# swacisko/ALGA

Hardware: AMD Instinct MI355X
Metric: overlap_edges_per_sec (higher is better)
Workload: dtype u32; 1 GPU; cfg4_50M_150bp: 50000000 x 150 bp reads, genome 250000000, seed 11, err 0.00 -> 90621096 nodes (both strands, duplicates removed), min_overlap 82, rsoemo 116; generated on the device (alga_amd.workload.device_build) in 1.0 s; nodes=90621096, edges=92350115

## Files before the change

### alga_amd/csrc/engine.hip

```cpp
#include <hip/hip_runtime.h>

#include <algorithm>
#include <chrono>
#include <cstdio>
#include <cstdlib>
#include <cstring>
#include <new>
#include <string>
#include <thread>
#include <vector>

#include "engine_internal.h"
#include "prefsuf_shard.h"

using namespace alga;

namespace {

using Prepared = AlgaPrepared;

int prepare(alga_engine *e, const alga_nodes *nodes, const alga_prefsuf_params *p, hipStream_t s, Prepared &out) {
    if (!nodes || !p) return alga_fail(e, ALGA_ERR_INVALID_ARGUMENT, "nodes/params must not be NULL");
    if (nodes->n < 0) return alga_fail(e, ALGA_ERR_INVALID_ARGUMENT, "negative node count");
    if (nodes->n > 0 && (!nodes->words || !nodes->len)) return alga_fail(e, ALGA_ERR_INVALID_ARGUMENT, "words/len must not be NULL");
    if (nodes->stride_words <= 0 && nodes->n > 0) return alga_fail(e, ALGA_ERR_INVALID_ARGUMENT, "stride_words must be positive");
    if (p->min_overlap < 1 || p->min_overlap > 501) return alga_fail(e, ALGA_ERR_INVALID_ARGUMENT, "min_overlap must be in [1, 501]");
    if (p->soes != 3) return alga_fail(e, ALGA_ERR_INVALID_ARGUMENT, "soes must be 3 (the reference hard-codes SOES = 3)");
    if (p->max_len_cap < 1 || p->max_len_cap > 500) return alga_fail(e, ALGA_ERR_INVALID_ARGUMENT, "max_len_cap must be in [1, 500]");
    if (p->rsoe_min_overlap < 0) return alga_fail(e, ALGA_ERR_INVALID_ARGUMENT, "rsoe_min_overlap must be >= 0");
    if (p->keys_shared < 0 || p->keys_shared > 2) return alga_fail(e, ALGA_ERR_INVALID_ARGUMENT, "keys_shared must be 0, 1 or 2");
    int rc;
    if ((rc = alga_ensure(e, e->counters, (CNT_TOTAL + 2) * sizeof(unsigned long long)))) return rc;
    HIP_TRY(e, hipMemsetAsync(e->counters.p, 0, (CNT_TOTAL + 2) * sizeof(unsigned long long), s));
    NodesDev nd;
    nd.words = nodes->words; nd.len = nodes->len; nd.from = nodes->align_from; nd.to = nodes->align_to;
    nd.n = nodes->n; nd.stride = nodes->stride_words;
    unsigned long long *cnt = (unsigned long long *) e->counters.p;
    int *d_maxlen = (int *) (cnt + CNT_TOTAL);
    unsigned long long mask_asym = 0;
    int min_len = 0;
    if (p->keys_shared == 2 && e->store_n == nodes->n && e->store_words == (const void *) nodes->words && e->stat_len == (const void *) nodes->len &&
        e->stat_from == (const void *) nodes->align_from && e->stat_to == (const void *) nodes->align_to) {
        out.max_len = e->stat_max_len; out.live = e->stat_live; mask_asym = e->stat_mask_asym; min_len = e->stat_min_len;
    } else {
        launch_node_stats(nd, cnt, d_maxlen, s);
        if ((rc = alga_check_launch(e, "k_node_stats"))) return rc;
        HIP_TRY(e, hipMemcpyAsync(e->h_counters, e->counters.p, (CNT_TOTAL + 2) * sizeof(unsigned long long), hipMemcpyDeviceToHost, s));
        HIP_TRY(e, hipStreamSynchronize(s));
        out.max_len = (int) (e->h_counters[CNT_TOTAL] & 0xFFFFFFFFull);
        min_len = out.max_len > 0 ? 0x7FFFFFFF - (int) (e->h_counters[CNT_TOTAL] >> 32) : 0;
        out.live = e->h_counters[CNT_LIVE_NODES];
        mask_asym = e->h_counters[CNT_MASK_ASYM];
        e->stat_max_len = out.max_len; e->stat_min_len = min_len; e->stat_live = out.live; e->stat_mask_asym = mask_asym;
        e->stat_len = (const void *) nodes->len; e->stat_from = (const void *) nodes->align_from; e->stat_to = (const void *) nodes->align_to;
    }
    out.nd = nd;
    out.uniform_len = (out.max_len > 0 && min_len == out.max_len && !nodes->align_from) ? out.max_len : 0;
    if ((int64_t) blocks_of(out.max_len) > (int64_t) nodes->stride_words)
        return alga_fail(e, ALGA_ERR_INVALID_ARGUMENT, "stride_words is smaller than the longest read needs");
    if (out.max_len > OL_MAX_NODE_LEN) return alga_fail(e, ALGA_ERR_CAPACITY, "a node is longer than 4 194 303 nt (overlap records keep the offset in 22 bits)");
    PrefSufCfg c;
    c.Lmin = p->min_overlap;
    c.rsoemo = p->rsoe_min_overlap;
    c.Lcap = std::min(out.max_len, p->max_len_cap) + 1;
    c.soes = p->soes;
    const int seed_nt = std::min(c.Lmin, SEED_MAX_NT);
    c.seed_words = (2 * seed_nt + 31) >> 5;
    c.seed_last_mask = (2 * seed_nt & 31) ? ((1u << (2 * seed_nt & 31)) - 1u) : 0xFFFFFFFFu;
    c.reversed = (c.rsoemo > c.Lcap) ? 1 : 0;
    c.stats = p->collect_stats ? 1 : 0;
    out.cfg = c;
    if (p->reduction < ALGA_REDUCTION_AUTO || p->reduction > ALGA_REDUCTION_SOURCE_SIDE)
        return alga_fail(e, ALGA_ERR_INVALID_ARGUMENT, "reduction must be an alga_reduction value");
    out.local_ok = out.max_len <= p->max_len_cap && out.max_len - c.Lmin <= LOCAL_MAX_SPAN && c.Lmin <= c.rsoemo && c.rsoemo <= c.Lcap &&
                   mask_asym == 0;
    out.local_sw = out.max_len - c.Lmin <= 63 ? 1 : 2;
    out.cluster_eq = 0;
    const bool wide = out.local_sw == 2 || blocks_of(out.max_len) > 13;
    if (out.local_ok && e->opt_probe != ALGA_PROBE_TABLE && !(wide && e->opt_probe == ALGA_PROBE_AUTO && out.live < (4ull << 20))) {
        int eq = 0;
        if (cluster_plan(c, out.max_len, out.live, e->opt_cluster_bucket_bias, &out.cluster, &eq)) out.cluster_eq = eq;
    }
    out.keys_shared = p->keys_shared;
    out.reduction = p->reduction;
    if (out.reduction == ALGA_REDUCTION_AUTO && e->opt_force_per_target) out.reduction = ALGA_REDUCTION_PER_TARGET;
    return ALGA_OK;
}

int cluster_alloc(alga_engine *e, const Prepared &pp) {
    int rc;
    const uint64_t n = (uint64_t) pp.nd.n;
    for (int k = 0; k < 2; k++) {
        if ((rc = alga_ensure(e, e->cl_keys[k], (n + ALGA_KEY_ARRAY_SLACK + 1) * sizeof(uint32_t)))) return rc;
        if ((rc = alga_ensure(e, e->cl_vals[k], (n + 1) * sizeof(uint32_t)))) return rc;
    }
    if ((rc = alga_ensure(e, e->cl_meta, (n + ALGA_KEY_ARRAY_SLACK + 1) * sizeof(uint32_t)))) return rc;
    if ((rc = alga_ensure(e, e->cl_runs, (n + 1) * CL_RMAX * 8))) return rc;
    if ((rc = alga_ensure(e, e->cl_nruns, n + 16))) return rc;
    if ((rc = alga_ensure(e, e->cl_store, (n + 2) * 16 * (size_t) pp.cluster_eq))) return rc;
    if ((rc = alga_ensure(e, e->cl_dir, ((size_t) pp.cluster.n_buckets + 2) * 16))) return rc;
    return alga_ensure(e, e->sort_temp, cluster_sort_temp_bytes(n));
}

int pile_alloc(alga_engine *e, uint64_t n, uint32_t n_buckets, hipStream_t s) {
    int rc;
    if ((rc = alga_ensure(e, e->cl_pile_rec, pile_record_bytes(n)))) return rc;
    if ((rc = alga_ensure(e, e->cl_pile_rec2, pile_record_bytes(n)))) return rc;
    if ((rc = alga_ensure(e, e->cl_pile_succ, ((size_t) n + 64) * 16))) return rc;
    if ((rc = alga_ensure(e, e->cl_pile_cnt, PILE_CNT_WORDS * sizeof(unsigned long long)))) return rc;
    if ((rc = alga_ensure(e, e->cl_pile_own, pile_own_mask_bytes(n)))) return rc;
    if (e->opt_pile_runs_list && (rc = alga_ensure(e, e->cl_pile_list, pile_list_bytes(n)))) return rc;
    if ((rc = alga_ensure(e, e->cl_defer, (size_t) (n + 64) * sizeof(int32_t)))) return rc;
    const void *before = e->cl_pile_tab.p;
    const size_t cap_before = e->cl_pile_tab.cap;
    if ((rc = alga_ensure(e, e->cl_pile_tab, pile_table_bytes(n_buckets)))) return rc;
    if (e->cl_pile_tab.p != before || e->cl_pile_tab.cap != cap_before) {
        HIP_TRY(e, hipMemsetAsync(e->cl_pile_tab.p, 0, e->cl_pile_tab.cap, s));
        HIP_TRY(e, hipStreamSynchronize(s));
        e->pile_epoch = 0;
    }
    return ALGA_OK;
}

int discover_impl(alga_engine *e, const Prepared &pp, int32_t src_begin, int32_t src_end, hipStream_t s, uint64_t *n_rec, bool local = false,
                  bool *overflow = nullptr) {
    int rc;
    const NodesDev &nd = pp.nd;
    const PrefSufCfg &cfg = pp.cfg;
    unsigned long long *cnt = (unsigned long long *) e->counters.p;
    *n_rec = 0;
    HIP_TRY(e, hipEventRecord(e->ev[EV_START], s));
    if (pp.live >= (1ull << 31)) return alga_fail(e, ALGA_ERR_CAPACITY, "too many nodes for one seed table; shard the input");
    const bool clustered = local && pp.cluster_eq != 0;
    e->pairs_timed = false;
    e->store_timed = false;
    e->pile_timed = false;
    e->pile_deg_pending = false;
    const bool all_sources = src_begin == 0 && src_end == pp.nd.n;
    const bool pile_index_left = e->opt_pile_range != 0 && e->pile_n == pp.nd.n && e->pile_words == (const void *) pp.nd.words;
    bool pile = clustered && e->opt_pile != 0 && e->opt_cluster_pairs != 0 && e->opt_cluster_order != 0 && pp.local_sw == 1 &&
                      (pp.keys_shared == 0 || (pp.keys_shared == 2 && pile_index_left)) &&
                      (all_sources || (e->opt_pile_range != 0 && src_begin >= 0 && src_end <= pp.nd.n && src_begin < src_end)) && pile_plan(cfg, pp.cluster, pp.cluster_eq, pp.uniform_len, pp.nd.from != nullptr || pp.nd.to != nullptr);
    e->loc_second_used = false;
    bool keys_only = false;
    const bool need_vals = !e->opt_own_sort || e->opt_test_unsorted_index;
    uint32_t n_buckets = 0, filter_bits = 0;
    bool have_table = false;
    auto build_table = [&]() -> int {
        n_buckets = seed_buckets_for(pp.live, e->seed_fill_x10);
        const size_t table_bytes = (size_t) n_buckets * SEED_BUCKET * sizeof(unsigned long long);
        int r;
        if ((r = alga_ensure(e, e->table, table_bytes))) return r;
        HIP_TRY(e, hipMemsetAsync(e->table.p, 0xFF, table_bytes, s));
        filter_bits = seed_filter_bits_for(pp.live);
        if (filter_bits) {
            if ((r = alga_ensure(e, e->filter, filter_bits / 8))) return r;
            HIP_TRY(e, hipMemsetAsync(e->filter.p, 0, filter_bits / 8, s));
        }
        launch_seed_build(nd, cfg, (unsigned long long *) e->table.p, n_buckets, (uint32_t *) e->filter.p, filter_bits, s);
        if ((r = alga_check_launch(e, "k_seed_build"))) return r;
        e->stats.table_slots = (uint64_t) n_buckets * SEED_BUCKET;
        have_table = true;
        return ALGA_OK;
    };
    ClusterCfg cc{};
    if (clustered) {
        cc = pp.cluster;
        if ((rc = cluster_alloc(e, pp))) return rc;
        if (pp.keys_shared == 2) {
            const bool store_left = e->store_n == nd.n && e->store_words == (const void *) nd.words && e->store_eq == pp.cluster_eq && e->store_buckets == cc.n_buckets;
            const bool piles_serve = pile && e->pile_kept_pure && e->store_buckets == cc.n_buckets && e->store_eq == pp.cluster_eq;
            if (!(store_left || piles_serve) || src_begin < e->store_run_begin || src_end > e->store_run_end)
                return alga_fail(e, ALGA_ERR_INVALID_ARGUMENT, "keys_shared = 2: no entry array of this node set that covers the sources is left from the previous build");
            keys_only = pile && e->pile_keys_only;
        } else {
            int32_t run_begin = 0, run_end = nd.n;
            if (pp.keys_shared == 1) {
                if (e->keyed_n != nd.n || e->keyed_words != (const void *) nd.words || src_begin < e->keyed_begin || src_end > e->keyed_end)
                    return alga_fail(e, ALGA_ERR_INVALID_ARGUMENT, "keys_shared: alga_prefsuf_keys_device has not been called on this node set for a range that covers the sources");
                run_begin = e->keyed_begin; run_end = e->keyed_end;
            } else {
                keys_only = pile && e->opt_pile_runs != 0 && !e->expect_pairwise && !e->opt_pile_check;
                launch_cluster_keys(nd, cfg, cc, 0, nd.n, (uint32_t *) e->cl_keys[0].p, need_vals ? (uint32_t *) e->cl_vals[0].p : nullptr, (uint32_t *) e->cl_meta.p, e->cl_runs.p,
                                    (uint8_t *) e->cl_nruns.p, s, !keys_only);
                if ((rc = alga_check_launch(e, "k_node_runs"))) return rc;
            }
            HIP_TRY(e, hipEventRecord(e->ev[EV_KEYS], s));
            e->keyed_n = -1;
            e->store_n = -1;
            HIP_TRY(e, launch_cluster_sort(nd, cc, (uint32_t *) e->cl_keys[0].p, (uint32_t *) e->cl_vals[0].p, (uint32_t *) e->cl_keys[1].p,
                                           (uint32_t *) e->cl_vals[1].p, e->sort_temp.p, cluster_sort_temp_bytes((uint64_t) nd.n), pp.keys_shared == 1 || !need_vals,
                                           e->ev[EV_SORT], e->opt_test_unsorted_index != 0, s, e->opt_own_sort != 0));
            const bool dir_late = pile && e->opt_pile_dir >= 1;
            e->dir_late = dir_late;
            if (!dir_late) {
                HIP_TRY(e, launch_cluster_dir(nd, cc, (const uint32_t *) e->cl_keys[1].p, e->cl_dir.p, cnt + CNT_TOTAL + 1, nullptr, s));
                HIP_TRY(e, hipEventRecord(e->ev[EV_DIR], s));
            }
            e->pile_n = -1;
            if (pile) {
                rc = e->opt_test_pile_oom ? alga_fail(e, ALGA_ERR_OUT_OF_MEMORY, "pile_alloc (option test_pile_oom)") : pile_alloc(e, (uint64_t) nd.n, cc.n_buckets, s);
                if (rc == ALGA_ERR_OUT_OF_MEMORY) {
                    (void) hipGetLastError();
                    alga_release(e->cl_pile_tab); alga_release(e->cl_pile_rec); alga_release(e->cl_pile_rec2); alga_release(e->cl_pile_succ); alga_release(e->cl_pile_own);
                    alga_release(e->cl_pile_list);
                    e->pile_epoch = 0; e->pile_n = -1;
                    e->err.clear();
                    pile = false;
                    rc = ALGA_OK;
                    if (keys_only) {
                        launch_cluster_keys(nd, cfg, cc, 0, nd.n, (uint32_t *) e->cl_keys[0].p, (uint32_t *) e->cl_vals[0].p, (uint32_t *) e->cl_meta.p, e->cl_runs.p,
                                            (uint8_t *) e->cl_nruns.p, s, true);
                        if ((rc = alga_check_launch(e, "k_node_runs"))) return rc;
                        keys_only = false;
                    }
                } else if (rc) return rc;
            }
            if (pile) {
                launch_pile_sample(nd, cc, pp.uniform_len, (const uint32_t *) e->cl_keys[1].p, (const uint32_t *) e->cl_vals[1].p, e->cl_dir.p,
                                   (unsigned long long *) e->cl_pile_cnt.p, e->opt_pile >= 2 ? e->opt_pile - 1 : 0, s, e->opt_pile_dir >= 1);
                if ((rc = alga_check_launch(e, "k_pile_build<sample>"))) return rc;
            }
            e->pile_tab_index = pile && e->opt_pile_dir >= 2 && e->opt_pile_skip_gather && !cfg.stats;
            if (dir_late) {
                HIP_TRY(e, hipEventRecord(e->ev[EV_SAMPLE], s));
                HIP_TRY(e, launch_cluster_dir(nd, cc, (const uint32_t *) e->cl_keys[1].p, e->cl_dir.p, cnt + CNT_TOTAL + 1,
                                              e->pile_tab_index ? (const unsigned long long *) e->cl_pile_cnt.p : nullptr, s));
                HIP_TRY(e, hipEventRecord(e->ev[EV_DIR], s));
            }
            HIP_TRY(e, launch_cluster_gather(nd, cc, pp.cluster_eq, (const uint32_t *) e->cl_keys[1].p, (const uint32_t *) e->cl_vals[1].p, (const uint32_t *) e->cl_meta.p,
                                             pp.uniform_len, e->cl_store.p, (pile && e->opt_pile_skip_gather) ? (const unsigned long long *) e->cl_pile_cnt.p : nullptr, s));
            HIP_TRY(e, hipEventRecord(e->ev[EV_GATHER], s));
            if (pile) {
                if (e->pile_epoch >= 511u) {
                    HIP_TRY(e, hipMemsetAsync(e->cl_pile_tab.p, 0, e->cl_pile_tab.cap, s));
                    e->pile_epoch = 0;
                }
                e->pile_epoch++;
                const bool from_consensus = e->opt_pile_runs != 0;
                launch_pile_build(nd, cfg, cc, pp.uniform_len, (const uint32_t *) e->cl_keys[1].p, (const uint32_t *) e->cl_vals[1].p, e->cl_dir.p, e->cl_pile_rec.p, e->cl_pile_rec2.p, e->cl_pile_tab.p,
                                  e->pile_epoch, e->cl_pile_succ.p, e->cl_runs.p, pp.uniform_len - cfg.Lmin + 1, (const unsigned long long *) e->cl_pile_cnt.p,
                                  from_consensus ? (uint32_t *) e->cl_pile_own.p : nullptr, (from_consensus && e->opt_pile_runs_list) ? e->cl_pile_list.p : nullptr, s,
                                  e->opt_pile_dir >= 1, cnt + CNT_TOTAL + 1, e->pile_tab_index, e->opt_pile_runs_ahead != 0);
                if ((rc = alga_check_launch(e, "k_pile_build"))) return rc;
                if (keys_only) {
                    launch_pile_own_ids((const uint32_t *) e->cl_pile_own.p, (const uint32_t *) e->cl_vals[1].p, (uint64_t) nd.n, (int32_t *) e->cl_defer.p, (uint32_t) nd.n,
                                        (unsigned long long *) e->cl_pile_cnt.p, s);
                    launch_cluster_runs_list(nd, cfg, cc, (const int32_t *) e->cl_defer.p, (const unsigned long long *) e->cl_pile_cnt.p + 3, (uint32_t) nd.n, (uint32_t) e->n_cu * 16u,
                                             e->cl_runs.p, (uint8_t *) e->cl_nruns.p, s);
                    launch_cluster_keys(nd, cfg, cc, 0, nd.n, (uint32_t *) e->cl_keys[0].p, (uint32_t *) e->cl_vals[0].p, (uint32_t *) e->cl_meta.p, e->cl_runs.p,
                                        (uint8_t *) e->cl_nruns.p, s, true, (const unsigned long long *) e->cl_pile_cnt.p);
                    if ((rc = alga_check_launch(e, "k_node_runs (own lists)"))) return rc;
                }
                if (e->opt_pile_check && from_consensus)
                    launch_pile_check(e->cl_pile_succ.p, (uint64_t) nd.n, cc.n_buckets, e->cl_pile_tab.p, e->cl_pile_rec2.p, e->pile_epoch, e->cl_runs.p, nd.n, pp.uniform_len - cfg.Lmin + 1,
                                      (unsigned long long *) e->cl_pile_cnt.p, s);
                e->pile_n = nd.n; e->pile_words = (const void *) nd.words;
                e->pile_keys_only = keys_only; e->pile_kept_pure = false;
                e->pile_timed = nd.n > 0;
            }
            e->store_timed = nd.n > 0;
            e->store_n = pile ? -1 : nd.n;
            e->store_words = (const void *) nd.words; e->store_eq = pp.cluster_eq; e->store_buckets = cc.n_buckets;
            e->store_run_begin = run_begin; e->store_run_end = run_end;
        }
        e->stats.table_slots = cc.n_buckets;
    } else if ((rc = build_table())) return rc;
    HIP_TRY(e, hipEventRecord(e->ev[EV_SEED], s));

    const uint64_t n_src = (uint64_t) std::max<int64_t>(0, (int64_t) src_end - src_begin);
    const uint64_t slack = std::max(probe_record_slack(e->n_cu, n_src, local), clustered ? cluster_record_slack(e->n_cu, n_src) : 0);
    uint64_t &hint = local ? e->rec_cap_hint_local : e->rec_cap_hint;
    uint64_t cap = std::max<uint64_t>(hint, (local ? 2 : 16) * n_src + 4096) + slack;
    if (local) {
        if ((rc = alga_ensure(e, e->outdeg, (size_t) (n_src + 1) * sizeof(uint32_t)))) return rc;
        if ((rc = alga_ensure(e, e->loc_first, (size_t) (n_src + 1) * sizeof(unsigned long long)))) return rc;
    }
    const uint32_t big_list_cap = 1u << 20;
    if (local && (rc = alga_ensure(e, e->loc_big_list, big_list_cap * sizeof(int32_t)))) return rc;
    bool pure_streamed = false;
    for (int attempt = 0; attempt < 4; attempt++) {
        if (cap >= (1ull << 32) - 16) return alga_fail(e, ALGA_ERR_CAPACITY, "more than 2^32 overlap records; shard the input");
        if (local) HIP_TRY(e, hipMemsetAsync(e->outdeg.p, 0, (size_t) (n_src + 1) * sizeof(uint32_t), s));
        if ((rc = alga_ensure(e, e->rec_dst, cap * sizeof(uint32_t)))) return rc;
        if ((rc = alga_ensure(e, e->rec_val, cap * sizeof(unsigned long long)))) return rc;
        HIP_TRY(e, hipMemsetAsync(cnt, 0, CNT_TOTAL * sizeof(unsigned long long), s));
        ProbeBig big{(int32_t *) e->loc_big_list.p, big_list_cap, 0u, nullptr, 0u};
        e->defer_list_valid = clustered && e->opt_cluster_pairs && pp.local_sw == 1 && pp.cluster_eq <= 4;
        if (clustered) {
            if (e->opt_cluster_pairs && pp.local_sw == 1 && pp.cluster_eq <= 4) {
                if ((rc = alga_ensure(e, e->cl_defer, (size_t) (n_src + 64) * sizeof(int32_t)))) return rc;
                const uint32_t slot_stride = e->opt_stream_slots >= 4 ? (uint32_t) (n_src + 1) : 0u;
                if ((rc = alga_ensure(e, e->loc_second, (size_t) (slot_stride ? LOCAL_SLOTS_MAX - 1 : 1) * (n_src + 1) * sizeof(unsigned long long)))) return rc;
                e->loc_second_used = true;
                e->loc_slot_stride = slot_stride;
                const bool by_key = e->opt_cluster_order != 0 && src_begin == 0 && src_end == nd.n;
                const bool piled = pile && e->pile_n == nd.n && e->pile_words == (const void *) nd.words;
                if (piled) {
                    if (!all_sources) {
                        if ((rc = alga_ensure(e, e->cl_pile_side_r, (size_t) (n_src + 64) * 16))) return rc;
                        if ((rc = alga_ensure(e, e->cl_pile_cursor, 64))) return rc;
                    }
                    launch_pile_probe(nd, cfg, cc, pp.uniform_len, e->cl_pile_tab.p, e->pile_epoch, e->cl_pile_rec.p, e->cl_pile_rec2.p, e->cl_pile_succ.p,
                                      e->cl_runs.p, cnt, (uint32_t *) e->outdeg.p, (unsigned long long *) e->loc_first.p, (unsigned long long *) e->loc_second.p,
                                      (int32_t *) e->cl_defer.p, (uint32_t) n_src, (const unsigned long long *) e->cl_pile_cnt.p, e->n_cu, s, src_begin, src_end,
                                      e->cl_pile_side_r.p, (unsigned long long *) e->cl_pile_cursor.p, e->opt_pile_probe_lean != 0, e->opt_pile_probe_tail != 0);
                    if ((rc = alga_check_launch(e, "k_pile_probe"))) return rc;
                    if (keys_only)
                        launch_cluster_runs_list(nd, cfg, cc, (const int32_t *) e->cl_defer.p, cnt + CNT_DEFERRED, (uint32_t) std::min<uint64_t>(n_src + 64, 0xFFFFFFFFull),
                                                 (uint32_t) e->n_cu * 16u, e->cl_runs.p, (uint8_t *) e->cl_nruns.p, s);
                }
                launch_probe_stream(nd, cfg, cc, pp.cluster_eq, e->cl_store.p, e->cl_dir.p, e->cl_runs.p, (const uint8_t *) e->cl_nruns.p,
                                    src_begin, src_end, by_key, cnt, e->n_cu, (uint32_t *) e->outdeg.p, (unsigned long long *) e->loc_first.p,
                                    (unsigned long long *) e->loc_second.p, (int32_t *) e->cl_defer.p, (uint32_t) n_src,
                                    piled ? (const unsigned long long *) e->cl_pile_cnt.p : nullptr, s, slot_stride);
                if ((rc = alga_check_launch(e, "k_probe_stream"))) return rc;
                if (piled) {
                    if ((rc = alga_ensure(e, e->cl_defer2, (size_t) (n_src + 64) * sizeof(int32_t)))) return rc;
                    pure_streamed = launch_probe_stream_list(nd, cfg, cc, pp.cluster_eq, e->cl_store.p, e->cl_dir.p, e->cl_runs.p, (const uint8_t *) e->cl_nruns.p, (int32_t *) e->cl_defer.p,
                                             (uint32_t) n_src, cnt, e->n_cu, (uint32_t *) e->outdeg.p, (unsigned long long *) e->loc_first.p,
                                             (unsigned long long *) e->loc_second.p, (int32_t *) e->cl_defer2.p, (const unsigned long long *) e->cl_pile_cnt.p, s, slot_stride, src_begin,
                                             (const uint32_t *) e->cl_keys[1].p, (const uint32_t *) e->cl_vals[1].p, pp.uniform_len, e->opt_pile_stream_by_id != 0,
                                             e->pile_tab_index ? e->cl_pile_tab.p : nullptr, e->pile_epoch);
                    if ((rc = alga_check_launch(e, "k_probe_stream (list)"))) return rc;
                }
                HIP_TRY(e, hipEventRecord(e->ev[EV_PAIRS], s));
                e->pairs_timed = true;
                launch_probe_clustered(nd, cfg, cc, pp.cluster_eq, e->cl_store.p, e->cl_dir.p, e->cl_runs.p, (const uint8_t *) e->cl_nruns.p, 0,
                                       (int32_t) n_src, (const int32_t *) e->cl_defer.p, src_begin, (uint32_t *) e->rec_dst.p, (unsigned long long *) e->rec_val.p,
                                       cap, cnt, e->n_cu, (uint32_t *) e->outdeg.p, (unsigned long long *) e->loc_first.p, &big, cnt + CNT_DEFERRED, 1, s,
                                       (const uint32_t *) e->cl_keys[1].p, (const uint32_t *) e->cl_vals[1].p, pp.uniform_len,
                                       (piled && e->opt_pile_skip_gather) ? (const unsigned long long *) e->cl_pile_cnt.p : nullptr,
                                       (piled && e->pile_tab_index) ? e->cl_pile_tab.p : nullptr, e->pile_epoch);
                e->pile_deg_pending = piled && e->opt_pile_deg_fold != 0;
                if (piled && !e->pile_deg_pending) launch_pile_deg((int32_t) n_src, (unsigned long long *) e->loc_first.p, (uint32_t *) e->outdeg.p, (const unsigned long long *) e->cl_pile_cnt.p, s);
            } else {
                launch_probe_clustered(nd, cfg, cc, pp.cluster_eq, e->cl_store.p, e->cl_dir.p, e->cl_runs.p, (const uint8_t *) e->cl_nruns.p, src_begin,
                                       src_end, nullptr, src_begin, (uint32_t *) e->rec_dst.p, (unsigned long long *) e->rec_val.p, cap, cnt, e->n_cu,
                                       (uint32_t *) e->outdeg.p, (unsigned long long *) e->loc_first.p, &big, nullptr, pp.local_sw, s);
            }
        }
        else
            launch_probe(nd, cfg, (const unsigned long long *) e->table.p, n_buckets, (const uint32_t *) e->filter.p, filter_bits, src_begin, src_end,
                         (uint32_t *) e->rec_dst.p, (unsigned long long *) e->rec_val.p, cap, cnt, e->n_cu, local ? pp.local_sw : 0, (uint32_t *) e->outdeg.p,
                         (unsigned long long *) e->loc_first.p, local ? &big : nullptr, s);
        if ((rc = alga_check_launch(e, "k_probe_sources"))) return rc;
        HIP_TRY(e, hipEventRecord(e->ev[EV_PROBE], s));
        HIP_TRY(e, hipMemcpyAsync(e->h_counters, cnt, (CNT_TOTAL + 2) * sizeof(unsigned long long), hipMemcpyDeviceToHost, s));
        HIP_TRY(e, hipStreamSynchronize(s));
        if (clustered && e->h_counters[CNT_TOTAL + 1] != 0) {
            e->store_n = -1; e->keyed_n = -1;
            return alga_fail(e, ALGA_ERR_HIP, "clustered index: the sorted key array is not in order (entry directory invalid)");
        }
        if (local && e->h_counters[CNT_LOCAL_OVERFLOW] != 0) {
            const uint64_t n_big = e->h_counters[CNT_LOCAL_OVERFLOW], max_items = e->h_counters[CNT_LOCAL_MAXITEMS];
            const uint64_t limit = e->big_limit >= 0 ? (uint64_t) e->big_limit : (uint64_t) local_big_limit();
            if (n_big > big_list_cap || max_items > limit) { if (overflow) *overflow = true; *n_rec = 0; return ALGA_OK; }
            big.count = (uint32_t) n_big;
            big.item_cap = (uint32_t) ((max_items + 63) & ~63ull);
            if ((rc = alga_ensure(e, e->loc_big_items, probe_big_bytes(e->n_cu, big.count, pp.local_sw, big.item_cap)))) return rc;
            big.items = e->loc_big_items.p;
            if (!have_table && (rc = build_table())) return rc;
            if (e->pile_deg_pending) {
                launch_pile_deg((int32_t) n_src, (unsigned long long *) e->loc_first.p, (uint32_t *) e->outdeg.p, (const unsigned long long *) e->cl_pile_cnt.p, s);
                e->pile_deg_pending = false;
            }
            HIP_TRY(e, hipMemsetAsync(cnt + CNT_LOCAL_OVERFLOW, 0, sizeof(unsigned long long), s));
            launch_probe(nd, cfg, (const unsigned long long *) e->table.p, n_buckets, (const uint32_t *) e->filter.p, filter_bits, src_begin, src_end,
                         (uint32_t *) e->rec_dst.p, (unsigned long long *) e->rec_val.p, cap, cnt, e->n_cu, pp.local_sw, (uint32_t *) e->outdeg.p,
                         (unsigned long long *) e->loc_first.p, &big, s);
            if ((rc = alga_check_launch(e, "k_probe_sources (second pass)"))) return rc;
            HIP_TRY(e, hipEventRecord(e->ev[EV_PROBE], s));
            HIP_TRY(e, hipMemcpyAsync(e->h_counters, cnt, CNT_TOTAL * sizeof(unsigned long long), hipMemcpyDeviceToHost, s));
            HIP_TRY(e, hipStreamSynchronize(s));
            if (e->h_counters[CNT_LOCAL_OVERFLOW] != 0) { if (overflow) *overflow = true; *n_rec = 0; return ALGA_OK; }
            e->stats.big_sources = n_big;
        }
        const uint64_t need = e->h_counters[CNT_RECORDS];
        if (need <= cap) {
            *n_rec = need;
            hint = std::max<uint64_t>(hint, need + need / 16 + 4096);
            if (overflow) *overflow = false;
            if (local) { e->stats.transitive_compares = e->h_counters[CNT_TR_COMPARES]; e->stats.generic_sources = e->h_counters[CNT_LOCAL_GENERIC]; }
            e->stats.records = e->h_counters[CNT_VALID_RECORDS];
            e->stats.raw_overlaps = e->h_counters[CNT_RAW];
            e->stats.windows_probed = e->h_counters[CNT_WINDOWS];
            e->stats.slots_scanned = e->h_counters[CNT_SLOTS];
            e->stats.probe_rounds = e->h_counters[CNT_ROUNDS];
            e->stats.pile_buckets = e->h_counters[CNT_PILE_BUCKETS]; e->stats.pile_irregular = e->h_counters[CNT_PILE_IRREGULAR];
            e->stats.pile_own_lists = e->h_counters[CNT_PILE_OWN];
            if (pile && pp.keys_shared != 2 && e->pile_n == nd.n) {
                const bool kept = e->opt_pile == 2 || e->stats.pile_irregular * (uint64_t) ALGA_PILE_DECLINE_ONE_IN <= e->stats.pile_buckets;
                e->stats.pile_mixed = kept && e->stats.pile_irregular * (uint64_t) ALGA_PILE_IRREGULAR_ONE_IN > e->stats.pile_buckets;
                e->stats.pile_deferred = (e->stats.pile_mixed || (kept && pure_streamed)) ? e->h_counters[CNT_DEFERRED_PILE] : (kept ? e->h_counters[CNT_DEFERRED] : 0);
                if (!kept || e->stats.pile_mixed || !e->opt_pile_skip_gather) e->store_n = nd.n;
                e->expect_pairwise = !kept;
                e->pile_kept_pure = kept && !e->stats.pile_mixed && e->opt_pile_skip_gather != 0;
                e->stats.pile_list_checked = 0; e->stats.pile_list_mismatch = 0;
                if (e->opt_pile_check) {
                    unsigned long long chk[2] = {0ull, 0ull};
                    HIP_TRY(e, hipMemcpyAsync(chk, (const unsigned long long *) e->cl_pile_cnt.p + 4, sizeof(chk), hipMemcpyDeviceToHost, s));
                    HIP_TRY(e, hipStreamSynchronize(s));
                    e->stats.pile_list_checked = chk[0]; e->stats.pile_list_mismatch = chk[1];
// ... 130 lines not shown
    return ALGA_OK;
}

double now_ms_host() { return std::chrono::duration<double, std::milli>(std::chrono::steady_clock::now().time_since_epoch()).count(); }

float ev_ms(alga_engine *e, int a, int b) {
    float ms = 0.f;
    if (hipEventElapsedTime(&ms, e->ev[a], e->ev[b]) != hipSuccess) return 0.f;
    return ms;
}

void store_phase_stats(alga_engine *e) {
    if (!e->store_timed) return;
    e->stats.ms_keys = ev_ms(e, EV_START, EV_KEYS);
    e->stats.ms_sort = ev_ms(e, EV_KEYS, EV_SORT);
    e->stats.ms_dir = ev_ms(e, e->dir_late ? EV_SAMPLE : EV_SORT, EV_DIR);
    e->stats.ms_gather = ev_ms(e, EV_DIR, EV_GATHER) + (e->dir_late ? ev_ms(e, EV_SORT, EV_SAMPLE) : 0.0);
    e->stats.ms_pile = e->pile_timed ? ev_ms(e, EV_GATHER, EV_SEED) : 0.0;
}

}

int alga_prepare(alga_engine *e, const alga_nodes *nodes, const alga_prefsuf_params *p, hipStream_t s, AlgaPrepared &out) { return prepare(e, nodes, p, s, out); }
int alga_cluster_alloc(alga_engine *e, const AlgaPrepared &pp) { return cluster_alloc(e, pp); }

extern "C" {

int alga_abi_version(void) { return ALGA_AMD_ABI_VERSION; }

struct DeviceGuard {
    int prev = -1;
    DeviceGuard() { if (hipGetDevice(&prev) != hipSuccess) prev = -1; }
    ~DeviceGuard() { if (prev >= 0) (void) hipSetDevice(prev); }
};

static void engine_free_handles(alga_engine *e) {
    if (e->h_counters) (void) hipHostFree(e->h_counters);
    for (int i = 0; i < EV_COUNT; i++) if (e->ev[i]) (void) hipEventDestroy(e->ev[i]);
    if (e->own_stream) (void) hipStreamDestroy(e->own_stream);
    if (e->side_stream) (void) hipStreamDestroy(e->side_stream);
    if (e->ev_side) (void) hipEventDestroy(e->ev_side);
    e->h_counters = nullptr; e->own_stream = nullptr; e->side_stream = nullptr; e->ev_side = nullptr;
    for (int i = 0; i < EV_COUNT; i++) e->ev[i] = nullptr;
}

int alga_engine_create(int hip_device, alga_engine **out) {
    if (!out) return ALGA_ERR_INVALID_ARGUMENT;
    *out = nullptr;
    int ndev = 0;
    hipError_t err = hipGetDeviceCount(&ndev);
    if (err != hipSuccess || ndev <= 0) return ALGA_ERR_NO_DEVICE;
    if (hip_device < 0 || hip_device >= ndev) return ALGA_ERR_INVALID_ARGUMENT;
    DeviceGuard guard;
    if (hipSetDevice(hip_device) != hipSuccess) return ALGA_ERR_NO_DEVICE;
    alga_engine *e = new (std::nothrow) alga_engine();
    if (!e) return ALGA_ERR_OUT_OF_MEMORY;
    e->device = hip_device;
    memset(&e->stats, 0, sizeof(e->stats));
    hipDeviceProp_t prop;
    if (hipGetDeviceProperties(&prop, hip_device) == hipSuccess) {
        snprintf(e->dev_name, sizeof(e->dev_name), "%s (%s, %d CUs)", prop.name, prop.gcnArchName, prop.multiProcessorCount);
        if (prop.multiProcessorCount > 0) e->n_cu = prop.multiProcessorCount;
    }
    int rc = ALGA_OK;
    if (hipStreamCreateWithFlags(&e->own_stream, hipStreamNonBlocking) != hipSuccess) { e->own_stream = nullptr; rc = ALGA_ERR_HIP; }
    if (rc == ALGA_OK && hipStreamCreateWithFlags(&e->side_stream, hipStreamNonBlocking) != hipSuccess) { e->side_stream = nullptr; rc = ALGA_ERR_HIP; }
    if (rc == ALGA_OK && hipEventCreateWithFlags(&e->ev_side, hipEventDisableTiming) != hipSuccess) { e->ev_side = nullptr; rc = ALGA_ERR_HIP; }
    for (int i = 0; i < EV_COUNT && rc == ALGA_OK; i++)
        if (hipEventCreate(&e->ev[i]) != hipSuccess) { e->ev[i] = nullptr; rc = ALGA_ERR_HIP; }
    if (rc == ALGA_OK && hipHostMalloc((void **) &e->h_counters, (CNT_TOTAL + 2 + alga_engine::H_EXTRA) * sizeof(unsigned long long)) != hipSuccess) { e->h_counters = nullptr; rc = ALGA_ERR_OUT_OF_MEMORY; }
    if (rc == ALGA_OK && hipHostGetDevicePointer((void **) &e->h_counters_dev, e->h_counters, 0) != hipSuccess) rc = ALGA_ERR_HIP;
    if (rc != ALGA_OK) { engine_free_handles(e); delete e; return rc; }
    *out = e;
    return ALGA_OK;
}

void alga_engine_destroy(alga_engine *e) {
    if (!e) return;
    DeviceGuard guard;
    (void) hipSetDevice(e->device);
    if (e->own_stream) (void) hipStreamSynchronize(e->own_stream);
    if (e->side_stream) (void) hipStreamSynchronize(e->side_stream);
    for (DevBuf *b : e->owned) alga_release(*b);
    alga_release(e->up_raw);
    for (DevBuf *b : {&e->in_bytes[0], &e->in_bytes[1], &e->in_nl[0], &e->in_nl[1], &e->in_tiles, &e->in_tile_off}) alga_release(*b);
    for (DevBuf *b : {&e->sp_rowptr, &e->sp_sorted, &e->sp_list, &e->sp_cnt, &e->sp_orow, &e->sp_out, &e->sp_in}) alga_release(*b);
    alga_staging_release(e);
    for (void *&p : e->gfa_pin) { if (p) (void) hipHostFree(p); p = nullptr; }
    for (auto &kv : e->host_lists) free(kv.first);
    e->host_lists.clear();
    engine_free_handles(e);
    delete e;
}

const char *alga_last_error(const alga_engine *e) { return e ? e->err.c_str() : "no engine"; }

int alga_engine_device_name(const alga_engine *e, char *buf, size_t buflen) {
    if (!e || !buf || buflen == 0) return ALGA_ERR_INVALID_ARGUMENT;
    snprintf(buf, buflen, "%s", e->dev_name);
    return ALGA_OK;
}

int alga_engine_set_option(alga_engine *e, const char *name, int64_t value) {
    if (!e || !name) return ALGA_ERR_INVALID_ARGUMENT;
    e->err.clear();
    if (!strcmp(name, "probe")) {
        if (value < ALGA_PROBE_AUTO || value > ALGA_PROBE_CLUSTER) return alga_fail(e, ALGA_ERR_INVALID_ARGUMENT, "option probe: 0 auto, 1 table, 2 cluster");
        e->opt_probe = (int) value;
    } else if (!strcmp(name, "cluster_bucket_bias")) {
        if (value < -8 || value > 8) return alga_fail(e, ALGA_ERR_INVALID_ARGUMENT, "option cluster_bucket_bias: -8 .. 8");
        e->opt_cluster_bucket_bias = (int) value;
    } else if (!strcmp(name, "cluster_pairs")) {
        e->opt_cluster_pairs = value != 0;
    } else if (!strcmp(name, "pile")) {
        e->opt_pile = (value == 2 || value == 3) ? (int) value : (value != 0);
    } else if (!strcmp(name, "pile_runs")) {
        e->opt_pile_runs = value != 0;
    } else if (!strcmp(name, "pile_runs_list")) {
        e->opt_pile_runs_list = value != 0;
    } else if (!strcmp(name, "pile_dir")) {
        if (value < 0 || value > 2) return alga_fail(e, ALGA_ERR_INVALID_ARGUMENT, "option pile_dir: 0 directory records, 1 k_pile_build from the keys, 2 ... and no directory for a pure pile build");
        e->opt_pile_dir = (int) value;
    } else if (!strcmp(name, "pile_deg_fold")) {
        e->opt_pile_deg_fold = value != 0;
    } else if (!strcmp(name, "emit_fused")) {
        e->opt_emit_fused = value != 0;
    } else if (!strcmp(name, "pile_probe_lean")) {
        e->opt_pile_probe_lean = value != 0;
    } else if (!strcmp(name, "pile_probe_tail")) {
        e->opt_pile_probe_tail = value != 0;
    } else if (!strcmp(name, "pile_runs_ahead")) {
        e->opt_pile_runs_ahead = value != 0;
    } else if (!strcmp(name, "pile_stream_by_id")) {
        e->opt_pile_stream_by_id = value != 0;
    } else if (!strcmp(name, "pile_check")) {
        e->opt_pile_check = value != 0;
    } else if (!strcmp(name, "pile_skip_gather")) {
        e->opt_pile_skip_gather = value != 0;
    } else if (!strcmp(name, "cluster_order")) {
        e->opt_cluster_order = value != 0;
    } else if (!strcmp(name, "local_big_max")) {
        e->big_limit = value < 0 ? -1 : (int) std::min<int64_t>(value, 1 << 20);
    } else if (!strcmp(name, "shard_bucket_max")) {
        e->opt_shard_dmax = (int) std::max<int64_t>(1, std::min<int64_t>(value, 4096));
    } else if (!strcmp(name, "rsort_variant")) {
        if (value < 0 || value > 1) return alga_fail(e, ALGA_ERR_INVALID_ARGUMENT, "option rsort_variant: 0 tiles of 8192 pairs, 1 tiles of 16384 pairs");
        rsort_set_variant((int) value);
    } else if (!strcmp(name, "stream_slots")) {
        e->opt_stream_slots = value >= 4 ? 4 : 2;
    } else if (!strcmp(name, "pile_range")) {
        e->opt_pile_range = value != 0;
    } else if (!strcmp(name, "pkb_legacy")) {
        e->opt_pkb_legacy = (int) value;
    } else if (!strcmp(name, "own_sort")) {
        e->opt_own_sort = value != 0;
    } else if (!strcmp(name, "test_presort_oom")) {
        e->opt_test_presort_oom = value != 0;
    } else if (!strcmp(name, "test_pile_oom")) {
        e->opt_test_pile_oom = value != 0;
    } else if (!strcmp(name, "test_unsorted_index")) {
        e->opt_test_unsorted_index = value != 0;
    } else if (!strcmp(name, "gfa_chunk_mb")) {
        if (value < 1 || value > 4096) return alga_fail(e, ALGA_ERR_INVALID_ARGUMENT, "option gfa_chunk_mb: 1 .. 4096");
        e->opt_gfa_chunk_mb = (int) value;
    } else if (!strcmp(name, "mst_mid_nodes")) {
        if (value < 8 || value > (1 << 20)) return alga_fail(e, ALGA_ERR_INVALID_ARGUMENT, "option mst_mid_nodes: 8 .. 2^20");
        e->opt_mst_mid_nodes = (int) value;
    } else if (!strcmp(name, "consensus_max_blocks")) {
        if (value < 0 || value > (1 << 20)) return alga_fail(e, ALGA_ERR_INVALID_ARGUMENT, "option consensus_max_blocks: 0 .. 2^20");
        e->opt_consensus_max_blocks = (int) value;
    } else if (!strcmp(name, "unitig_ruling")) {
        if (value < -1 || value > 1) return alga_fail(e, ALGA_ERR_INVALID_ARGUMENT, "option unitig_ruling: -1, 0 or 1");
        e->opt_unitig_ruling = (int) value;
    } else if (!strcmp(name, "correct_slice_keys")) {
        if (value < 1 || value > (1ll << 31)) return alga_fail(e, ALGA_ERR_INVALID_ARGUMENT, "option correct_slice_keys: 1 .. 2^31");
        e->opt_correct_slice_keys = value;
    } else if (!strcmp(name, "correct_dir_bits")) {
        if (value < 0 || value > 28) return alga_fail(e, ALGA_ERR_INVALID_ARGUMENT, "option correct_dir_bits: 0 (auto) or 1 .. 28");
        e->opt_correct_dir_bits = (int) value;
    } else if (!strcmp(name, "place_dir_bits")) {
        if (value < 0 || value > 26) return alga_fail(e, ALGA_ERR_INVALID_ARGUMENT, "option place_dir_bits: 0 (auto) or 1 .. 26");
        e->opt_place_dir_bits = (int) value;
    } else if (!strcmp(name, "ipolish_max_blocks")) {
        if (value < 1 || value > 8192) return alga_fail(e, ALGA_ERR_INVALID_ARGUMENT, "option ipolish_max_blocks: 1 .. 8192");
        e->opt_ipolish_max_blocks = (int) value;
    } else if (!strcmp(name, "auto_reduction_per_target")) {
        e->opt_force_per_target = value != 0;
    } else return alga_fail(e, ALGA_ERR_INVALID_ARGUMENT, "unknown option");
    return ALGA_OK;
}

int alga_engine_reserve(alga_engine *e, int32_t n_nodes, int32_t max_len, int32_t min_overlap, uint64_t n_edges_hint) {
    if (!e) return ALGA_ERR_INVALID_ARGUMENT;
    e->err.clear();
    if (n_nodes < 0 || max_len < 1 || min_overlap < 1) return alga_fail(e, ALGA_ERR_INVALID_ARGUMENT, "alga_engine_reserve: n_nodes >= 0, max_len >= 1, min_overlap >= 1");
    DeviceGuard guard;
    HIP_TRY(e, hipSetDevice(e->device));
    int rc;
    const uint64_t n = (uint64_t) n_nodes;
    const uint64_t E = n_edges_hint ? n_edges_hint : n + n / 16 + 4096;
    if ((rc = alga_ensure(e, e->counters, (CNT_TOTAL + 2) * sizeof(unsigned long long)))) return rc;
    Prepared pp;
    pp.nd.n = n_nodes; pp.max_len = max_len; pp.live = n;
    pp.cfg.Lmin = min_overlap; pp.cfg.Lcap = std::min(max_len, 500) + 1; pp.cfg.rsoemo = min_overlap; pp.cfg.soes = 3;
    int eq = 0;
    const bool local = max_len <= 500 && max_len - min_overlap <= LOCAL_MAX_SPAN;
    const bool clustered = local && e->opt_probe != ALGA_PROBE_TABLE &&
                           cluster_plan(pp.cfg, max_len, n, e->opt_cluster_bucket_bias, &pp.cluster, &eq);
    if (clustered) {
        pp.cluster_eq = eq;
        if ((rc = cluster_alloc(e, pp))) return rc;
        if (max_len - min_overlap <= 63 && eq <= 4) {
            if ((rc = alga_ensure(e, e->cl_defer, (size_t) (n + 64) * sizeof(int32_t)))) return rc;
            if ((rc = alga_ensure(e, e->loc_second, (size_t) (e->opt_stream_slots >= 4 ? LOCAL_SLOTS_MAX - 1 : 1) * (n + 1) * sizeof(unsigned long long)))) return rc;
        }
        if (e->opt_pile != 0 && e->opt_cluster_pairs != 0 && e->opt_cluster_order != 0 && max_len - min_overlap <= 63 && pile_plan(pp.cfg, pp.cluster, eq, max_len, false)) {
            if ((rc = pile_alloc(e, n, pp.cluster.n_buckets, e->own_stream))) return rc;
        }
    } else {
        const uint32_t nb = seed_buckets_for(n, e->seed_fill_x10);
        if ((rc = alga_ensure(e, e->table, (size_t) nb * SEED_BUCKET * sizeof(unsigned long long)))) return rc;
        const uint32_t fb = seed_filter_bits_for(n);
        if (fb && (rc = alga_ensure(e, e->filter, fb / 8))) return rc;
    }
    if (local) {
        const uint64_t slack = std::max(probe_record_slack(e->n_cu, n, true), clustered ? cluster_record_slack(e->n_cu, n) : 0);
        const uint64_t cap = std::max<uint64_t>(e->rec_cap_hint_local, 2 * n + 4096) + slack;
        if ((rc = alga_ensure(e, e->outdeg, (size_t) (n + 1) * sizeof(uint32_t)))) return rc;
        if ((rc = alga_ensure(e, e->loc_first, (size_t) (n + 1) * sizeof(unsigned long long)))) return rc;
        if ((rc = alga_ensure(e, e->loc_big_list, (1u << 20) * sizeof(int32_t)))) return rc;
        if ((rc = alga_ensure(e, e->rec_dst, cap * sizeof(uint32_t)))) return rc;
        if ((rc = alga_ensure(e, e->rec_val, cap * sizeof(unsigned long long)))) return rc;
        if ((rc = alga_ensure(e, e->scan_scratch, scan_scratch_bytes(n)))) return rc;
        if ((rc = alga_ensure(e, e->out_rowptr, (size_t) (n + 1) * sizeof(uint32_t)))) return rc;
        if ((rc = alga_ensure(e, e->out_cnt, (size_t) (n + 1) * sizeof(uint32_t)))) return rc;
    }
    if ((rc = alga_ensure(e, e->edges, (size_t) (E + 1) * sizeof(alga_edge_dev)))) return rc;
    if (!e->warmed && n_nodes > 0) {
        const int W = blocks_of(max_len), stride = hbm_row_stride(W), wn = 4096;
        std::vector<uint32_t> rows((size_t) wn * stride, 0u);
        std::vector<int32_t> lens((size_t) wn, max_len);
        uint64_t x = 0x9E3779B97F4A7C15ull;
        for (int i = 0; i < wn; i++)
            for (int k = 0; k < W; k++) {
                x ^= x << 13; x ^= x >> 7; x ^= x << 17;
                uint32_t w = (uint32_t) (x >> 16);
                const int used = 2 * max_len - 32 * k;
                if (used < 32) w &= used <= 0 ? 0u : ((1u << used) - 1u);
                rows[(size_t) i * stride + k] = w;
            }
        void *d_rows = nullptr, *d_len = nullptr;
        if (hipMalloc(&d_rows, rows.size() * 4) == hipSuccess && hipMalloc(&d_len, lens.size() * 4) == hipSuccess &&
            hipMemcpy(d_rows, rows.data(), rows.size() * 4, hipMemcpyHostToDevice) == hipSuccess &&
            hipMemcpy(d_len, lens.data(), lens.size() * 4, hipMemcpyHostToDevice) == hipSuccess) {
            alga_nodes nd{(const uint32_t *) d_rows, stride, (const int32_t *) d_len, wn, nullptr, nullptr};
            alga_prefsuf_params wp;
            alga_prefsuf_default_params(&wp);
            wp.min_overlap = min_overlap; wp.rsoe_min_overlap = std::min(max_len, min_overlap + (max_len - min_overlap) / 2);
            const alga_edge *d = nullptr;
            uint64_t m = 0;
            const int wrc = alga_prefsuf_build_device(e, &nd, &wp, nullptr, &d, &m);
            (void) wrc;
            e->err.clear();
            e->warmed = true;
        }
        if (d_rows) (void) hipFree(d_rows);
        if (d_len) (void) hipFree(d_len);
        (void) hipGetLastError();
        alga_forget_node_set(e);
        memset(&e->stats, 0, sizeof(e->stats));
    }
    return ALGA_OK;
}

void alga_prefsuf_default_params(alga_prefsuf_params *p) {
    if (!p) return;
    memset(p, 0, sizeof(*p));
    p->min_overlap = 0;
    p->rsoe_min_overlap = 0;
    p->soes = 3;
    p->max_len_cap = 500;
    p->collect_stats = 0;
}

int alga_prefsuf_build_device(alga_engine *e, const alga_nodes *nodes, const alga_prefsuf_params *p, void *hip_stream,
                              const alga_edge **d_edges, uint64_t *n_edges) {
    if (!e) return ALGA_ERR_INVALID_ARGUMENT;
    e->err.clear();
    if (!d_edges || !n_edges) return alga_fail(e, ALGA_ERR_INVALID_ARGUMENT, "output pointers must not be NULL");
    *d_edges = nullptr; *n_edges = 0;
    HIP_TRY(e, hipSetDevice(e->device));
    hipStream_t s = hip_stream ? (hipStream_t) hip_stream : e->own_stream;
    memset(&e->stats, 0, sizeof(e->stats));
    Prepared pp;
    int rc = prepare(e, nodes, p, s, pp);
    if (rc) return rc;
    e->stats.nodes_live = pp.live;
    uint64_t n_rec = 0, E = 0;
    bool done = false;
    if (pp.reduction == ALGA_REDUCTION_SOURCE_SIDE || (pp.reduction == ALGA_REDUCTION_AUTO && pp.local_ok)) {
        rc = build_local(e, pp, 0, nodes->n, s, &E);
        if (rc == ALGA_OK) done = true;
        else if (rc != ALGA_ERR_UNSUPPORTED || pp.reduction == ALGA_REDUCTION_SOURCE_SIDE) return rc;
        else { e->err.clear(); memset(&e->stats, 0, sizeof(e->stats)); e->stats.nodes_live = pp.live; }
    }
    if (!done) {
// ... 581 lines not shown
```

### alga_amd/csrc/engine_internal.h

```cpp
#pragma once
#include <hip/hip_runtime.h>

#include <cstdio>
#include <algorithm>
#include <string>
#include <vector>
#include <unordered_map>

#include "../../include/alga_amd.h"
#include "prefsuf_common.h"
#include "prefsuf_kernels.h"
#include "pkb_kernels.h"

struct DevBuf {
    void  *p = nullptr;
    size_t cap = 0;
};

enum { EV_START = 0, EV_SEED, EV_PROBE, EV_GROUP, EV_REDUCE, EV_EMIT, EV_PAIRS, EV_KEYS, EV_SORT, EV_GATHER, EV_DIR, EV_SAMPLE, EV_COUNT };
constexpr int ALGA_STAGE_THREADS = 8;

struct alga_engine {
    std::vector<DevBuf *> owned;
    int         device = -1;
    hipStream_t own_stream = nullptr;
    hipStream_t side_stream = nullptr;
    hipEvent_t  ev_side = nullptr;
    std::string err;
    char        dev_name[256] = {0};
    int         n_cu = 256;
    int         seed_fill_x10 = 20;
    int         opt_probe = 0;
    int         opt_cluster_bucket_bias = 0;
    int         opt_force_per_target = 0;
    int         opt_shard_dmax = 4096;
    int         opt_test_unsorted_index = 0;
    hipEvent_t  ev[EV_COUNT] = {};
    DevBuf table, filter, counters, rowptr, rec_dst, rec_val, keys, seg_key, seg_val, heads, sort_temp, out_cnt, outdeg, out_rowptr, edges, scan_scratch;
    DevBuf cl_defer;
    uint32_t h_first_hkey = 255;
    int32_t keyed_n = -1, keyed_begin = 0, keyed_end = 0;
    bool defer_list_valid = false;
    const void *keyed_words = nullptr;
    int32_t store_n = -1, store_run_begin = 0, store_run_end = 0, store_eq = 0;
    uint32_t store_buckets = 0;
    const void *store_words = nullptr;
    int stat_max_len = 0, stat_min_len = 0; uint64_t stat_live = 0; unsigned long long stat_mask_asym = 0;
    const void *stat_len = nullptr, *stat_from = nullptr, *stat_to = nullptr;
    bool   warmed = false;
    bool   pairs_timed = false;
    bool   store_timed = false;
    bool   pile_keys_only = false, pile_kept_pure = false;
    int    opt_pile_range = 1;
    int    opt_pile_skip_gather = 1;
    int    opt_pile = 1;
    int    opt_pile_runs = 1;
    int    opt_pile_runs_list = 1;
    DevBuf cl_pile_list;
    int    opt_pile_deg_fold = 1;
    int    opt_emit_fused = 1;
    int    opt_pile_dir = 2;
    bool   dir_late = false;
    bool   pile_tab_index = false;
    int    opt_pile_stream_by_id = 0;
    int    opt_pile_probe_lean = 1;
    int    opt_pile_probe_tail = 1;
    int    opt_pile_runs_ahead = 0;
    bool   pile_deg_pending = false;
    int    opt_pile_check = 0;
    bool   expect_pairwise = false;
    DevBuf cl_pile_side_r, cl_pile_cursor;
    DevBuf cl_pile_own;
    int    opt_pkb_legacy = 0;
    int    opt_own_sort = 1;
    int    opt_test_presort_oom = 0;
    int    opt_test_pile_oom = 0;
    bool   pile_timed = false;
    DevBuf cl_pile_succ;
    DevBuf cl_pile_rec2;
    DevBuf cl_pile_rec, cl_pile_cnt, cl_pile_tab;
    uint32_t pile_epoch = 0;
    int32_t pile_n = -1; const void *pile_words = nullptr;
    int    opt_cluster_order = 1;
    int    opt_cluster_pairs = 1;
    DevBuf cl_keys[2], cl_vals[2], cl_meta, cl_runs, cl_nruns, cl_store, cl_dir;
    DevBuf loc_second;
    bool   loc_second_used = false;
    uint32_t loc_slot_stride = 0;
    int    opt_stream_slots = 4;
    DevBuf loc_first, loc_big_list, loc_big_items;
    int    big_limit = -1;
    DevBuf edge_keys, edge_keys2, edge_vals, edge_vals2, edges_sorted, xs_dst, xs_val;
    DevBuf up_words, up_len, up_from, up_to;
    DevBuf up_len_narrow;
    DevBuf cp_deg, cp_dst, cp_off;
    DevBuf cl_defer2;
    DevBuf pk_keys, pk_keys2, pk_vals, pk_vals2, pk_marks, pk_big, pk_add, pk_ekeys, pk_ekeys2, pk_flag, pk_pos, pk_edges[2], pk_rowptr, pk_deg,
           pk_mask, pk_cnt, pk_io, pk_io2, pk_tips, pk_heads, pk_g[2], pk_addk, pk_addk2, pk_merged, pk_hsz, pk_hsz2, pk_heads2, pk_nadd, pk_koff,
           pk_gsz, pk_fixlist, pk_bounds, pk_tiprec, pk_tipidx, pk_keys_all, pk_vals_all;
    DevBuf pk_keys2b, pk_vals2b, pk_headsb, pk_hszb, sort_temp2, pk_fixlist2, pk_cnt2;
    DevBuf pp_rows, pp_len, pp_perm[2], pp_keys[2], pp_mark, pp_keep, pp_pos, pp_out_rows, pp_out_len, pp_out_pair, pp_tally;
    bool        stage_ready = false;
    void       *stage_pin[ALGA_STAGE_THREADS][2] = {};
    hipEvent_t  stage_ev[ALGA_STAGE_THREADS][2] = {};
    hipStream_t stage_stream[ALGA_STAGE_THREADS] = {};
    DevBuf      up_raw;
    std::unordered_map<void *, size_t> host_lists;
    void       *host_spare = nullptr;
    size_t      host_spare_cap = 0;
    DevBuf      in_bytes[2], in_nl[2], in_tiles, in_tile_off;
    DevBuf      sp_rowptr, sp_sorted, sp_list, sp_cnt, sp_orow, sp_out, sp_in;
    DevBuf      tp_cnt, tp_keys[2], tp_vals[2], tp_flag, tp_pos, tp_best, tp_est, tp_rev, tp_rfid, tp_rowptr[2], tp_alive, tp_kill, tp_rec[2], tp_branch,
                tp_overflow, tp_ws, tp_out;
    DevBuf      mp_cnt, mp_rowptr, mp_rows, mp_len, mp_owner, mp_pend[2], mp_win, mp_overflow, mp_overflow2, mp_ws, mp_ws_big, mp_orow, mp_out;
    struct MstFilled { const void *p = nullptr; size_t bytes = 0; uint32_t hbits = 0, cap_nodes = 0, cap_edges = 0; int32_t n_ws = 0; } mp_filled[2];
    int         opt_mst_mid_nodes = 4096;
    DevBuf      gfa_sizes, gfa_off, gfa_rowptr, gfa_tiles, gfa_bounds, gfa_buf;
    void       *gfa_pin[2] = {nullptr, nullptr};
    size_t      gfa_pin_cap = 0;
    int         opt_gfa_chunk_mb = 256;
    DevBuf      ut_cnt, ut_keys[2], ut_vals[2], ut_flag, ut_pos, ut_best, ut_estar, ut_rowptr, ut_nxt, ut_noff, ut_prv, ut_rank[2], ut_min[2], ut_tail,
                ut_win, ut_pair, ut_pcnt, ut_ulen, ut_ulen2, ut_uwords, ut_path_off, ut_word_off, ut_tiles, ut_path_node, ut_path_pos, ut_uid, ut_words,
                ut_edges, ut_link, ut_rnode, ut_rrec[2];
    int         opt_unitig_ruling = -1;
    uint64_t    ut_n_pairs = 0, ut_n_edges = 0;
    bool        ut_valid = false;
    int32_t     ut_n_nodes = 0;
    uint64_t    ut_total_bases = 0;
    bool        ut_is_contig = false;
    DevBuf      ex_cnt, ex_rowptr, ex_w, ex_kcnt, ex_dlink, ex_outcnt, ex_sole, ex_xhead, ex_xbase, ex_xrank, ex_uid, ex_scnt, ex_seam_off,
                ex_seam_entry, ex_pcnt, ex_uwords, ex_ulen, ex_ulen2, ex_path_off, ex_word_off, ex_path_node, ex_path_pos, ex_words, ex_edges;
    bool        ut_is_extended = false;
    DevBuf      ct_cnt, ct_B[2], ct_rowptr, ct_pflag, ct_runkey, ct_chain, ct_headchain, ct_drop, ct_flag, ct_pos, ct_keys[2], ct_vals[2], ct_hw, ct_hk, ct_H,
                ct_hrow, ct_hsorted, ct_hlist, ct_hcnt, ct_win, ct_pair, ct_oid, ct_cid, ct_deg, ct_epos, ct_ekeys[2], ct_evals[2], ct_names;
    DevBuf      cs_cnt, cs_words, cs_mask, cs_votes, cs_trim, cs_len, cs_changed;
    bool        cs_valid = false;
    bool        cs_has_votes = false;
    DevBuf      fc_cnt, fc_keys[2], fc_vals, fc_first, fc_min, fc_list[2], fc_flag, fc_ids, fc_verdict, fc_rank, fc_id, fc_new, fc_trim, fc_begin, fc_len,
                fc_order, fc_wbegin, fc_wlen, fc_rows, fc_rlen, fc_tid;
    bool        fc_valid = false;
    uint64_t    fc_n_accepted = 0;
    int         opt_consensus_max_blocks = 0;
    DevBuf      cr_cnt, cr_table, cr_hist, cr_keys[2], cr_flag, cr_pos, cr_solid, cr_dir;
    int64_t     opt_correct_slice_keys = 1ll << 28;
    int         opt_correct_dir_bits = 0;
    DevBuf      seed_keys[2], seed_vals[2], seed_dir, seed_ub;
    DevBuf      pl_cnt, pl_fbegin, pl_flen, pl_scan, pl_cols, pl_diff;
    DevBuf      pl_target, pl_pos, pl_mm, pl_hits, pl_state, pl_coloff, pl_cover, pl_tstat, pl_hist;
    bool        pl_valid = false;
    uint64_t    pl_targets = 0, pl_reads = 0;
    uint64_t    pl_ncolumns = 0, pl_nhist = 0;
    uint64_t    pl_final_epoch = 0;
    uint64_t    fc_epoch = 0;
    int         opt_place_dir_bits = 0;
    DevBuf      po_cnt, po_keys[2], po_vals[2], po_marks, po_pop, po_scan;
    DevBuf      po_coloff, po_words, po_ccols, po_cbases, po_tstat, po_counts;
    bool        po_valid = false;
    uint64_t    po_targets = 0, po_columns = 0;
    uint64_t    po_final_epoch = 0;
    uint64_t    pl_serial = 0, po_pl_serial = 0;
    DevBuf      sc_cnt, sc_keys[2], sc_vals[2], sc_span, sc_heads, sc_pos, sc_bstart, sc_best, sc_choice, sc_partner, sc_lists[2], sc_head, sc_first, sc_scan;
    DevBuf      sc_ba, sc_bb, sc_blinks, sc_bspan, sc_bgap, sc_bstate, sc_estate, sc_scaffold, sc_rank, sc_orient, sc_start, sc_gapafter, sc_jlinks, sc_soff,
                sc_smembers, sc_slen;
    bool        sc_valid = false;
    uint64_t    sc_targets = 0, sc_scaffolds = 0, sc_longest = 0;
    uint64_t    sc_pl_serial = 0;
    DevBuf      br_cnt, br_diff, br_starts, br_rpos, br_marks, br_rfirst, br_rlast, br_closed, br_cpos;
    DevBuf      br_span, br_ccols, br_cfirst, br_clast, br_tcuts, br_poff, br_begin, br_len, br_ptarget, br_pstart, br_words;
    bool        br_valid = false;
    uint64_t    br_targets = 0, br_pieces = 0, br_cuts = 0, br_columns = 0, br_longest = 0;
    DevBuf      gr_cnt, gr_flag, gr_pos, gr_cand, gr_elen, gr_eoff, gr_ecols, gr_x, gr_g;
    struct GrowSet { DevBuf end, over, mm, hits, state, count, estop, evoters, left, right, len, coloff, begin, words; } gr_set[2];
    int         gr_cur = 0;
    bool        gr_valid = false;
    uint64_t    gr_reads = 0, gr_targets = 0, gr_columns = 0, gr_longest = 0;
    DevBuf      mg_cnt, mg_elen, mg_epad, mg_eoff, mg_ecols, mg_pcols, mg_join, mg_lists[2], mg_head, mg_first, mg_scan;
    struct MergeSet { DevBuf partner, olen, mm, hits, estate, merged, rank, orient, start, ovafter, moff, mmembers, len, coloff, begin, words; } mg_set[2];
    int         mg_cur = 0;
    bool        mg_valid = false;
    uint64_t    mg_targets = 0, mg_merged = 0, mg_columns = 0, mg_longest = 0;
    DevBuf      gp_cnt, gp_flag, gp_pos, gp_list, gp_cols, gp_best, gp_runs, gp_nruns, gp_diff, gp_scan;
    DevBuf      gp_target, gp_rpos, gp_end, gp_edits, gp_state, gp_cigoff, gp_cigar, gp_cover, gp_tstat;
    bool        gp_valid = false;
    uint64_t    gp_reads = 0, gp_targets = 0, gp_columns = 0, gp_ncigar = 0;
    uint64_t    gp_pl_serial = 0;
    DevBuf      ip_cnt, ip_keys[2], ip_vals[2], ip_marks, ip_pop, ip_pwords, ip_ptstat, ip_counts4, ip_del, ip_diff, ip_scan, ip_ikey[2], ip_islot[2], ip_winkey,
                ip_winvotes, ip_insall, ip_width, ip_evn, ip_evoff, ip_code;
    struct IpolishSet { DevBuf len, coloff, begin, words, newcol, evcol, evkind, evlen, evbases, evvotes, evcover, tstat, counts, span, oldoff; } ip_set[2];
    int         ip_cur = 0;
    int         opt_ipolish_max_blocks = 8192;
    bool        ip_valid = false;
    uint64_t    ip_targets = 0, ip_columns = 0, ip_columns_before = 0, ip_events = 0, ip_longest = 0;
    DevBuf      sh_keys[2], sh_vals[2], sh_store, sh_dir, sh_desc_out, sh_dkey[2], sh_dval[2], sh_small_top, sh_pending, sh_bitmap, sh_small_out,
                sh_ssrc[2], sh_skey[2], sh_edges_out, sh_deg, sh_rowptr, sh_cursor, sh_edges, sh_flagged, sh_cnt, sh_gflag, sh_gpos, sh_gstart;
    struct {
        int      phase = 0;
        int      rank = 0, n_ranks = 1, eq = 0, uniform_len = 0;
        int32_t  n = 0;
        const void *words = nullptr;
        alga::PrefSufCfg cfg{};
        alga::ClusterCfg cc{};
        uint32_t bucket_base = 0, bpr = 0;
        uint64_t n_targets = 0, n_desc = 0, n_rec = 0;
        uint32_t *d_keys_sorted = nullptr;
        unsigned long long *d_vals_sorted = nullptr;
    } sh;
    alga_shard_stats shard_stats{};
    struct {
        int      phase = 0;
        int      rounds = 0, round = 0, rank = 0, n_ranks = 1, cur = 0, key_bits = 0;
        int32_t  prio[4] = {0, 1, 2, 3};
        uint64_t E = 0, nk = 0;
        uint32_t n_tips = 0;
        int      pre_set = 0, cur_set = 0;
        bool     no_look_ahead = false;
        int      pre_round = -1;
        bool     kmers_all = false;
        size_t   kmers_stride = 0;
        int      kmers_sort_bits = 0;
        alga_nodes dn{};
// ... 122 lines not shown
```

### alga_amd/csrc/prefsuf_cluster.hip

```cpp
#include <hip/hip_runtime.h>
#include <algorithm>
#include "prefsuf_common.h"
#include "prefsuf_kernels.h"
#include "prefsuf_device.h"
#include "prefsuf_cluster_device.h"

namespace alga {


template <int TKW, bool WIDE, bool RUNS>
__global__ void __launch_bounds__(TK_ROWS) k_node_runs(NodesDev nd, PrefSufCfg cfg, ClusterCfg cc, int node_begin, int node_end,
                                                        uint32_t *__restrict__ keys, uint32_t *__restrict__ vals, uint32_t *__restrict__ meta,
                                                        uint2 *__restrict__ runs, uint8_t *__restrict__ nruns, const int32_t *__restrict__ id_list, const unsigned long long *__restrict__ id_count,
                                                        const unsigned long long *__restrict__ only_if_declined ) {
    if (only_if_declined && !pile_cnt_declines(only_if_declined)) return;
    __shared__ uint32_t s[TK_ROWS][TKW];
    __shared__ uint32_t stk[RUNS ? 2 * (NR_STACK + 1) : 1][TK_ROWS];
    __shared__ uint16_t rbuf[RUNS ? CL_RMAX + 1 : 1][TK_ROWS];
    const int list_n = id_list ? (int) min((unsigned long long) (node_end - node_begin), *id_count) : 0;
    __shared__ int sid[TK_ROWS];
    for (int blk = (int) blockIdx.x; id_list ? blk * TK_ROWS < list_n : node_begin + blk * TK_ROWS < node_end; blk += (int) gridDim.x) {
    const int base = node_begin + blk * TK_ROWS;
    const int nrows = id_list ? min(TK_ROWS, list_n - blk * TK_ROWS) : min(TK_ROWS, node_end - base);
    if (blk != (int) blockIdx.x) __syncthreads();
    if (id_list) {
        if ((int) threadIdx.x < nrows) sid[threadIdx.x] = min(max(id_list[blk * TK_ROWS + (int) threadIdx.x], 0), nd.n - 1);
        __syncthreads();
    }
    if ((nd.stride & 3) == 0 && 4 * ((TKW + 3) / 4) <= nd.stride && (reinterpret_cast<uintptr_t>(nd.words) & 15u) == 0) {
        constexpr int PCS = (TKW + 3) / 4;
        for (int u = (int) threadIdx.x; u < nrows * PCS; u += TK_ROWS) {
            const int r = u / PCS, pc = u - r * PCS;
            const uint4 x = *reinterpret_cast<const uint4 *>(nd.words + (size_t) (id_list ? sid[r] : base + r) * nd.stride + 4 * pc);
            const uint32_t xs[4] = {x.x, x.y, x.z, x.w};
#pragma unroll
            for (int q = 0; q < 4; q++) if (4 * pc + q < TKW) s[r][4 * pc + q] = xs[q];
        }
    } else
    for (int c = (int) (threadIdx.x & 15u); c < TKW; c += 16)
        for (int r = (int) (threadIdx.x >> 4); r < nrows; r += TK_ROWS / 16)
            s[r][c] = c < nd.stride ? nd.words[(size_t) (id_list ? sid[r] : base + r) * nd.stride + c] : 0u;
    __syncthreads();
    const int t = (int) threadIdx.x;
    const bool in = t < nrows;
    const int i = id_list ? sid[in ? t : 0] : base + (in ? t : 0);
    const int len = in ? nd.len[i] : 0;
    const bool act = in && len >= cfg.Lmin && len > 0;
    const bool is_tgt = act && (!nd.to || nd.to[i]);
    const bool is_src = act && (!nd.from || nd.from[i]);
    const uint32_t *row = s[in ? t : 0];
    const int w = cc.w;
    const int nwin = len - cfg.Lmin + 1;
    const int fs = cc.idx_shift - CL_MBITS;
    int nr = 0;
    bool uncovered = false;
    bool stack_ovf = false;
    uint32_t cur0 = 0xFFFFFFFFu;
    if (RUNS) {
        node_runs_core<WIDE>(row, nwin, act, cc, stk, rbuf, t, nr, uncovered, stack_ovf, cur0);
        const int nr_stored = nr < CL_RMAX ? nr : CL_RMAX;
        const uint32_t nr_code = !is_src ? 0u : ((nr > CL_RMAX || stack_ovf || uncovered) ? (uint32_t) CL_RUNS_FLAGGED : (uint32_t) nr);
        int p1 = nwin;
        for (int r = 0; r < CL_RMAX; r++) {
            if (r < nr_stored && is_src) {
                const uint32_t d = rbuf[r][t];
                const int q = (int) (d & 255u);
                uint32_t h, pk;
                kmer_key(row, q < (WIDE ? 192 : 128) ? q : 0, true, cc, h, pk);
                runs[(size_t) i * CL_RMAX + r] = make_uint2(cluster_key(h, fs), d | ((uint32_t) p1 << 16) | (r == 0 ? nr_code << 24 : 0u));
                p1 = (int) (d >> 8);
            }
        }
        if (in && !is_src) runs[(size_t) i * CL_RMAX] = make_uint2(0u, 0u);
        if (in) nruns[i] = (uint8_t) nr_code;
        if (id_list) continue;
    } else {
        const int nk = act ? min(nwin, WIDE ? 64 : nwin) - 1 + w : 0;
        uint64_t b0;
        {
            const uint32_t x0 = row[0], x1 = row[1], x2 = row[2], x3 = row[3], x4 = row[4];
            const uint32_t d0 = compress_even(class0_mask16(x0, x1)) | (compress_even(class0_mask16(x1, x2)) << 16);
            const uint32_t d1 = compress_even(class0_mask16(x2, x3)) | (compress_even(class0_mask16(x3, x4)) << 16);
            b0 = (uint64_t) d0 | ((uint64_t) d1 << 32);
            b0 &= nk >= 64 ? ~0ull : (nk <= 0 ? 0ull : ((1ull << nk) - 1ull));
            b0 &= w >= 64 ? ~0ull : ((1ull << w) - 1ull);
        }
        while (b0 != 0ull) {
            const int e = __builtin_ctzll(b0);
            b0 &= b0 - 1ull;
            const int bit = 2 * e, q = bit >> 5, r = bit & 31;
            const uint32_t x0 = row[q], x1 = row[q + 1], x2 = row[q + 2];
            const uint32_t pk = order_key0(kmer_hash(funnel(x0, x1, r) & cc.lo_mask, funnel(x1, x2, r) & cc.hi_mask), e);
            cur0 = pk < cur0 ? pk : cur0;
        }
    }
    uint32_t key = 0xFFFFFFFFu, m = act ? (((uint32_t) len << 8) | (is_src ? CL_META_FROM : 0u)) : 0u;
    if (is_tgt) {
        uint32_t pmin = cur0;
        if (pmin == 0xFFFFFFFFu) {
            for (int k = 0; k < w; k++) { uint32_t h, pk; kmer_key(row, k, true, cc, h, pk); pmin = pk < pmin ? pk : pmin; }
        }
        uint32_t h, pk;
        kmer_key(row, (int) (pmin & 255u), true, cc, h, pk);
        key = tgt_sort_key(cluster_key(h, fs), pmin & 255u, fs);
        m = (pmin & 255u) | ((uint32_t) len << 8) | (is_src ? CL_META_FROM : 0u);
    }
    if (in) { keys[i] = key; if (vals) vals[i] = (uint32_t) i; meta[i] = m; }
    }
}

template <int EQ, bool UNIFORM>
__global__ void __launch_bounds__(256) k_tgt_gather(NodesDev nd, uint64_t count ,
                                                     const uint32_t *__restrict__ keys, const uint32_t *__restrict__ vals,
                                                     const uint32_t *__restrict__ meta, uint32_t uniform_meta, int fs, uint4 *__restrict__ store,
                                                     const unsigned long long *__restrict__ pile_cnt ) {
    if (pile_cnt && pile_cnt[1] * PILE_IRREGULAR_ONE_IN <= pile_cnt[0]) return;
    for (uint64_t t = (uint64_t) blockIdx.x * blockDim.x + threadIdx.x; t < count * EQ; t += (uint64_t) gridDim.x * blockDim.x) {
    const uint64_t j = t / EQ;
    const int c = (int) (t % EQ);
    const uint32_t key = keys[j];
    const uint32_t id = vals[j];
    const uint32_t *row = nd.words + (size_t) id * nd.stride;
    uint4 v;
    if ((nd.stride & 3) == 0 && 4 * c + 3 < nd.stride && ((uintptr_t) nd.words & 15u) == 0) v = reinterpret_cast<const uint4 *>(row)[c];
    else {
        v.x = 4 * c + 0 < nd.stride ? row[4 * c + 0] : 0u; v.y = 4 * c + 1 < nd.stride ? row[4 * c + 1] : 0u;
        v.z = 4 * c + 2 < nd.stride ? row[4 * c + 2] : 0u; v.w = 4 * c + 3 < nd.stride ? row[4 * c + 3] : 0u;
    }
    if (c == EQ - 1) {
        v.y = id; v.z = key;
        if (!UNIFORM) v.w = meta[id];
        else if (key != 0xFFFFFFFFu) v.w = uniform_meta | ((key >> fs) & ((1u << CL_MBITS) - 1u));
        else v.w = (uint32_t) nd.len[id] == (uniform_meta >> 8 & 0xFFFu) ? uniform_meta : 0u;
    }
    store[j * EQ + c] = v;
    }
}

constexpr int TD_TILE = 256, TD_HALO = 96;
__global__ void __launch_bounds__(TD_TILE) k_tgt_dir(const uint32_t *__restrict__ keys, uint64_t n, int shift, uint32_t n_buckets ,
                                                     uint32_t bucket_base , uint4 *__restrict__ dir,
                                                     unsigned long long *__restrict__ bad ,
                                                     const unsigned long long *__restrict__ pile_cnt ) {
    if (pile_cnt && pile_cnt_pure(pile_cnt)) return;
    __shared__ uint32_t sb[TD_TILE + TD_HALO + 1];
    const uint64_t base = (uint64_t) blockIdx.x * TD_TILE;
    const uint32_t nb3 = n_buckets << 3;
    auto tagged = [&](uint64_t k) -> uint32_t { if (k >= n) return nb3; const uint32_t x = keys[k]; return x == 0xFFFFFFFFu ? nb3 : (x >> (shift - 3)) - (bucket_base << 3); };
    for (int k = (int) threadIdx.x; k <= TD_TILE + TD_HALO; k += TD_TILE)
        sb[k] = (base == 0 && k == 0) ? 0xFFFFFFFFu : tagged(base + (uint64_t) k - 1u);
    __syncthreads();
    const int t = (int) threadIdx.x, lane = lane_id();
    const uint64_t j = base + (uint64_t) t;
    auto put = [&](int64_t b, const uint4 &rec) { dir[b] = rec; };
    auto tally = [](unsigned long long acc, uint32_t cls) { return acc + (0x0101010101010100ull << (8u * cls)); };
    if (j >= 1 && j < n && sb[t + 1] < sb[t]) atomicOr(bad, 1ull);
    const uint32_t b = sb[t + 1] >> 3;
    const bool start = j <= n && b != (sb[t] >> 3);
    if (start && b == n_buckets) put(b, make_uint4((uint32_t) j, 0u, 0u, 0u));
    const bool real = start && b != n_buckets;
    constexpr int TD_SHORT = 4;
    const bool is_short = real && (sb[t + 1 + TD_SHORT] >> 3) != b;
    if (is_short) {
        unsigned long long acc = 0ull;
        int u = 0;
#pragma unroll
        for (; u < TD_SHORT; u++) {
            const uint32_t x = sb[t + 1 + u];
            if ((x >> 3) != b) break;
            acc = tally(acc, x & 7u);
        }
        put(b, make_uint4((uint32_t) j, (uint32_t) u, (uint32_t) acc, (uint32_t) (acc >> 32)));
    }
    unsigned long long longs = __ballot(real && !is_short);
    const int g = lane >> 4, gl = lane & 15;
    while (longs != 0ull) {
        int lsel = 64;
#pragma unroll
        for (int q = 0; q < 4; q++) {
            const int l = longs ? __builtin_ctzll(longs) : 64;
            longs = longs ? (longs & (longs - 1ull)) : 0ull;
            lsel = g == q ? l : lsel;
        }
        const bool has = lsel < 64;
        const int t0 = (t & ~63) + (has ? lsel : 0);
        const uint32_t bb = bperm(b, has ? lsel : 0);
        unsigned long long acc = 0ull;
        bool open = has, past = false;
        for (int u = 0;; u += 16) {
            const int idx = t0 + 1 + u + gl;
            const bool staged = idx <= TD_TILE + TD_HALO;
            const uint32_t x = staged ? sb[idx] : 0xFFFFFFFFu;
            const bool inb = open && staged && (x >> 3) == bb;
            const unsigned long long c = inb ? ((0x0101010101010100ull << (8u * (x & 7u))) | 1ull) : 0ull;
            uint32_t lo = (uint32_t) c, hi = (uint32_t) (c >> 32);
            lo += (uint32_t) __builtin_amdgcn_update_dpp(0, (int) lo, 0x111, 0xF, 0xF, true); hi += (uint32_t) __builtin_amdgcn_update_dpp(0, (int) hi, 0x111, 0xF, 0xF, true);
            lo += (uint32_t) __builtin_amdgcn_update_dpp(0, (int) lo, 0x112, 0xF, 0xF, true); hi += (uint32_t) __builtin_amdgcn_update_dpp(0, (int) hi, 0x112, 0xF, 0xF, true);
            lo += (uint32_t) __builtin_amdgcn_update_dpp(0, (int) lo, 0x114, 0xF, 0xF, true); hi += (uint32_t) __builtin_amdgcn_update_dpp(0, (int) hi, 0x114, 0xF, 0xF, true);
            lo += (uint32_t) __builtin_amdgcn_update_dpp(0, (int) lo, 0x118, 0xF, 0xF, true); hi += (uint32_t) __builtin_amdgcn_update_dpp(0, (int) hi, 0x118, 0xF, 0xF, true);
            lo = bperm(lo, lane | 15); hi = bperm(hi, lane | 15);
            acc += ((unsigned long long) hi << 32) | lo;
            const uint32_t took = lo & 255u, cnt = (uint32_t) acc & 255u;
            if (open && took < 16u) { open = false; past = t0 + 1 + u + (int) took > TD_TILE + TD_HALO; }
            else if (open && cnt >= 240u) { open = false; past = true; }
            if (__ballot(open) == 0ull) break;
        }
        if (has && gl == 0) {
            const uint64_t j0 = base + (uint64_t) t0;
            uint64_t k = j0 + (uint64_t) ((uint32_t) acc & 255u);
            acc &= ~255ull;
            if (past) {
                for (; k < j0 + 256u; k++) {
                    const uint32_t x = tagged(k);
                    if ((x >> 3) != bb) break;
                    acc = tally(acc, x & 7u);
                }
                if (k >= j0 + 256u && (tagged(k) >> 3) == bb) {
                    uint64_t a = k, z = n;
                    while (z - a > 1) { const uint64_t mid = a + (z - a) / 2; if ((tagged(mid) >> 3) == bb) a = mid; else z = mid; }
                    k = z;
                }
            }
            const uint32_t c = (uint32_t) (k - j0);
            put(bb, make_uint4((uint32_t) j0, c, c <= 255u ? (uint32_t) acc : 0u, c <= 255u ? (uint32_t) (acc >> 32) : 0u));
        }
    }
}

#ifndef CL_OCC
#define CL_OCC 6
#endif

struct ByIdEntries {
    const uint32_t *skeys, *sids;
    uint32_t uniform_meta;
    const unsigned long long *pile_cnt;
    BucketIndex bx;
};
__device__ __forceinline__ void by_id_pair(const ByIdEntries &by, size_t ei, uint32_t n_nodes, uint32_t &key, uint32_t &id) {
    key = by.skeys[ei];
    id = min(by.sids[ei], n_nodes - 1u);
}
template <int EQ>
__device__ __forceinline__ void entry_by_id(const NodesDev &nd, uint32_t uniform_meta, int fs, uint32_t key, uint32_t id, uint32_t (&ew)[4 * EQ]) {
    static_assert(EQ == 3, "entries by id: rows of nine words");
    const uint32_t *row = nd.words + (size_t) id * nd.stride;
    if ((nd.stride & 3) == 0 && nd.stride >= 12 && ((uintptr_t) nd.words & 15u) == 0) {
        const uint4 v0 = reinterpret_cast<const uint4 *>(row)[0], v1 = reinterpret_cast<const uint4 *>(row)[1];
        ew[0] = v0.x; ew[1] = v0.y; ew[2] = v0.z; ew[3] = v0.w; ew[4] = v1.x; ew[5] = v1.y; ew[6] = v1.z; ew[7] = v1.w;
        ew[8] = row[8];
    } else {
#pragma unroll
        for (int k = 0; k < 9; k++) ew[k] = k < nd.stride ? row[k] : 0u;
    }
    ew[9] = id; ew[10] = key;
    ew[11] = key != 0xFFFFFFFFu ? (uniform_meta | ((key >> fs) & ((1u << CL_MBITS) - 1u))) : 0u;
}
template <bool STATS, int EQ, int KF, int SW = 1, bool BYID = false>
__global__ void __launch_bounds__(PROBE_WAVES * 64, SW == 1 && EQ <= 4 ? CL_OCC : 4)
k_probe_clustered(NodesDev nd, PrefSufCfg cfg, ClusterCfg cc, const uint4 *__restrict__ store, const uint4 *__restrict__ dir,
// ... 645 lines not shown
                    const int rho_j = lenj - (lenBs - dj), Lv = lenj - (d - dj);
                    const bool vok = ((mjj & ITEM_FROM) != 0u) & (Cj != id) & (dj < d) & (Lv >= Lbig) & (rho_j <= rho) & ((rho_j > 0) | ((int) Cj > Bs));
                    const uint4 m4 = sMask[min(max(2 * rho_j, 0), 128)];
                    const uint32_t df = ((oi.w[0] ^ oj.w[0]) & m4.x) | ((oi.w[1] ^ oj.w[1]) & m4.y) | ((oi.w[2] ^ oj.w[2]) & m4.z) | ((oi.w[3] ^ oj.w[3]) & m4.w);
                    return want & vok & (df == 0u);
                } else return want && via_ok<1>(Bs, lenBs, Lbig, Cj, mjj, oj, id, d, rho, oi);
            };
            bool removed = via_of(j, has_pred);
            const int reach = (cfg.Lcap - 1) - Lbig;
            uint64_t cand = 0ull;
            if (pass && has_pred && !removed) {
                cand = below & ~(1ull << (63 - __clzll((long long) below)));
                if (d - reach > 0) cand &= ~((1ull << (d - reach)) - 1ull);
            }
            while (__ballot(cand != 0ull) != 0ull) {
                const bool need = cand != 0ull;
                const int top = need ? 63 - __clzll((long long) cand) : 0;
                const int j2 = need ? (int) Tb[top] : lane;
                const bool r2 = via_of(j2, need);
                removed = removed | r2;
                cand = (need && !r2) ? cand & ~(1ull << top) : 0ull;
                n_tried2 += need ? 1 : 0;
            }
            const bool keep = pass && !removed;
            if (clash) atomicOr(stp, 1u);
            if (keep) atomicAdd(stp, 0x100u);
            wave_lds_fence();
            stv = *stp;
            if (keep && stv == 0x100u) {
                o.first[Bs - o.src_base] = ((unsigned long long) id << 32) | (uint32_t) d;
                o.deg[Bs - o.src_base] = 1u;
                st_rec++;
            }
            const uint32_t nst = stv >> 8;
            const bool seg_multi = ev && (stv & 255u) == 0u && nst >= 2u && nst <= max_stand;
            if (__ballot(seg_multi) != 0ull) {
                uint64_t segm = 0ull;
#pragma unroll
                for (int q = 0; q < 8; q++) { const uint64_t mq = __ballot(ev && s8 == q); segm = s8 == q ? mq : segm; }
                const uint64_t km = __ballot(keep) & segm;
                const int ds0 = lenBs - cfg.rsoemo + 1;
                const uint64_t lowm = ds0 <= 0 ? 0ull : (ds0 >= 64 ? ~0ull : ((1ull << ds0) - 1ull));
                const bool my_kept = pass && (d < ds0 || __popcll(below & ~lowm) < 3);
                bool fin_me = false;
                uint64_t kmr = seg_multi ? km : 0ull;
                for (int it = 0; it < LOCAL_SLOTS_MAX; it++) {
                    if (__ballot(kmr != 0ull) == 0ull) break;
                    const bool on = kmr != 0ull;
                    const int sl = on ? __builtin_ctzll(kmr) : lane;
                    kmr = on ? kmr & (kmr - 1ull) : 0ull;
                    const uint32_t Cs = bperm(id, sl);
                    const int dsl = (int) bperm((uint32_t) d, sl);
                    const bool ks = bperm(my_kept ? 1u : 0u, sl) != 0u;
                    const uint64_t supm = __ballot(on && my_kept && id == Cs && d < dsl) & segm;
                    if (on && lane == sl) fin_me = ks && supm == 0ull;
                }
                const uint64_t F = __ballot(fin_me) & segm;
                if (fin_me) {
                    const int r = __popcll(F & ((1ull << lane) - 1ull));
                    const unsigned long long mine = ((unsigned long long) id << 32) | (uint32_t) d;
                    if (r == 0) { o.first[Bs - o.src_base] = mine; o.deg[Bs - o.src_base] = (uint32_t) __popcll(F); }
                    else o.second[(size_t) (r - 1) * o.slot_stride + (size_t) (Bs - o.src_base)] = mine;
                    st_rec++;
                }
            }
        }
        if (STATS) {
            st_rounds++;
            const bool fin = ev && (stv & 255u) == 0u && (stv >> 8) <= max_stand;
            st_slots += fin; st_raw += fin && pass; st_cmp += (fin && has_pred ? 1 : 0) + (fin ? n_tried2 : 0);
        }
        if (gl == 0) {
            if (g >= cur && g < e) {
                const uint32_t sv = sStat[wave][4 * b0 + g];
                const bool ok = ((fl0 >> g) & 1u) != 0u && (sv & 255u) == 0u && (sv >> 8) <= max_stand;
                red = ok ? red | 1u : red & ~1u;
                if (STATS && ok) st_win += (uint64_t) ((int) sSrc[wave][4 * b0 + g].y - cfg.Lmin + 1);
            }
            if (4 + g >= cur && 4 + g < e) {
                const uint32_t sv = sStat[wave][4 * b1 + g];
                const bool ok = ((fl1 >> g) & 1u) != 0u && (sv & 255u) == 0u && (sv >> 8) <= max_stand;
                red = ok ? red | 2u : red & ~2u;
                if (STATS && ok) st_win += (uint64_t) ((int) sSrc[wave][4 * b1 + g].y - cfg.Lmin + 1);
            }
        }
        const uint32_t ninc = finish_runs(b2, nnr_eff, nrun, nrec);
        cur = e;
        if (rot) {
            n_seen += __popc(fl0 >> 4);
            defer_rows(gl == 0 && ((fl0 >> (4 + g)) & 1u) != 0u && (red & 1u) == 0u, (int) sSrc[wave][4 * b0 + g].x);
            uint32_t t4w, fl2;
            quad_plan(ninc, nnr, t4w, fl2);
            tw = (tw >> 32) | ((uint64_t) t4w << 32);
            fl0 = fl1; fl1 = fl2;
            red >>= 1;
            const int bt = b0; b0 = b1; b1 = b2; b2 = bt;
            pos0 = step <= src_end - pos0 ? pos0 + step : src_end;
            have0 = pos0 < src_end;
            cur -= 4;
            bail = n_seen >= 192 && 2 * n_deferred > n_seen;
        }
    }
    if (bail && have0) {
        defer_rows(gl == 0 && g < cur && ((fl0 >> (4 + g)) & 1u) != 0u && (red & 1u) == 0u, (int) sSrc[wave][4 * b0 + g].x);
        bool first = true;
        for (int q = pos0; q < src_end; q = step <= src_end - q ? q + step : src_end) {
            const int j = q + g < src_end ? q + g : last_src;
            const int b = BYKEY ? (int) reinterpret_cast<const uint32_t *>(store)[(size_t) j * (4 * EQ) + 4 * EQ - 3]
                                : (LIST ? (int) min((uint32_t) src_list[j], (uint32_t) nd.n - 1u) : j);
            const bool dfr = gl == 0 && q + g < src_end && !(first && g < cur) && (run_w[(size_t) b * (2 * CL_RMAX) + 1] >> 24) != 0u;
            defer_rows(dfr, b);
            first = false;
        }
    }
    flush_defer();
    st_rec = wave_sum_u64(st_rec);
    if (lane == 0 && st_rec) atomicAdd(&o.counters[CNT_VALID_RECORDS], (unsigned long long) st_rec);
    if (STATS) {
        st_raw = wave_sum_u64(st_raw); st_slots = wave_sum_u64(st_slots); st_win = wave_sum_u64(st_win); st_cmp = wave_sum_u64(st_cmp);
        if (lane == 0) {
            atomicAdd(&o.counters[CNT_RAW], (unsigned long long) st_raw);
            atomicAdd(&o.counters[CNT_SLOTS], (unsigned long long) st_slots);
            atomicAdd(&o.counters[CNT_WINDOWS], (unsigned long long) st_win);
            atomicAdd(&o.counters[CNT_TR_COMPARES], (unsigned long long) st_cmp);
            atomicAdd(&o.counters[CNT_ROUNDS], (unsigned long long) st_rounds);
        }
    }
}

bool cluster_plan(const PrefSufCfg &cfg, int max_len, uint64_t live, int bucket_log2_bias, ClusterCfg *c, int *eq) {
    const int W = blocks_of(max_len);
    int e = (W + 3 + 3) / 4;
    if (e < 2) e = 2;
    const int nwin = max_len - cfg.Lmin + 1;
    if (e > CL_MAX_EQ || nwin < 1 || nwin > 128) return false;
    int kk = std::min(32, std::max(cfg.Lmin - 63, std::min(cfg.Lmin, CL_KMIN)));
    const int nw_half = std::min(nwin, 64);
    if (nw_half > std::min(cfg.Lmin - kk + 1, 64)) kk = cfg.Lmin - nw_half + 1;
    if (kk < CL_KMIN_HARD || kk > 32 || kk > cfg.Lmin) return false;
    c->kk = kk;
    c->w = std::min(cfg.Lmin - kk + 1, 64);
    c->lo_mask = kk >= 16 ? 0xFFFFFFFFu : ((1u << (2 * kk)) - 1u);
    c->hi_mask = kk <= 16 ? 0u : (kk >= 32 ? 0xFFFFFFFFu : ((1u << (2 * kk - 32)) - 1u));
    int bits = 4;
    while (bits < 28 && (1ull << bits) < live) bits++;
    bits = std::max(4, std::min(32 - CL_MBITS, bits + bucket_log2_bias));
    c->n_buckets = 1u << bits;
    c->idx_shift = 32 - bits;
    *eq = e;
    return true;
}

size_t cluster_sort_temp_bytes(uint64_t n) { return sort_u32_pairs_temp_bytes(n); }

void launch_cluster_keys(const NodesDev &nd, const PrefSufCfg &cfg, const ClusterCfg &cc, int32_t node_begin, int32_t node_end, uint32_t *keys, uint32_t *vals,
                         uint32_t *meta, void *runs, uint8_t *nruns, hipStream_t s, bool with_runs, const unsigned long long *only_if_declined) {
    if (node_end <= node_begin) return;
    const uint64_t m = (uint64_t) (node_end - node_begin);
    const unsigned long long *gate = only_if_declined;
    const dim3 grid((unsigned) (gate ? std::min<uint64_t>((m + TK_ROWS - 1) / TK_ROWS, 8192) : (m + TK_ROWS - 1) / TK_ROWS)), block(TK_ROWS);
    const int32_t *nol = nullptr; const unsigned long long *noc = nullptr;
#define NR_LAUNCH(TKW, WIDE) do { if (with_runs) hipLaunchKernelGGL((k_node_runs<TKW, WIDE, true>), grid, block, 0, s, nd, cfg, cc, (int) node_begin, (int) node_end, keys, vals, meta, (uint2 *) runs, nruns, nol, noc, gate); \
                                  else hipLaunchKernelGGL((k_node_runs<TKW, WIDE, false>), grid, block, 0, s, nd, cfg, cc, (int) node_begin, (int) node_end, keys, vals, meta, (uint2 *) runs, nruns, nol, noc, gate); } while (0)
    if (blocks_of(cfg.Lcap - 1) > 13 || (cfg.Lcap - 1) - cfg.Lmin + 1 > 64) NR_LAUNCH(21, true);
    else if (blocks_of(cfg.Lcap - 1) <= 9) NR_LAUNCH(11, false);
    else NR_LAUNCH(17, false);
#undef NR_LAUNCH
}

void launch_cluster_runs_list(const NodesDev &nd, const PrefSufCfg &cfg, const ClusterCfg &cc, const int32_t *ids, const unsigned long long *count, uint32_t cap, uint32_t grid_blocks,
                              void *runs, uint8_t *nruns, hipStream_t s) {
    if (cap == 0 || nd.n <= 0) return;
    const dim3 grid(std::max<uint32_t>(1u, std::min<uint32_t>(grid_blocks, (cap + TK_ROWS - 1) / TK_ROWS))), block(TK_ROWS);
    uint32_t *nok = nullptr;
#define NR_LAUNCH(TKW, WIDE) hipLaunchKernelGGL((k_node_runs<TKW, WIDE, true>), grid, block, 0, s, nd, cfg, cc, 0, (int) cap, nok, nok, nok, (uint2 *) runs, nruns, ids, count, (const unsigned long long *) nullptr)
    if (blocks_of(cfg.Lcap - 1) > 13 || (cfg.Lcap - 1) - cfg.Lmin + 1 > 64) NR_LAUNCH(21, true);
    else if (blocks_of(cfg.Lcap - 1) <= 9) NR_LAUNCH(11, false);
    else NR_LAUNCH(17, false);
#undef NR_LAUNCH
}

__global__ void __launch_bounds__(256) k_iota(uint32_t *__restrict__ v, uint32_t n) {
    for (uint32_t i = blockIdx.x * 256u + threadIdx.x; i < n; i += gridDim.x * 256u) v[i] = i;
}

hipError_t launch_cluster_store(const NodesDev &nd, const ClusterCfg &cc, uint32_t *keys, uint32_t *vals, uint32_t *keys2, uint32_t *vals2,
                                void *sort_temp, size_t sort_temp_bytes, void *dir, bool fill_vals,
                                hipEvent_t ev_sorted, unsigned long long *bad_flag, bool test_skip_sort, hipStream_t s, bool own_sort) {
    const hipError_t err = launch_cluster_sort(nd, cc, keys, vals, keys2, vals2, sort_temp, sort_temp_bytes, fill_vals, ev_sorted, test_skip_sort, s, own_sort);
    return err != hipSuccess ? err : launch_cluster_dir(nd, cc, keys2, dir, bad_flag, nullptr, s);
}

hipError_t launch_cluster_sort(const NodesDev &nd, const ClusterCfg &cc, uint32_t *keys, uint32_t *vals, uint32_t *keys2, uint32_t *vals2, void *sort_temp, size_t sort_temp_bytes,
                               bool fill_vals, hipEvent_t ev_sorted, bool test_skip_sort, hipStream_t s, bool own_sort) {
    if (nd.n <= 0) return hipSuccess;
    const uint64_t n = (uint64_t) nd.n;
    if (fill_vals && (!own_sort || test_skip_sort)) hipLaunchKernelGGL(k_iota, dim3((unsigned) std::min<uint64_t>((n + 255) / 256, 8192)), dim3(256), 0, s, vals, (uint32_t) n);
    hipError_t err = hipSuccess;
    if (test_skip_sort) {
        err = hipMemcpyAsync(keys2, keys, n * sizeof(uint32_t), hipMemcpyDeviceToDevice, s);
        if (err == hipSuccess) err = hipMemcpyAsync(vals2, vals, n * sizeof(uint32_t), hipMemcpyDeviceToDevice, s);
    } else err = sort_u32_pairs(sort_temp, sort_temp_bytes, keys, keys2, own_sort ? (const uint32_t *) nullptr : vals, vals2, n, cc.idx_shift - 3, s, own_sort);
    if (err != hipSuccess) return err;
    if (ev_sorted) (void) hipEventRecord(ev_sorted, s);
    return hipSuccess;
}

constexpr int DF_UNROLL = 4;
__global__ void __launch_bounds__(256) k_dir_fill(uint4 *__restrict__ dir, uint64_t n_rec, const unsigned long long *__restrict__ pile_cnt) {
    if (pile_cnt && pile_cnt_pure(pile_cnt)) return;
    const uint4 z = make_uint4(0u, 0u, 0u, 0u);
    for (uint64_t p = (uint64_t) blockIdx.x * (256u * DF_UNROLL); p < n_rec; p += (uint64_t) gridDim.x * (256u * DF_UNROLL)) {
#pragma unroll
        for (int u = 0; u < DF_UNROLL; u++) {
            const uint64_t i = p + (uint64_t) u * 256u + threadIdx.x;
            if (i < n_rec) dir[i] = z;
        }
    }
}

hipError_t launch_cluster_dir(const NodesDev &nd, const ClusterCfg &cc, const uint32_t *keys2, void *dir, unsigned long long *bad_flag, const unsigned long long *only_if_no_pure_piles,
                              hipStream_t s) {
    if (nd.n <= 0) return hipSuccess;
    const uint64_t n = (uint64_t) nd.n, n_rec = (uint64_t) cc.n_buckets + 2;
    if (only_if_no_pure_piles)
        hipLaunchKernelGGL(k_dir_fill, dim3((unsigned) std::min<uint64_t>((n_rec + 256 * DF_UNROLL - 1) / (256 * DF_UNROLL), 1u << 17)), dim3(256), 0, s, (uint4 *) dir, n_rec,
                           only_if_no_pure_piles);
    else {
        const hipError_t err = hipMemsetAsync(dir, 0, n_rec * 16, s);
        if (err != hipSuccess) return err;
    }
    hipLaunchKernelGGL(k_tgt_dir, dim3((unsigned) ((n + 1 + TD_TILE - 1) / TD_TILE)), dim3(TD_TILE), 0, s, keys2, n, cc.idx_shift, cc.n_buckets, 0u, (uint4 *) dir, bad_flag, only_if_no_pure_piles);
    return hipGetLastError();
}

hipError_t launch_cluster_gather(const NodesDev &nd, const ClusterCfg &cc, int eq, const uint32_t *keys2, const uint32_t *vals2, const uint32_t *meta, int uniform_len,
                                 void *store, const unsigned long long *pile_cnt, hipStream_t s) {
    if (nd.n <= 0) return hipSuccess;
    const uint64_t n = (uint64_t) nd.n;
    const uint64_t pieces = n * (uint64_t) eq;
    const unsigned g = (unsigned) std::min<uint64_t>((pieces + 255) / 256, 1u << 16);
    const int fs = cc.idx_shift - CL_MBITS;
    const uint32_t um = uniform_len > 0 ? (((uint32_t) uniform_len << 8) | CL_META_FROM) : 0u;
#define TG_LAUNCH(E, U) hipLaunchKernelGGL((k_tgt_gather<E, U>), dim3(g), dim3(256), 0, s, nd, n, keys2, vals2, meta, um, fs, (uint4 *) store, pile_cnt)
#define TG_EQ(E) do { if (uniform_len > 0) TG_LAUNCH(E, true); else TG_LAUNCH(E, false); } while (0)
    if (eq == 2)      TG_EQ(2);
    else if (eq == 3) TG_EQ(3);
    else if (eq == 4) TG_EQ(4);
    else              TG_EQ(5);
#undef TG_EQ
#undef TG_LAUNCH
    return hipGetLastError();
}

hipError_t launch_cluster_store_slice(const NodesDev &nd, const ClusterCfg &cc, int eq, uint64_t m, uint32_t bucket_base, uint32_t n_buckets_local, uint32_t *keys,
                                      uint32_t *vals, uint32_t *keys2, uint32_t *vals2, const uint32_t *meta, int uniform_len, void *sort_temp, size_t sort_temp_bytes,
                                      void *store, void *dir, unsigned long long *bad_flag, hipStream_t s, bool own_sort) {
    hipError_t err = hipMemsetAsync(dir, 0, ((size_t) n_buckets_local + 2) * 16, s);
    if (err != hipSuccess || m == 0) return err;
    err = sort_u32_pairs(sort_temp, sort_temp_bytes, keys, keys2, vals, vals2, m, cc.idx_shift - 3, s, own_sort);
    if (err != hipSuccess) return err;
    const uint64_t n = m, pieces = m * (uint64_t) eq;
    const unsigned g = (unsigned) ((pieces + 255) / 256);
    const int fs = cc.idx_shift - CL_MBITS;
    const uint32_t um = uniform_len > 0 ? (((uint32_t) uniform_len << 8) | CL_META_FROM) : 0u;
#define TG_LAUNCH(E, U) hipLaunchKernelGGL((k_tgt_gather<E, U>), dim3(g), dim3(256), 0, s, nd, n, (const uint32_t *) keys2, (const uint32_t *) vals2, meta, um, fs, (uint4 *) store, (const unsigned long long *) nullptr)
#define TG_EQ(E) do { if (uniform_len > 0) TG_LAUNCH(E, true); else TG_LAUNCH(E, false); } while (0)
    if (eq == 2)      TG_EQ(2);
    else if (eq == 3) TG_EQ(3);
    else if (eq == 4) TG_EQ(4);
    else              TG_EQ(5);
#undef TG_EQ
#undef TG_LAUNCH
    hipLaunchKernelGGL(k_tgt_dir, dim3((unsigned) ((n + 1 + TD_TILE - 1) / TD_TILE)), dim3(TD_TILE), 0, s, (const uint32_t *) keys2, n, cc.idx_shift, n_buckets_local, bucket_base,
                       (uint4 *) dir, bad_flag, (const unsigned long long *) nullptr);
    return hipGetLastError();
}

uint64_t cluster_probe_blocks(int n_cu, uint64_t n_src) {
    return std::max<uint64_t>(1, std::min<uint64_t>((n_src + PROBE_WAVES - 1) / PROBE_WAVES, (uint64_t) std::max(1, n_cu) * CL_OCC));
}

uint64_t cluster_record_slack(int n_cu, uint64_t n_src) { return cluster_probe_blocks(n_cu, n_src) * PROBE_WAVES * (uint64_t) REC_CHUNK_LOCAL; }

void launch_probe_stream(const NodesDev &nd, const PrefSufCfg &cfg, const ClusterCfg &cc, int eq, const void *store, const void *dir,
                         const void *runs, const uint8_t *nruns, int32_t src_begin, int32_t src_end, bool by_key, unsigned long long *counters, int n_cu,
                         uint32_t *deg, unsigned long long *first, unsigned long long *second, int32_t *defer_list, uint32_t defer_cap,
                         const unsigned long long *pile_cnt, hipStream_t s, uint32_t slot_stride) {
    const int64_t ns = (int64_t) src_end - src_begin;
    if (ns <= 0) return;
    const uint64_t quads = ((uint64_t) ns + 3) / 4;
    const int kf = (2 * cfg.Lmin) >> 5;
    const int kfs = (eq == 3 && (kf == 5 || kf == 3)) || (eq == 2 && kf == 3) ? kf : 0;
    dim3 grid((unsigned) std::max<uint64_t>(1, std::min<uint64_t>((quads + PROBE_WAVES - 1) / PROBE_WAVES, (uint64_t) std::max(1, n_cu) * clq_occ(eq <= 3 ? eq : 4, kfs, by_key)))),
         block(PROBE_WAVES * 64);
    ProbeOut o{nullptr, nullptr, 0, counters, deg, first, by_key ? 0 : src_begin, second};
    o.slot_stride = slot_stride;
    const uint4 *st = (const uint4 *) store;
#define CLQ_LAUNCH(ST, E, K, BK) hipLaunchKernelGGL((k_probe_stream<ST, E, K, BK>), grid, block, 0, s, nd, cfg, cc, st, (const uint4 *) dir, (const uint2 *) runs, nruns, src_begin, src_end, o, defer_list, defer_cap, pile_cnt, \
                                                    (const int32_t *) nullptr, (const unsigned long long *) nullptr, ByIdEntries{nullptr, nullptr, 0u, nullptr, BucketIndex{nullptr, 0u}})
#define CLQ_ORDER(ST, E, K) do { if (by_key) CLQ_LAUNCH(ST, E, K, true); else CLQ_LAUNCH(ST, E, K, false); } while (0)
#define CLQ_STATS(E, K) do { if (cfg.stats) CLQ_ORDER(true, E, K); else CLQ_ORDER(false, E, K); } while (0)
    if (eq == 3 && kf == 5)      CLQ_STATS(3, 5);
    else if (eq == 3 && kf == 3) CLQ_STATS(3, 3);
    else if (eq == 2 && kf == 3) CLQ_STATS(2, 3);
    else if (eq == 2)            CLQ_STATS(2, 0);
    else if (eq == 3)            CLQ_STATS(3, 0);
    else                         CLQ_STATS(4, 0);
#undef CLQ_STATS
#undef CLQ_ORDER
#undef CLQ_LAUNCH
}

__global__ void __launch_bounds__(256) k_defer_swap(const unsigned long long *__restrict__ pile_cnt, unsigned long long *__restrict__ counters, const int32_t *__restrict__ list2,
                                                     int32_t *__restrict__ list, uint32_t cap, bool pure_too ) {
    if (!(pile_cnt_mixed(pile_cnt) || (pure_too && !pile_cnt_declines(pile_cnt)))) return;
    const uint64_t n2 = min(counters[CNT_DEFERRED2], (unsigned long long) cap);
    for (uint64_t i = (uint64_t) blockIdx.x * blockDim.x + threadIdx.x; i < n2; i += (uint64_t) gridDim.x * blockDim.x) list[i] = list2[i];
    if (blockIdx.x == 0 && threadIdx.x == 0) { counters[CNT_DEFERRED_PILE] = counters[CNT_DEFERRED]; counters[CNT_DEFERRED] = n2; }
}

bool launch_probe_stream_list(const NodesDev &nd, const PrefSufCfg &cfg, const ClusterCfg &cc, int eq, const void *store, const void *dir, const void *runs, const uint8_t *nruns,
                              int32_t *src_list, uint32_t list_cap, unsigned long long *counters, int n_cu, uint32_t *deg, unsigned long long *first,
                              unsigned long long *second, int32_t *defer2, const unsigned long long *pile_cnt, hipStream_t s, uint32_t slot_stride, int32_t src_base,
                              const uint32_t *skeys, const uint32_t *sids, int uniform_len, bool by_id, const void *tab, uint32_t epoch) {
    if (eq != 3 || list_cap == 0) return false;
    const int kf = (2 * cfg.Lmin) >> 5;
    const int kfs = (kf == 5 || kf == 3) ? kf : 0;
    const dim3 grid((unsigned) std::max(1, n_cu) * clq_occ(3, kfs, false)), block(PROBE_WAVES * 64);
    ProbeOut o{nullptr, nullptr, 0, counters, deg, first, src_base, second};
    o.slot_stride = slot_stride;
    const bool pure_too = by_id && skeys && sids && uniform_len > 0 && nd.n > 0;
    const ByIdEntries by{skeys, sids, uniform_len > 0 ? (((uint32_t) uniform_len << 8) | CL_META_FROM) : 0u, pile_cnt, BucketIndex{(const uint4 *) tab, epoch}};
#define CLQ_LIST(K, BI) hipLaunchKernelGGL((k_probe_stream<false, 3, K, false, true, BI>), grid, block, 0, s, nd, cfg, cc, (const uint4 *) store, (const uint4 *) dir, (const uint2 *) runs, nruns, 0, \
                                           (int32_t) std::min<uint32_t>(list_cap, 0x7FFFFFFFu), o, defer2, list_cap, pile_cnt, (const int32_t *) src_list, (const unsigned long long *) (counters + CNT_DEFERRED), by)
#define CLQ_BOTH(K) do { CLQ_LIST(K, false); if (pure_too) CLQ_LIST(K, true); } while (0)
    if (kf == 5) CLQ_BOTH(5); else if (kf == 3) CLQ_BOTH(3); else CLQ_BOTH(0);
#undef CLQ_BOTH
#undef CLQ_LIST
    hipLaunchKernelGGL(k_defer_swap, dim3(1024), dim3(256), 0, s, pile_cnt, counters, (const int32_t *) defer2, src_list, list_cap, pure_too);
    return pure_too;
}

void launch_probe_clustered(const NodesDev &nd, const PrefSufCfg &cfg, const ClusterCfg &cc, int eq, const void *store, const void *dir,
                            const void *runs, const uint8_t *nruns, int32_t src_begin, int32_t src_end, const int32_t *src_list, int32_t src_base,
                            uint32_t *rec_dst, unsigned long long *rec_val, uint64_t rec_cap,
                            unsigned long long *counters, int n_cu, uint32_t *deg, unsigned long long *first, const ProbeBig *big,
                            const unsigned long long *list_count, int sw , hipStream_t s,
                            const uint32_t *skeys, const uint32_t *sids, int uniform_len, const unsigned long long *pile_cnt, const void *tab, uint32_t epoch) {
    const int64_t ns = (int64_t) src_end - src_begin;
    if (ns <= 0) return;
    dim3 grid((unsigned) cluster_probe_blocks(n_cu, (uint64_t) ns)), block(PROBE_WAVES * 64);
    ProbeOut o{rec_dst, rec_val, rec_cap, counters, deg, first, src_base};
    if (big) { o.big_list = big->list; o.big_list_cap = big->list_cap; }
    const uint4 *st = (const uint4 *) store;
// ... 30 lines not shown
```

### alga_amd/csrc/prefsuf_cluster_device.h

```cpp
#pragma once
#include <hip/hip_runtime.h>
#include "prefsuf_common.h"
#include "../../include/alga_amd.h"
#include "prefsuf_device.h"

namespace alga {

__device__ __forceinline__ uint32_t kmer_hash(uint32_t lo, uint32_t hi) {
    return (lo ^ __funnelshift_l(hi, hi, 13) ^ (hi >> 7)) * 0x9E3779B1u;
}

__device__ __forceinline__ bool kmer_class0(uint32_t lo) { return (lo & 3u) == 0u && ((((lo >> 2) ^ (lo >> 3)) & 1u) != 0u); }
__device__ __forceinline__ uint32_t order_key0(uint32_t h, int pos) { return ((h >> 1) & 0x7FFFFF00u) | (uint32_t) pos; }
__device__ __forceinline__ uint32_t order_key(uint32_t h, uint32_t lo, int pos) { return order_key0(h, pos) | (kmer_class0(lo) ? 0u : 0x80000000u); }
__device__ __forceinline__ uint32_t class0_mask16(uint32_t cur, uint32_t nxt) {
    const uint32_t nx = __funnelshift_r(cur, nxt, 2);
    return ~(cur | (cur >> 1)) & (nx ^ (nx >> 1)) & 0x55555555u;
}
__device__ __forceinline__ uint32_t compress_even(uint32_t x) {
    x = (x | (x >> 1)) & 0x33333333u;
    x = (x | (x >> 2)) & 0x0F0F0F0Fu;
    x = (x | (x >> 4)) & 0x00FF00FFu;
    return (x | (x >> 8)) & 0x0000FFFFu;
}

__device__ __forceinline__ uint32_t cluster_key(uint32_t h, int fs) {
    uint32_t k = h * 0x9E3779B1u;
    k ^= k >> 15;
    k *= 0x85EBCA77u;
    k ^= k >> 13;
    k *= 0xC2B2AE3Du;
    return (k >> (fs + CL_MBITS)) == (0xFFFFFFFFu >> (fs + CL_MBITS)) ? k ^ 0x80000000u : k;
}

__device__ __forceinline__ uint32_t tgt_sort_key(uint32_t ckey, uint32_t m_c, int fs) {
    const uint32_t fm = ((1u << CL_MBITS) - 1u) << fs;
    return (ckey & ~fm) | ((m_c << fs) & fm);
}
__device__ __forceinline__ bool same_cluster(uint32_t entry_key, uint32_t ckey, int fs) {
    return ((entry_key ^ ckey) & ~(((1u << CL_MBITS) - 1u) << fs)) == 0u;
}

constexpr unsigned long long PILE_IRREGULAR_ONE_IN = ALGA_PILE_IRREGULAR_ONE_IN;
constexpr unsigned long long PILE_DECLINE_ONE_IN = ALGA_PILE_DECLINE_ONE_IN;
__device__ __forceinline__ bool pile_cnt_declines(const unsigned long long *c) { return c[1] * PILE_DECLINE_ONE_IN > c[0]; }
__device__ __forceinline__ bool pile_cnt_mixed(const unsigned long long *c) { return !pile_cnt_declines(c) && c[1] * PILE_IRREGULAR_ONE_IN > c[0]; }
__device__ __forceinline__ bool pile_cnt_pure(const unsigned long long *c) { return !pile_cnt_declines(c) && !pile_cnt_mixed(c); }
struct BucketIndex {
    const uint4 *tab;
    uint32_t epoch;
};
template <bool MAYBE_TAB>
__device__ __forceinline__ uint4 bucket_record(const uint4 *__restrict__ dir, const BucketIndex &bx, bool from_tab, uint32_t bucket) {
    if constexpr (!MAYBE_TAB) return dir[bucket];
    else {
        const uint4 *line = bx.tab + (size_t) bucket * 8;
        const uint4 *pr = from_tab ? line + 4 : dir + bucket;
        const uint32_t *pt = from_tab ? reinterpret_cast<const uint32_t *>(line + 3) + 3 : reinterpret_cast<const uint32_t *>(pr);
        const uint32_t *pf = from_tab ? reinterpret_cast<const uint32_t *>(line + 5) : reinterpret_cast<const uint32_t *>(pr);
        const uint4 r = *pr;
        const uint32_t tag = *pt, full = *pf;
        if (!from_tab) return r;
        const uint32_t n = r.x & 255u;
        const bool valid = (tag >> 23) == bx.epoch;
        return valid ? make_uint4(r.y, n == 127u ? full : n, r.z, r.w) : make_uint4(0u, 0u, 0u, 0u);
    }
}

__device__ __forceinline__ void run_slice(const uint4 &rec, uint32_t run_y, uint32_t &e0, uint32_t &cnt) {
    const int q = (int) (run_y & 255u), p0 = (int) ((run_y >> 8) & 255u), p1 = (int) ((run_y >> 16) & 255u);
    int mlo = q - p1 + 1, mhi = q - p0;
    mlo = mlo < 0 ? 0 : mlo; mhi = mhi > 63 ? 63 : mhi;
    e0 = rec.x; cnt = rec.y;
    if (mhi < mlo) { cnt = 0u; return; }
    if (rec.y > 255u) return;
    const int s0 = mlo >> 3, s1 = (mhi >> 3) + 1;
    const uint32_t b0 = ((s0 < 4 ? rec.z : rec.w) >> (8 * (s0 & 3))) & 255u;
    const uint32_t b1 = s1 >= 8 ? rec.y : (((s1 < 4 ? rec.z : rec.w) >> (8 * (s1 & 3))) & 255u);
    e0 = rec.x + b0; cnt = b1 - b0;
}

template <int RS = 1, int RW = 0>
__device__ __forceinline__ uint32_t row_word(const uint32_t *row, int k) {
    if (RW > 0) { const uint32_t v = row[(k < RW ? k : RW - 1) * RS]; return k < RW ? v : 0u; }
    return row[k * RS];
}

template <int RS = 1, int RW = 0>
__device__ __forceinline__ void kmer_key(const uint32_t *row, int i, bool valid, const ClusterCfg &cc, uint32_t &h, uint32_t &pk) {
    const int bit = 2 * i, q = bit >> 5, r = bit & 31;
    const uint32_t x0 = row_word<RS, RW>(row, q), x1 = row_word<RS, RW>(row, q + 1), x2 = row_word<RS, RW>(row, q + 2);
    const uint32_t lo = funnel(x0, x1, r) & cc.lo_mask;
    h = kmer_hash(lo, funnel(x1, x2, r) & cc.hi_mask);
    pk = valid ? order_key(h, lo, i) : 0xFFFFFFFFu;
}

constexpr int TK_ROWS = 128;
constexpr int NR_STACK = 8;

template <bool WIDE, int RCAP = CL_RMAX, int RS = 1, int RW = 0>
__device__ __forceinline__ void node_runs_core(const uint32_t *row, int nwin, bool act, const ClusterCfg &cc, uint32_t (*stk)[TK_ROWS], uint16_t (*rbuf)[TK_ROWS], int t,
                                               int &nr, bool &uncovered, bool &stack_ovf, uint32_t &cur0, int step = 64) {
    constexpr int S0 = NR_STACK + 1;
    const int w = cc.w;
    nr = 0; uncovered = false; stack_ovf = false; cur0 = 0xFFFFFFFFu;
    for (int hb = (WIDE && nwin > step) ? ((nwin - 1) / step) * step : 0; hb >= 0; hb -= step) {
        const int h0 = hb >> 4;
        auto rowh = [&](int k) -> uint32_t { return row_word<RS, RW>(row, h0 + k); };
        const int nwh = !WIDE ? nwin : (nwin - hb < step ? nwin - hb : step);
        const int nk = act ? nwh - 1 + w : 0;
        uint64_t m_lo, m_hi;
        {
            uint32_t dm[4];
#pragma unroll
            for (int d = 0; d < 4; d++) {
                const uint32_t x0 = rowh(2 * d), x1 = rowh(2 * d + 1), x2 = rowh(2 * d + 2);
                dm[d] = compress_even(class0_mask16(x0, x1)) | (compress_even(class0_mask16(x1, x2)) << 16);
            }
            m_lo = (uint64_t) dm[0] | ((uint64_t) dm[1] << 32);
            m_hi = (uint64_t) dm[2] | ((uint64_t) dm[3] << 32);
            m_lo &= nk >= 64 ? ~0ull : (nk <= 0 ? 0ull : ((1ull << nk) - 1ull));
            m_hi &= nk <= 64 ? 0ull : ((1ull << (nk - 64)) - 1ull);
        }
        uint64_t b0 = w >= 64 ? m_lo : (m_lo & ((1ull << w) - 1ull));
        uint64_t b1 = w >= 64 ? m_hi : ((m_lo >> w) | (m_hi << (64 - w)));
        auto key_at = [&](int pos) -> uint32_t {
            const int bit = 2 * pos, q = bit >> 5, r = bit & 31;
            const uint32_t x0 = rowh(q), x1 = rowh(q + 1), x2 = rowh(q + 2);
            return order_key0(kmer_hash(funnel(x0, x1, r) & cc.lo_mask, funnel(x1, x2, r) & cc.hi_mask), pos);
        };
        uint32_t cur1 = 0xFFFFFFFFu;
        int sp1 = 0;
        while (b1 != 0ull) {
            const int e = __builtin_ctzll(b1);
            b1 &= b1 - 1ull;
            const uint32_t pk = key_at(w + e);
            const bool push = pk < cur1;
            stk[(push && sp1 < NR_STACK) ? sp1 : NR_STACK][t] = pk;
            cur1 = push ? pk : cur1;
            sp1 += push ? 1 : 0;
        }
        uint32_t cur0h = 0xFFFFFFFFu;
        int sp0 = 0;
        while (b0 != 0ull) {
            const int e = 63 - __builtin_clzll(b0);
            b0 ^= 1ull << e;
            const uint32_t pk = key_at(e);
            const bool push = pk < cur0h;
            stk[S0 + ((push && sp0 < NR_STACK) ? sp0 : NR_STACK)][t] = pk;
            cur0h = push ? pk : cur0h;
            sp0 += push ? 1 : 0;
        }
        if (hb == 0) cur0 = cur0h;
        stack_ovf = stack_ovf || sp1 > NR_STACK || sp0 > NR_STACK;
        sp1 = sp1 > NR_STACK ? NR_STACK : sp1;
        sp0 = sp0 > NR_STACK ? NR_STACK : sp0;
        {
            const uint32_t hq = (uint32_t) hb | ((uint32_t) hb << 8);
            uint32_t top = sp1 > 0 ? stk[sp1 - 1][t] : 0xFFFFFFFFu;
            uint32_t nxt0 = stk[S0][t];
            uint32_t c0 = 0xFFFFFFFFu, win = top;
            int i0 = 0, p_hi = nwh - 1;
            int e0 = sp0 > 0 ? (int) (nxt0 & 255u) : -1;
            int e1 = sp1 > 0 ? (int) (top & 255u) - w : -1;
            while ((e0 > e1 ? e0 : e1) >= 0) {
                const int pe = e0 > e1 ? e0 : e1;
                const bool take0 = e0 >= e1;
                const int row_i = take0 ? S0 + i0 + 1 : (sp1 >= 2 ? sp1 - 2 : NR_STACK);
                const uint32_t v = stk[row_i][t];
                i0 += take0 ? 1 : 0;
                sp1 -= take0 ? 0 : 1;
                c0 = take0 ? nxt0 : c0;
                nxt0 = take0 ? v : nxt0;
                top = take0 ? top : (sp1 >= 1 ? v : 0xFFFFFFFFu);
                e0 = take0 ? (i0 < sp0 ? (int) (v & 255u) : -1) : e0;
                e1 = take0 ? e1 : (sp1 >= 1 ? (int) (v & 255u) - w : -1);
                const uint32_t wn = c0 < top ? c0 : top;
                const int pc = pe < p_hi ? pe : p_hi;
                const bool em = wn != win && pc < p_hi;
                rbuf[(em && nr < RCAP) ? nr : RCAP][t] = (uint16_t) (((win & 255u) | ((uint32_t) (pc + 1) << 8)) + hq);
                uncovered = uncovered || (em && win == 0xFFFFFFFFu);
                nr += em ? 1 : 0;
                p_hi = em ? pc : p_hi;
                win = wn;
            }
            if (act) {
                if (nr < RCAP) rbuf[nr][t] = (uint16_t) ((win & 255u) + hq);
                uncovered = uncovered || win == 0xFFFFFFFFu;
                nr++;
            }
        }
    }
}

__device__ __forceinline__ uint32_t bperm(uint32_t v, int src_lane) { return (uint32_t) __builtin_amdgcn_ds_bpermute(src_lane << 2, (int) v); }

}
```

### alga_amd/csrc/prefsuf_kernels.h

```cpp
#pragma once
#include <hip/hip_runtime.h>
#include <stddef.h>
#include <stdint.h>
#include "prefsuf_common.h"

namespace alga {

struct alga_edge_dev { int32_t src, dst, offset; };

void launch_restride(const uint32_t *in, int stride_in, uint32_t *out, int stride_out, uint64_t n, hipStream_t s);
void launch_widen_len(const void *in, int elem_bytes , int32_t *out, uint64_t n, hipStream_t s);
void launch_compact_edges(const alga_edge_dev *edges, int32_t n, uint64_t n_edges, uint8_t *deg, uint32_t *dst, uint8_t *off, unsigned long long *bad, hipStream_t s);
void launch_expand_twins(const uint32_t *in, int stride_in, const int32_t *len , uint32_t *out, int stride_out, uint64_t n_pairs, hipStream_t s);
void launch_node_stats(const NodesDev &nd, unsigned long long *counters, int *max_len , hipStream_t s);

uint32_t seed_buckets_for(uint64_t live_nodes, int fill_x10);
uint32_t seed_filter_bits_for(uint64_t live_nodes);
void launch_seed_build(const NodesDev &nd, const PrefSufCfg &cfg, unsigned long long *table, uint32_t n_buckets, uint32_t *filter,
                       uint32_t filter_bits, hipStream_t s);

struct ProbeBig { int32_t *list; uint32_t list_cap; uint32_t count; void *items; uint32_t item_cap; };
int    local_item_capacity();
int    local_big_limit();
size_t probe_big_bytes(int n_cu, uint32_t count, int local, uint32_t item_cap);

void launch_probe(const NodesDev &nd, const PrefSufCfg &cfg, const unsigned long long *table, uint32_t n_buckets,
                  const uint32_t *filter, uint32_t filter_bits, int32_t src_begin, int32_t src_end, uint32_t *rec_dst, unsigned long long *rec_val, uint64_t rec_cap,
                  unsigned long long *counters, int n_cu, int local , uint32_t *deg , unsigned long long *first ,
                  const ProbeBig *big , hipStream_t s);
uint64_t probe_record_slack(int n_cu, uint64_t n_src, bool local);
void launch_local_emit(int32_t src_base, int32_t n_src, const uint32_t *deg, const unsigned long long *first, const unsigned long long *second,
                       const uint32_t *rec_dst, const unsigned long long *rec_val, uint64_t n_rec, uint32_t *rowptr, uint32_t *cursor,
                       alga_edge_dev *edges, const int32_t *record_sources, const unsigned long long *record_sources_count, uint32_t record_sources_cap, hipStream_t s, uint32_t slot_stride = 0,
                       uint64_t *fused_scratch = nullptr, const unsigned long long *pile_cnt = nullptr);

bool       cluster_plan(const PrefSufCfg &cfg, int max_len, uint64_t live, int bucket_log2_bias, ClusterCfg *c, int *eq);
size_t     cluster_sort_temp_bytes(uint64_t n);
void       launch_cluster_keys(const NodesDev &nd, const PrefSufCfg &cfg, const ClusterCfg &cc, int32_t node_begin, int32_t node_end, uint32_t *keys,
                               uint32_t *vals, uint32_t *meta, void *runs, uint8_t *nruns, hipStream_t s, bool with_runs = true ,
                               const unsigned long long *only_if_declined = nullptr );
void       launch_cluster_runs_list(const NodesDev &nd, const PrefSufCfg &cfg, const ClusterCfg &cc, const int32_t *ids, const unsigned long long *count, uint32_t cap,
                                    uint32_t grid_blocks, void *runs, uint8_t *nruns, hipStream_t s);
hipError_t launch_cluster_store(const NodesDev &nd, const ClusterCfg &cc, uint32_t *keys, uint32_t *vals, uint32_t *keys2 , uint32_t *vals2, void *sort_temp,
                                size_t sort_temp_bytes, void *dir, bool fill_vals, hipEvent_t ev_sorted ,
                                unsigned long long *bad_flag ,
                                bool test_skip_sort , hipStream_t s, bool own_sort = true);
hipError_t launch_cluster_sort(const NodesDev &nd, const ClusterCfg &cc, uint32_t *keys, uint32_t *vals, uint32_t *keys2, uint32_t *vals2, void *sort_temp, size_t sort_temp_bytes,
                               bool fill_vals, hipEvent_t ev_sorted, bool test_skip_sort, hipStream_t s, bool own_sort = true);
hipError_t launch_cluster_dir(const NodesDev &nd, const ClusterCfg &cc, const uint32_t *keys2, void *dir, unsigned long long *bad_flag, const unsigned long long *only_if_no_pure_piles,
                              hipStream_t s);
hipError_t launch_cluster_gather(const NodesDev &nd, const ClusterCfg &cc, int eq, const uint32_t *keys2, const uint32_t *vals2, const uint32_t *meta,
                                 int uniform_len , void *store,
                                 const unsigned long long *pile_cnt , hipStream_t s);
uint64_t   cluster_record_slack(int n_cu, uint64_t n_src);
void       launch_probe_clustered(const NodesDev &nd, const PrefSufCfg &cfg, const ClusterCfg &cc, int eq, const void *store, const void *dir,
                                  const void *runs, const uint8_t *nruns, int32_t src_begin, int32_t src_end, const int32_t *src_list, int32_t src_base, uint32_t *rec_dst, unsigned long long *rec_val, uint64_t rec_cap,
                                  unsigned long long *counters, int n_cu, uint32_t *deg, unsigned long long *first, const ProbeBig *big,
                                  const unsigned long long *list_count ,
                                  int sw , hipStream_t s,
                                  const uint32_t *skeys = nullptr, const uint32_t *sids = nullptr, int uniform_len = 0,
                                  const unsigned long long *pile_cnt = nullptr ,
                                  const void *tab = nullptr , uint32_t epoch = 0);
void       launch_probe_stream(const NodesDev &nd, const PrefSufCfg &cfg, const ClusterCfg &cc, int eq, const void *store, const void *dir,
                               const void *runs, const uint8_t *nruns, int32_t src_begin, int32_t src_end, bool by_key ,
                               unsigned long long *counters, int n_cu, uint32_t *deg, unsigned long long *first, unsigned long long *second, int32_t *defer_list,
                               uint32_t defer_cap, const unsigned long long *pile_cnt ,
                               hipStream_t s, uint32_t slot_stride = 0 );
void       launch_pile_deg(int32_t n, unsigned long long *first, uint32_t *deg, const unsigned long long *pile_cnt, hipStream_t s);
bool       pile_plan(const PrefSufCfg &cfg, const ClusterCfg &cc, int eq, int uniform_len, bool masks);
size_t     pile_record_bytes(uint64_t n);
size_t     pile_table_bytes(uint32_t n_buckets);
void       launch_pile_sample(const NodesDev &nd, const ClusterCfg &cc, int uniform_len, const uint32_t *skeys , const uint32_t *sids , const void *dir,
                              unsigned long long *pile_cnt , int no_sample, hipStream_t s,
                              bool from_keys = false );
constexpr int PILE_CNT_WORDS = 6;
size_t     pile_own_mask_bytes(uint64_t n);
size_t     pile_list_bytes(uint64_t n);
void       launch_pile_build(const NodesDev &nd, const PrefSufCfg &cfg, const ClusterCfg &cc, int uniform_len, const uint32_t *skeys, const uint32_t *sids, const void *dir, void *rec,
                             void *rec2 , void *tab, uint32_t epoch, void *side, const void *runs, int nwin, const unsigned long long *pile_cnt,
                             uint32_t *own_mask ,
                             void *plist , hipStream_t s,
                             bool from_keys = false , unsigned long long *bad_flag = nullptr,
                             bool full_record = false ,
                             bool runs_ahead = false );
void       launch_pile_own_ids(const uint32_t *own_mask, const uint32_t *sids, uint64_t n_entries, int32_t *list, uint32_t cap, unsigned long long *pile_cnt, hipStream_t s);
void       launch_pile_check(const void *side, uint64_t n_entries, uint32_t n_buckets, const void *tab, const void *rec2, uint32_t epoch, const void *runs, int n_nodes, int nwin,
                             unsigned long long *pile_cnt, hipStream_t s);
bool       launch_probe_stream_list(const NodesDev &nd, const PrefSufCfg &cfg, const ClusterCfg &cc, int eq, const void *store, const void *dir, const void *runs, const uint8_t *nruns,
                                    int32_t *src_list, uint32_t list_cap, unsigned long long *counters, int n_cu, uint32_t *deg, unsigned long long *first,
                                    unsigned long long *second, int32_t *defer2, const unsigned long long *pile_cnt, hipStream_t s, uint32_t slot_stride = 0,
                                    int32_t src_base = 0 ,
                                    const uint32_t *skeys = nullptr, const uint32_t *sids = nullptr, int uniform_len = 0, bool by_id = false,
                                    const void *tab = nullptr , uint32_t epoch = 0);
void       launch_pile_probe(const NodesDev &nd, const PrefSufCfg &cfg, const ClusterCfg &cc, int uniform_len, const void *tab, uint32_t epoch, const void *rec, const void *rec2, const void *side,
                             const void *runs, unsigned long long *counters, uint32_t *deg, unsigned long long *first, unsigned long long *second, int32_t *defer_list,
                             uint32_t defer_cap, const unsigned long long *pile_cnt, int n_cu, hipStream_t s, int32_t src_begin, int32_t src_end,
                             void *side_range , unsigned long long *cursor ,
                             bool lean = true , bool tail = false );

size_t     rsort_u32_pairs_temp_bytes(uint64_t n);
void       rsort_set_variant(int v);
hipError_t rsort_u32_pairs(void *temp, size_t temp_bytes, const uint32_t *keys_in, uint32_t *keys_out, const uint32_t *vals_in, uint32_t *vals_out, uint64_t n,
                           int begin_bit, hipStream_t s);
size_t     sort_u32_pairs_temp_bytes(uint64_t n);
hipError_t sort_u32_pairs(void *temp, size_t temp_bytes, const uint32_t *keys_in, uint32_t *keys_out, const uint32_t *vals_in, uint32_t *vals_out,
                          uint64_t n, int begin_bit , hipStream_t s, bool own_sort = true );
size_t     rsort_u64_pairs_temp_bytes(uint64_t n);
hipError_t rsort_u64_pairs(void *temp, size_t temp_bytes, const unsigned long long *keys_in, unsigned long long *keys_out, const unsigned long long *vals_in,
                           unsigned long long *vals_out, uint64_t n, int bits, hipStream_t s);
hipError_t rsort_u32_u64(void *temp, size_t temp_bytes, const uint32_t *keys_in, uint32_t *keys_out, const unsigned long long *vals_in, unsigned long long *vals_out,
                         uint64_t n, int begin_bit, int end_bit, hipStream_t s);
size_t     sort_u64_pairs_temp_bytes(uint64_t n, int bits);
hipError_t sort_u64_pairs(void *temp, size_t temp_bytes, const unsigned long long *keys_in, unsigned long long *keys_out,
                          const unsigned long long *vals_in, unsigned long long *vals_out, uint64_t n, int bits, hipStream_t s);

void launch_make_keys(const uint32_t *rec_dst, uint64_t n_rec, int32_t dst_begin, int32_t dst_end, uint32_t *keys,
                      unsigned long long *n_valid, hipStream_t s);
size_t     sort_records_temp_bytes(uint64_t n, int bits);
hipError_t sort_records(void *temp, size_t temp_bytes, const uint32_t *keys_in, uint32_t *keys_out, const unsigned long long *vals_in,
                        unsigned long long *vals_out, uint64_t n, int bits, hipStream_t s);
void launch_rowptr_from_sorted(const uint32_t *keys, const unsigned long long *n_valid_ptr, uint64_t n_rec_max, int32_t n_owned,
                               uint32_t *rowptr, hipStream_t s);

size_t   scan_scratch_bytes(uint64_t n);
uint64_t scan_total_index(uint64_t n);
void launch_exclusive_scan(const uint32_t *in, uint64_t n, uint32_t *out, uint64_t *scratch, hipStream_t s);
void launch_exclusive_scan_pile_deg(uint32_t *deg, uint64_t n, uint32_t *out, uint64_t *scratch, unsigned long long *first, const unsigned long long *pile_cnt, hipStream_t s);
constexpr int MAIL_SEGS = 6;
struct MailSeg { const uint32_t *src; uint32_t words, dst; };
struct MailArgs {
    MailSeg seg[MAIL_SEGS];
    int n = 0;
    void add(const void *src, uint32_t words, uint32_t dst_word) { seg[n].src = (const uint32_t *) src; seg[n].words = words; seg[n].dst = dst_word; n++; }
};
void launch_mail(const MailArgs &a, uint32_t *host_block_dev, hipStream_t s);

int  reduce_targets_per_block(uint64_t n_records, uint64_t n_targets);
void launch_gather_heads(const NodesDev &nd, const unsigned long long *seg_val, const unsigned long long *n_valid_ptr, uint64_t n_rec_max,
                         void *heads , hipStream_t s);
void launch_reduce_targets(const NodesDev &nd, const PrefSufCfg &cfg, int32_t dst_begin, int32_t n_owned, int32_t targets_per_block,
                           const uint32_t *rowptr, unsigned long long *seg_val, const void *heads, uint32_t *out_cnt, uint32_t *outdeg,
                           unsigned long long *counters, hipStream_t s);
void launch_scatter_by_source(const PrefSufCfg &cfg, int32_t dst_begin, int32_t n_owned, const uint32_t *rowptr,
                              const unsigned long long *seg_val, const uint32_t *out_cnt, const uint32_t *out_rowptr, uint32_t *out_cursor,
                              alga_edge_dev *edges, hipStream_t s);
void launch_sort_rows(int32_t n, const uint32_t *out_rowptr, alga_edge_dev *edges, hipStream_t s);

void launch_edges_to_keys(const alga_edge_dev *e, uint64_t n, unsigned long long *keys, uint32_t *vals, hipStream_t s);
void launch_keys_to_edges(const unsigned long long *keys, const uint32_t *vals, uint64_t n, alga_edge_dev *e, hipStream_t s);
size_t     sort_edges_temp_bytes(uint64_t n);
hipError_t sort_edges(void *temp, size_t temp_bytes, const unsigned long long *keys_in, unsigned long long *keys_out, const uint32_t *vals_in,
                      uint32_t *vals_out, uint64_t n, int src_bits, hipStream_t s);

}
```

### alga_amd/csrc/radix_sort.hip

```cpp
#include <hip/hip_runtime.h>

#include <algorithm>
#include <cstdint>

#include "prefsuf_kernels.h"

namespace alga {

namespace {

constexpr int RS_THREADS = 512;
constexpr int RS_WAVES = RS_THREADS / 64;
constexpr int RS_IPT = 16;
constexpr int RS_TILE_MAX = 1024 * RS_IPT;
constexpr int RS_MAX_BITS = 10;
constexpr int RS_MAX_DIGITS = 1 << RS_MAX_BITS;
constexpr int RS_CHUNKS = 512;

struct RsPlan {
    int passes = 0;
    int bits[5] = {0, 0, 0, 0, 0}, shift[5] = {0, 0, 0, 0, 0};
    uint32_t n_tiles = 0, chunks = 0, tiles_per_chunk = 0;
    int tile = 8192;
};

int g_rs_variant = 0;

RsPlan rs_plan(uint64_t n, int begin_bit, int end_bit, int variant) {
    RsPlan p;
    p.tile = variant == 2 ? 4096 : (variant == 1 ? 16384 : 8192);
    const int RS_TILE = p.tile;
    const int total = end_bit - begin_bit;
    p.passes = (total + RS_MAX_BITS - 1) / RS_MAX_BITS;
    int at = begin_bit;
    for (int i = 0; i < p.passes; i++) {
        const int left = end_bit - at, todo = p.passes - i;
        p.bits[i] = (left + todo - 1) / todo;
        p.shift[i] = at;
        at += p.bits[i];
    }
    p.n_tiles = (uint32_t) ((n + RS_TILE - 1) / RS_TILE);
    p.chunks = std::max<uint32_t>(1, std::min<uint32_t>(RS_CHUNKS, p.n_tiles));
    p.tiles_per_chunk = (p.n_tiles + p.chunks - 1) / std::max<uint32_t>(1, p.chunks);
    p.chunks = p.tiles_per_chunk ? (p.n_tiles + p.tiles_per_chunk - 1) / p.tiles_per_chunk : 1;
    return p;
}

template <int TILE>
__global__ void __launch_bounds__(RS_THREADS) k_rs_hist(const uint32_t *__restrict__ keys, uint64_t n, int shift, int nbits, uint32_t n_tiles, uint32_t tiles_per_chunk,
                                                        uint32_t *__restrict__ tile_pref, uint32_t *__restrict__ chunk_tot, int aligned) {
    constexpr int Q = TILE / (4 * RS_THREADS);
    __shared__ uint32_t h[RS_MAX_DIGITS], run[RS_MAX_DIGITS];
    const uint32_t D = 1u << nbits, mask = D - 1u;
    const uint32_t c = blockIdx.x, t0 = c * tiles_per_chunk, t1 = min(t0 + tiles_per_chunk, n_tiles);
    for (uint32_t d = threadIdx.x; d < D; d += RS_THREADS) { run[d] = 0; h[d] = 0; }
    __syncthreads();
    uint4 k[Q], kn[Q];
    auto fetch = [&](uint32_t t, uint4 *dst) {
        const uint64_t base = (uint64_t) t * TILE;
        if (t < t1 && aligned && base + TILE <= n) {
            const uint4 *p = (const uint4 *) (keys + base);
#pragma unroll
            for (int j = 0; j < Q; j++) dst[j] = p[j * RS_THREADS + threadIdx.x];
        }
    };
    fetch(t0, k);
    for (uint32_t t = t0; t < t1; t++) {
        const uint64_t base = (uint64_t) t * TILE;
        fetch(t + 1, kn);
        if (aligned && base + TILE <= n) {
#pragma unroll
            for (int j = 0; j < Q; j++) {
                atomicAdd(&h[(k[j].x >> shift) & mask], 1u); atomicAdd(&h[(k[j].y >> shift) & mask], 1u);
                atomicAdd(&h[(k[j].z >> shift) & mask], 1u); atomicAdd(&h[(k[j].w >> shift) & mask], 1u);
            }
        } else {
#pragma unroll 4
            for (int j = 0; j < TILE / RS_THREADS; j++) {
                const uint64_t i = base + (uint64_t) j * RS_THREADS + threadIdx.x;
                if (i < n) atomicAdd(&h[(keys[i] >> shift) & mask], 1u);
            }
        }
        __syncthreads();
        for (uint32_t d = threadIdx.x; d < D; d += RS_THREADS) {
            const uint32_t x = h[d], r = run[d];
            tile_pref[(size_t) t * D + d] = r;
            run[d] = r + x;
            h[d] = 0;
        }
        __syncthreads();
#pragma unroll
        for (int j = 0; j < Q; j++) k[j] = kn[j];
    }
    for (uint32_t d = threadIdx.x; d < D; d += RS_THREADS) chunk_tot[(size_t) c * D + d] = run[d];
}

constexpr int RS_SC_DIGITS = 16, RS_SC_GROUPS = RS_THREADS / RS_SC_DIGITS;
__global__ void __launch_bounds__(RS_THREADS) k_rs_scan_chunks(uint32_t *__restrict__ chunk_tot, uint32_t chunks, int nbits, uint32_t *__restrict__ digit_tot) {
    __shared__ uint32_t gs[RS_SC_GROUPS][RS_SC_DIGITS];
    const uint32_t D = 1u << nbits;
    const uint32_t g = threadIdx.x / RS_SC_DIGITS, dl = threadIdx.x % RS_SC_DIGITS, d = blockIdx.x * RS_SC_DIGITS + dl;
    const uint32_t cpg = (chunks + RS_SC_GROUPS - 1) / RS_SC_GROUPS, c0 = min(g * cpg, chunks), c1 = min(c0 + cpg, chunks);
    uint32_t s = 0;
    if (d < D) for (uint32_t c = c0; c < c1; c++) s += chunk_tot[(size_t) c * D + d];
    gs[g][dl] = s;
    __syncthreads();
    uint32_t base = 0, total = 0;
#pragma unroll 8
    for (int q = 0; q < RS_SC_GROUPS; q++) { const uint32_t x = gs[q][dl]; base += (uint32_t) q < g ? x : 0u; total += x; }
    if (d < D) {
        for (uint32_t c = c0; c < c1; c++) { const uint32_t x = chunk_tot[(size_t) c * D + d]; chunk_tot[(size_t) c * D + d] = base; base += x; }
        if (g == 0) digit_tot[d] = total;
    }
}

__device__ inline uint32_t rs_wave_incl_scan(uint32_t x) {
#pragma unroll
    for (int o = 1; o < 64; o <<= 1) { const uint32_t y = __shfl_up(x, o, 64); if ((int) (threadIdx.x & 63u) >= o) x += y; }
    return x;
}

template <int WAVES>
__device__ inline uint32_t rs_block_excl_scan(uint32_t x, uint32_t *wsum) {
    const uint32_t incl = rs_wave_incl_scan(x);
    if ((threadIdx.x & 63u) == 63u) wsum[threadIdx.x >> 6] = incl;
    __syncthreads();
    uint32_t base = 0;
#pragma unroll
    for (int q = 0; q < WAVES; q++) base += (uint32_t) q < (threadIdx.x >> 6) ? wsum[q] : 0u;
    __syncthreads();
    return base + incl - x;
}

__global__ void __launch_bounds__(RS_THREADS) k_rs_scan_digits(const uint32_t *__restrict__ digit_tot, int nbits, uint32_t *__restrict__ digit_base) {
    __shared__ uint32_t wsum[RS_WAVES];
    const uint32_t D = 1u << nbits, d0 = 2u * threadIdx.x;
    const uint32_t a = d0 < D ? digit_tot[d0] : 0u, b = d0 + 1 < D ? digit_tot[d0 + 1] : 0u;
    const uint32_t ex = rs_block_excl_scan<RS_WAVES>(a + b, wsum);
    if (d0 < D) digit_base[d0] = ex;
    if (d0 + 1 < D) digit_base[d0 + 1] = ex + a;
}

template <int NB>
__device__ inline void rs_match(uint32_t d, uint32_t &plo, uint32_t &phi) {
    plo = 0xFFFFFFFFu; phi = 0xFFFFFFFFu;
#pragma unroll
    for (int b = 0; b < NB; b++) {
        const uint32_t x = (uint32_t) (((int32_t) (d << (31 - b))) >> 31);
        const unsigned long long m = __ballot(x != 0u);
        plo &= ~((uint32_t) m ^ x);
        phi &= ~((uint32_t) (m >> 32) ^ x);
    }
}

template <int NB, int THREADS, bool IOTA>
__global__ void __launch_bounds__(THREADS) k_rs_scatter(const uint32_t *__restrict__ kin, const uint32_t *__restrict__ vin, uint32_t *__restrict__ kout,
                                                           uint32_t *__restrict__ vout, uint64_t n, int shift, int nbits, uint32_t n_tiles, uint32_t tiles_per_chunk,
                                                           const uint32_t *__restrict__ tile_pref, const uint32_t *__restrict__ chunk_base,
                                                           const uint32_t *__restrict__ digit_base) {
    constexpr int DMAX = 1 << NB, WAVES = THREADS / 64, RS_TILE = THREADS * RS_IPT;
    __shared__ unsigned short cnt[WAVES][DMAX];
    __shared__ uint32_t goff[DMAX];
    __shared__ uint32_t stage[RS_TILE];
    __shared__ uint32_t wsum[WAVES];
    const uint32_t per = (n_tiles + 7u) >> 3;
    const uint32_t t = (blockIdx.x & 7u) * per + (blockIdx.x >> 3);
    if (t >= n_tiles) return;
    const uint32_t D = 1u << nbits, mask = D - 1u;
    const uint32_t w = threadIdx.x >> 6, lane = threadIdx.x & 63u;
    {
        uint32_t *z = (uint32_t *) &cnt[0][0];
        for (uint32_t i = threadIdx.x; i < WAVES * DMAX / 2; i += THREADS) z[i] = 0;
        const uint32_t c = t / tiles_per_chunk;
        for (uint32_t d = threadIdx.x; d < D; d += THREADS)
            goff[d] = tile_pref[(size_t) t * D + d] + chunk_base[(size_t) c * D + d] + digit_base[d];
    }
    const uint64_t tbase = (uint64_t) t * RS_TILE;
    const uint32_t nv = (uint32_t) min((uint64_t) RS_TILE, n - tbase);
    uint32_t k[RS_IPT], v[RS_IPT];
#pragma unroll
    for (int j = 0; j < RS_IPT; j++) {
        const uint32_t idx = w * (64u * RS_IPT) + (uint32_t) j * 64u + lane;
        const bool ok = idx < nv;
        k[j] = ok ? kin[tbase + idx] : 0xFFFFFFFFu;
        v[j] = !ok ? 0u : (IOTA ? (uint32_t) (tbase + idx) : vin[tbase + idx]);
    }
    __syncthreads();
    unsigned short pos[RS_IPT];
#pragma unroll
    for (int j = 0; j < RS_IPT; j++) {
        const uint32_t d = (k[j] >> shift) & mask;
        uint32_t plo, phi;
        rs_match<NB>(d, plo, phi);
        const uint32_t below = __builtin_amdgcn_mbcnt_hi(phi, __builtin_amdgcn_mbcnt_lo(plo, 0u));
        const uint32_t c0 = cnt[w][d];
        pos[j] = (unsigned short) (c0 + below);
        if (below == 0u) cnt[w][d] = (unsigned short) (c0 + (uint32_t) (__popc(plo) + __popc(phi)));
    }
    __syncthreads();
    {
        const uint32_t d0 = 2u * threadIdx.x;
        uint32_t a = 0, b = 0;
        if (d0 < D) {
#pragma unroll
            for (int q = 0; q < WAVES; q++) {
                uint32_t *pp = (uint32_t *) &cnt[q][d0];
                const uint32_t x = *pp;
                *pp = a | (b << 16);
                a += x & 0xFFFFu; b += x >> 16;
            }
        }
        const uint32_t ex = rs_block_excl_scan<WAVES>(a + b, wsum);
        if (d0 < D) {
#pragma unroll
            for (int q = 0; q < WAVES; q++) {
                uint32_t *pp = (uint32_t *) &cnt[q][d0];
                const uint32_t x = *pp;
                *pp = ((x & 0xFFFFu) + ex) | (((x >> 16) + ex + a) << 16);
            }
            goff[d0] -= ex;
            if (d0 + 1 < D) goff[d0 + 1] -= ex + a;
        }
    }
    __syncthreads();
#pragma unroll
    for (int j = 0; j < RS_IPT; j++) {
        const uint32_t d = (k[j] >> shift) & mask;
        pos[j] = (unsigned short) (pos[j] + cnt[w][d]);
        stage[pos[j]] = k[j];
    }
    __syncthreads();
    uint32_t ga[RS_IPT];
#pragma unroll
    for (int j = 0; j < RS_IPT; j++) {
        const uint32_t i = (uint32_t) j * THREADS + threadIdx.x;
        const uint32_t key = stage[i];
        ga[j] = goff[(key >> shift) & mask] + i;
        if (i < nv) kout[ga[j]] = key;
    }
    __syncthreads();
#pragma unroll
    for (int j = 0; j < RS_IPT; j++) stage[pos[j]] = v[j];
    __syncthreads();
#pragma unroll
    for (int j = 0; j < RS_IPT; j++) {
        const uint32_t i = (uint32_t) j * THREADS + threadIdx.x;
        if (i < nv) vout[ga[j]] = stage[i];
// ... 5 lines not shown

template <typename K>
__global__ void __launch_bounds__(RS_THREADS) k_rs_hist64(const K *__restrict__ keys, uint64_t n, int shift, int nbits, uint32_t n_tiles,
                                                          uint32_t tiles_per_chunk, uint32_t *__restrict__ tile_pref, uint32_t *__restrict__ chunk_tot) {
    __shared__ uint32_t h[RS_MAX_DIGITS], run[RS_MAX_DIGITS];
    const uint32_t D = 1u << nbits, mask = D - 1u;
    const uint32_t c = blockIdx.x, t0 = c * tiles_per_chunk, t1 = min(t0 + tiles_per_chunk, n_tiles);
    for (uint32_t d = threadIdx.x; d < D; d += RS_THREADS) { run[d] = 0; h[d] = 0; }
    __syncthreads();
    K k[RS_IPT64], kn[RS_IPT64];
    auto fetch = [&](uint32_t t, K *dst) {
        const uint64_t base = (uint64_t) t * RS_TILE64;
        if (t < t1 && base + RS_TILE64 <= n) {
#pragma unroll
            for (int j = 0; j < RS_IPT64; j++) dst[j] = keys[base + (uint64_t) j * RS_THREADS + threadIdx.x];
        }
    };
    fetch(t0, k);
    for (uint32_t t = t0; t < t1; t++) {
        const uint64_t base = (uint64_t) t * RS_TILE64;
        fetch(t + 1, kn);
        if (base + RS_TILE64 <= n) {
#pragma unroll
            for (int j = 0; j < RS_IPT64; j++) atomicAdd(&h[(uint32_t) (k[j] >> shift) & mask], 1u);
        } else {
            for (int j = 0; j < RS_IPT64; j++) {
                const uint64_t i = base + (uint64_t) j * RS_THREADS + threadIdx.x;
                if (i < n) atomicAdd(&h[(uint32_t) (keys[i] >> shift) & mask], 1u);
            }
        }
        __syncthreads();
        for (uint32_t d = threadIdx.x; d < D; d += RS_THREADS) {
            const uint32_t x = h[d], r = run[d];
            tile_pref[(size_t) t * D + d] = r;
            run[d] = r + x;
            h[d] = 0;
        }
        __syncthreads();
#pragma unroll
        for (int j = 0; j < RS_IPT64; j++) k[j] = kn[j];
    }
    for (uint32_t d = threadIdx.x; d < D; d += RS_THREADS) chunk_tot[(size_t) c * D + d] = run[d];
}

template <typename K, int NB>
__global__ void __launch_bounds__(RS_THREADS) k_rs_scatter64(const K *__restrict__ kin, const unsigned long long *__restrict__ vin,
                                                             K *__restrict__ kout, unsigned long long *__restrict__ vout, uint64_t n, int shift,
                                                             int nbits, uint32_t n_tiles, uint32_t tiles_per_chunk, const uint32_t *__restrict__ tile_pref,
                                                             const uint32_t *__restrict__ chunk_base, const uint32_t *__restrict__ digit_base) {
    constexpr int DMAX = 1 << NB, WAVES = RS_THREADS / 64;
    __shared__ unsigned short cnt[WAVES][DMAX];
    __shared__ uint32_t goff[DMAX];
    __shared__ unsigned long long stage[RS_TILE64];
    __shared__ uint32_t wsum[WAVES];
    const uint32_t per = (n_tiles + 7u) >> 3;
    const uint32_t t = (blockIdx.x & 7u) * per + (blockIdx.x >> 3);
    if (t >= n_tiles) return;
    const uint32_t D = 1u << nbits, mask = D - 1u;
    const uint32_t w = threadIdx.x >> 6, lane = threadIdx.x & 63u;
    {
        uint32_t *z = (uint32_t *) &cnt[0][0];
        for (uint32_t i = threadIdx.x; i < WAVES * DMAX / 2; i += RS_THREADS) z[i] = 0;
        const uint32_t c = t / tiles_per_chunk;
        for (uint32_t d = threadIdx.x; d < D; d += RS_THREADS)
            goff[d] = tile_pref[(size_t) t * D + d] + chunk_base[(size_t) c * D + d] + digit_base[d];
    }
    const uint64_t tbase = (uint64_t) t * RS_TILE64;
    const uint32_t nv = (uint32_t) min((uint64_t) RS_TILE64, n - tbase);
    K k[RS_IPT64];
    unsigned long long v[RS_IPT64];
#pragma unroll
    for (int j = 0; j < RS_IPT64; j++) {
        const uint32_t idx = w * (64u * RS_IPT64) + (uint32_t) j * 64u + lane;
        const bool ok = idx < nv;
        k[j] = ok ? kin[tbase + idx] : (K) ~(K) 0;
        v[j] = ok ? vin[tbase + idx] : 0ull;
    }
    __syncthreads();
    unsigned short pos[RS_IPT64];
#pragma unroll
    for (int j = 0; j < RS_IPT64; j++) {
        const uint32_t d = (uint32_t) (k[j] >> shift) & mask;
        uint32_t plo, phi;
        rs_match<NB>(d, plo, phi);
        const uint32_t below = __builtin_amdgcn_mbcnt_hi(phi, __builtin_amdgcn_mbcnt_lo(plo, 0u));
        const uint32_t c0 = cnt[w][d];
        pos[j] = (unsigned short) (c0 + below);
        if (below == 0u) cnt[w][d] = (unsigned short) (c0 + (uint32_t) (__popc(plo) + __popc(phi)));
    }
    __syncthreads();
    {
        const uint32_t d0 = 2u * threadIdx.x;
        uint32_t a = 0, b = 0;
        if (d0 < D) {
#pragma unroll
            for (int q = 0; q < WAVES; q++) {
                uint32_t *pp = (uint32_t *) &cnt[q][d0];
                const uint32_t x = *pp;
                *pp = a | (b << 16);
                a += x & 0xFFFFu; b += x >> 16;
            }
        }
        const uint32_t ex = rs_block_excl_scan<WAVES>(a + b, wsum);
        if (d0 < D) {
#pragma unroll
            for (int q = 0; q < WAVES; q++) {
                uint32_t *pp = (uint32_t *) &cnt[q][d0];
                const uint32_t x = *pp;
                *pp = ((x & 0xFFFFu) + ex) | (((x >> 16) + ex + a) << 16);
            }
            goff[d0] -= ex;
            if (d0 + 1 < D) goff[d0 + 1] -= ex + a;
        }
    }
    __syncthreads();
#pragma unroll
    for (int j = 0; j < RS_IPT64; j++) {
        const uint32_t d = (uint32_t) (k[j] >> shift) & mask;
        pos[j] = (unsigned short) (pos[j] + cnt[w][d]);
        stage[pos[j]] = (unsigned long long) k[j];
    }
    __syncthreads();
    uint32_t ga[RS_IPT64];
#pragma unroll
    for (int j = 0; j < RS_IPT64; j++) {
        const uint32_t i = (uint32_t) j * RS_THREADS + threadIdx.x;
        const K key = (K) stage[i];
        ga[j] = goff[(uint32_t) (key >> shift) & mask] + i;
        if (i < nv) kout[ga[j]] = key;
    }
    __syncthreads();
#pragma unroll
    for (int j = 0; j < RS_IPT64; j++) stage[pos[j]] = v[j];
    __syncthreads();
#pragma unroll
    for (int j = 0; j < RS_IPT64; j++) {
        const uint32_t i = (uint32_t) j * RS_THREADS + threadIdx.x;
        if (i < nv) vout[ga[j]] = stage[i];
    }
}

size_t rs_align(size_t x) { return (x + 255) & ~(size_t) 255; }

}

size_t rsort_u32_pairs_temp_bytes(uint64_t n) {
    const RsPlan p = rs_plan(n, 0, 32, 0);
    return 2 * rs_align((size_t) (n + 4) * 4) + rs_align((size_t) p.n_tiles * RS_MAX_DIGITS * 4) + rs_align((size_t) RS_CHUNKS * RS_MAX_DIGITS * 4) +
           2 * rs_align(RS_MAX_DIGITS * 4);
}

void rsort_set_variant(int v) { if (v == 0 || v == 1) g_rs_variant = v; }

hipError_t rsort_u32_pairs(void *temp, size_t temp_bytes, const uint32_t *keys_in, uint32_t *keys_out, const uint32_t *vals_in, uint32_t *vals_out, uint64_t n,
                           int begin_bit, hipStream_t s) {
    if (n == 0) return hipSuccess;
    if (begin_bit < 0 || begin_bit > 31 || n >= (1ull << 32) - RS_TILE_MAX) return hipErrorInvalidValue;
    if (temp_bytes < rsort_u32_pairs_temp_bytes(n)) return hipErrorInvalidValue;
    const int variant = g_rs_variant;
    const RsPlan p = rs_plan(n, begin_bit, 32, variant);
    char *at = (char *) temp;
    uint32_t *tk = (uint32_t *) at; at += rs_align((size_t) (n + 4) * 4);
    uint32_t *tv = (uint32_t *) at; at += rs_align((size_t) (n + 4) * 4);
    uint32_t *tile_pref = (uint32_t *) at; at += rs_align((size_t) rs_plan(n, 0, 32, 0).n_tiles * RS_MAX_DIGITS * 4);
    uint32_t *chunk_tot = (uint32_t *) at; at += rs_align((size_t) RS_CHUNKS * RS_MAX_DIGITS * 4);
    uint32_t *digit_tot = (uint32_t *) at; at += rs_align(RS_MAX_DIGITS * 4);
    uint32_t *digit_base = (uint32_t *) at;
    const uint32_t *ki = keys_in, *vi = vals_in;
    for (int i = 0; i < p.passes; i++) {
        const bool to_out = ((p.passes - 1 - i) & 1) == 0;
        uint32_t *ko = to_out ? keys_out : tk, *vo = to_out ? vals_out : tv;
        const int nb = p.bits[i], sh = p.shift[i];
        const int aligned = (int) ((((uintptr_t) ki) & 15u) == 0);
        if (p.tile == 8192)
            hipLaunchKernelGGL((k_rs_hist<8192>), dim3(p.chunks), dim3(RS_THREADS), 0, s, ki, n, sh, nb, p.n_tiles, p.tiles_per_chunk, tile_pref, chunk_tot, aligned);
        else
            hipLaunchKernelGGL((k_rs_hist<16384>), dim3(p.chunks), dim3(RS_THREADS), 0, s, ki, n, sh, nb, p.n_tiles, p.tiles_per_chunk, tile_pref, chunk_tot, aligned);
        hipLaunchKernelGGL(k_rs_scan_chunks, dim3(((1u << nb) + RS_SC_DIGITS - 1u) / RS_SC_DIGITS), dim3(RS_THREADS), 0, s, chunk_tot, p.chunks, nb, digit_tot);
        hipLaunchKernelGGL(k_rs_scan_digits, dim3(1), dim3(RS_THREADS), 0, s, (const uint32_t *) digit_tot, nb, digit_base);
        const dim3 grid(8u * ((p.n_tiles + 7u) / 8u));
#define RS_SCATTER_(NB_, T_, I_) hipLaunchKernelGGL((k_rs_scatter<NB_, T_, I_>), grid, dim3(T_), 0, s, ki, vi, ko, vo, n, sh, nb, p.n_tiles, p.tiles_per_chunk, \
                                                   (const uint32_t *) tile_pref, (const uint32_t *) chunk_tot, (const uint32_t *) digit_base)
#define RS_SCATTER(NB_, T_) do { if (vi) RS_SCATTER_(NB_, T_, false); else RS_SCATTER_(NB_, T_, true); } while (0)
        if (p.tile == 8192) { if (nb <= 8) RS_SCATTER(8, 512); else RS_SCATTER(10, 512); }
        else                { if (nb <= 8) RS_SCATTER(8, 1024); else RS_SCATTER(10, 1024); }
#undef RS_SCATTER_
#undef RS_SCATTER
        ki = ko; vi = vo;
    }
    return hipGetLastError();
}

size_t rsort_u64_pairs_temp_bytes(uint64_t n) {
    const RsPlan p = rs_plan(n, 0, 32, 2);
    return 2 * rs_align((size_t) (n + 4) * 8) + rs_align((size_t) p.n_tiles * RS_MAX_DIGITS * 4) + rs_align((size_t) RS_CHUNKS * RS_MAX_DIGITS * 4) +
           2 * rs_align(RS_MAX_DIGITS * 4);
}

hipError_t rsort_u64_pairs(void *temp, size_t temp_bytes, const unsigned long long *keys_in, unsigned long long *keys_out, const unsigned long long *vals_in,
                           unsigned long long *vals_out, uint64_t n, int bits, hipStream_t s) {
    if (n == 0) return hipSuccess;
    if (bits < 1 || bits > 50 || n >= (1ull << 32) - RS_TILE_MAX) return hipErrorInvalidValue;
    if (temp_bytes < rsort_u64_pairs_temp_bytes(n)) return hipErrorInvalidValue;
    const RsPlan p = rs_plan(n, 0, bits, 2);
    char *at = (char *) temp;
    unsigned long long *tk = (unsigned long long *) at; at += rs_align((size_t) (n + 4) * 8);
    unsigned long long *tv = (unsigned long long *) at; at += rs_align((size_t) (n + 4) * 8);
    uint32_t *tile_pref = (uint32_t *) at; at += rs_align((size_t) p.n_tiles * RS_MAX_DIGITS * 4);
    uint32_t *chunk_tot = (uint32_t *) at; at += rs_align((size_t) RS_CHUNKS * RS_MAX_DIGITS * 4);
    uint32_t *digit_tot = (uint32_t *) at; at += rs_align(RS_MAX_DIGITS * 4);
    uint32_t *digit_base = (uint32_t *) at;
    const unsigned long long *ki = keys_in, *vi = vals_in;
    for (int i = 0; i < p.passes; i++) {
        const bool to_out = ((p.passes - 1 - i) & 1) == 0;
        unsigned long long *ko = to_out ? keys_out : tk, *vo = to_out ? vals_out : tv;
        const int nb = p.bits[i], sh = p.shift[i];
        hipLaunchKernelGGL((k_rs_hist64<unsigned long long>), dim3(p.chunks), dim3(RS_THREADS), 0, s, ki, n, sh, nb, p.n_tiles, p.tiles_per_chunk, tile_pref, chunk_tot);
        hipLaunchKernelGGL(k_rs_scan_chunks, dim3(((1u << nb) + RS_SC_DIGITS - 1u) / RS_SC_DIGITS), dim3(RS_THREADS), 0, s, chunk_tot, p.chunks, nb, digit_tot);
        hipLaunchKernelGGL(k_rs_scan_digits, dim3(1), dim3(RS_THREADS), 0, s, (const uint32_t *) digit_tot, nb, digit_base);
        const dim3 grid(8u * ((p.n_tiles + 7u) / 8u));
        if (nb <= 8) hipLaunchKernelGGL((k_rs_scatter64<unsigned long long, 8>), grid, dim3(RS_THREADS), 0, s, ki, vi, ko, vo, n, sh, nb, p.n_tiles, p.tiles_per_chunk,
                                        (const uint32_t *) tile_pref, (const uint32_t *) chunk_tot, (const uint32_t *) digit_base);
        else hipLaunchKernelGGL((k_rs_scatter64<unsigned long long, 10>), grid, dim3(RS_THREADS), 0, s, ki, vi, ko, vo, n, sh, nb, p.n_tiles, p.tiles_per_chunk,
                                (const uint32_t *) tile_pref, (const uint32_t *) chunk_tot, (const uint32_t *) digit_base);
        ki = ko; vi = vo;
    }
    return hipGetLastError();
}

hipError_t rsort_u32_u64(void *temp, size_t temp_bytes, const uint32_t *keys_in, uint32_t *keys_out, const unsigned long long *vals_in, unsigned long long *vals_out,
                         uint64_t n, int begin_bit, int end_bit, hipStream_t s) {
    if (n == 0) return hipSuccess;
    if (begin_bit < 0 || end_bit > 32 || end_bit <= begin_bit || n >= (1ull << 32) - RS_TILE_MAX) return hipErrorInvalidValue;
    if (temp_bytes < rsort_u64_pairs_temp_bytes(n)) return hipErrorInvalidValue;
    const RsPlan p = rs_plan(n, begin_bit, end_bit, 2);
    char *at = (char *) temp;
    uint32_t *tk = (uint32_t *) at; at += rs_align((size_t) (n + 4) * 8);
    unsigned long long *tv = (unsigned long long *) at; at += rs_align((size_t) (n + 4) * 8);
    uint32_t *tile_pref = (uint32_t *) at; at += rs_align((size_t) p.n_tiles * RS_MAX_DIGITS * 4);
    uint32_t *chunk_tot = (uint32_t *) at; at += rs_align((size_t) RS_CHUNKS * RS_MAX_DIGITS * 4);
    uint32_t *digit_tot = (uint32_t *) at; at += rs_align(RS_MAX_DIGITS * 4);
    uint32_t *digit_base = (uint32_t *) at;
    const uint32_t *ki = keys_in;
    const unsigned long long *vi = vals_in;
    for (int i = 0; i < p.passes; i++) {
        const bool to_out = ((p.passes - 1 - i) & 1) == 0;
        uint32_t *ko = to_out ? keys_out : tk;
        unsigned long long *vo = to_out ? vals_out : tv;
        const int nb = p.bits[i], sh = p.shift[i];
        hipLaunchKernelGGL((k_rs_hist64<uint32_t>), dim3(p.chunks), dim3(RS_THREADS), 0, s, ki, n, sh, nb, p.n_tiles, p.tiles_per_chunk, tile_pref, chunk_tot);
        hipLaunchKernelGGL(k_rs_scan_chunks, dim3(((1u << nb) + RS_SC_DIGITS - 1u) / RS_SC_DIGITS), dim3(RS_THREADS), 0, s, chunk_tot, p.chunks, nb, digit_tot);
        hipLaunchKernelGGL(k_rs_scan_digits, dim3(1), dim3(RS_THREADS), 0, s, (const uint32_t *) digit_tot, nb, digit_base);
        const dim3 grid(8u * ((p.n_tiles + 7u) / 8u));
        if (nb <= 8) hipLaunchKernelGGL((k_rs_scatter64<uint32_t, 8>), grid, dim3(RS_THREADS), 0, s, ki, vi, ko, vo, n, sh, nb, p.n_tiles, p.tiles_per_chunk,
                                        (const uint32_t *) tile_pref, (const uint32_t *) chunk_tot, (const uint32_t *) digit_base);
        else hipLaunchKernelGGL((k_rs_scatter64<uint32_t, 10>), grid, dim3(RS_THREADS), 0, s, ki, vi, ko, vo, n, sh, nb, p.n_tiles, p.tiles_per_chunk,
                                (const uint32_t *) tile_pref, (const uint32_t *) chunk_tot, (const uint32_t *) digit_base);
        ki = ko; vi = vo;
    }
    return hipGetLastError();
}

}
```

### alga_amd/csrc/sort_records.hip

```cpp
#include <algorithm>
#include <cstring>
#include <hip/hip_runtime.h>
#include <rocprim/rocprim.hpp>

#include "prefsuf_kernels.h"
#include "pkb_kernels.h"
#include "ingest_kernels.h"
#include "prefsuf_shard.h"

namespace alga {

size_t sort_records_temp_bytes(uint64_t n, int bits) {
    size_t bytes = 0;
    (void) rocprim::radix_sort_pairs(nullptr, bytes, (const uint32_t *) nullptr, (uint32_t *) nullptr,
                                     (const unsigned long long *) nullptr, (unsigned long long *) nullptr, (size_t) n, 0u,
                                     (unsigned) bits, (hipStream_t) 0);
    return bytes;
}

hipError_t sort_records(void *temp, size_t temp_bytes, const uint32_t *keys_in, uint32_t *keys_out, const unsigned long long *vals_in,
                        unsigned long long *vals_out, uint64_t n, int bits, hipStream_t s) {
    if (n == 0) return hipSuccess;
    return rocprim::radix_sort_pairs(temp, temp_bytes, keys_in, keys_out, vals_in, vals_out, (size_t) n, 0u, (unsigned) bits, s);
}

size_t sort_edges_temp_bytes(uint64_t n) {
    size_t bytes = 0;
    (void) rocprim::radix_sort_pairs(nullptr, bytes, (const unsigned long long *) nullptr, (unsigned long long *) nullptr,
                                     (const uint32_t *) nullptr, (uint32_t *) nullptr, (size_t) n, 0u, 64u, (hipStream_t) 0);
    return bytes;
}

hipError_t sort_edges(void *temp, size_t temp_bytes, const unsigned long long *keys_in, unsigned long long *keys_out, const uint32_t *vals_in,
                      uint32_t *vals_out, uint64_t n, int src_bits, hipStream_t s) {
    if (n == 0) return hipSuccess;
    return rocprim::radix_sort_pairs(temp, temp_bytes, keys_in, keys_out, vals_in, vals_out, (size_t) n, 0u, (unsigned) (32 + src_bits), s);
}

size_t sort_u64_pairs_temp_bytes(uint64_t n, int bits) {
    size_t bytes = 0;
    (void) rocprim::radix_sort_pairs(nullptr, bytes, (const unsigned long long *) nullptr, (unsigned long long *) nullptr,
                                     (const unsigned long long *) nullptr, (unsigned long long *) nullptr, (size_t) n, 0u, (unsigned) bits,
                                     (hipStream_t) 0);
    return bytes;
}

hipError_t sort_u64_pairs(void *temp, size_t temp_bytes, const unsigned long long *keys_in, unsigned long long *keys_out,
                          const unsigned long long *vals_in, unsigned long long *vals_out, uint64_t n, int bits, hipStream_t s) {
    if (n == 0) return hipSuccess;
    return rocprim::radix_sort_pairs(temp, temp_bytes, keys_in, keys_out, vals_in, vals_out, (size_t) n, 0u, (unsigned) bits, s);
}

using Sort10 = rocprim::radix_sort_config<rocprim::default_config, rocprim::default_config,
                                          rocprim::radix_sort_onesweep_config<rocprim::kernel_config<1024, 16>, rocprim::kernel_config<1024, 16>, 10,
                                                                              rocprim::block_radix_rank_algorithm::match>>;
static bool sort_u32_three_wide_passes(int begin_bit) { const int bits = 32 - begin_bit; return bits > 24 && bits <= 30; }

size_t sort_u32_pairs_temp_bytes(uint64_t n) {
    size_t a = 0, b = 0;
    (void) rocprim::radix_sort_pairs(nullptr, a, (const uint32_t *) nullptr, (uint32_t *) nullptr, (const uint32_t *) nullptr,
                                     (uint32_t *) nullptr, (size_t) n, 0u, 32u, (hipStream_t) 0);
    (void) rocprim::radix_sort_pairs<Sort10>(nullptr, b, (const uint32_t *) nullptr, (uint32_t *) nullptr, (const uint32_t *) nullptr,
                                             (uint32_t *) nullptr, (size_t) n, 2u, 32u, (hipStream_t) 0);
    const size_t own = rsort_u32_pairs_temp_bytes(n);
    return std::max(own, a > b ? a : b);
}

hipError_t sort_u32_pairs(void *temp, size_t temp_bytes, const uint32_t *keys_in, uint32_t *keys_out, const uint32_t *vals_in, uint32_t *vals_out,
                          uint64_t n, int begin_bit, hipStream_t s, bool own_sort) {
    if (n == 0) return hipSuccess;
    if (begin_bit < 0 || begin_bit > 31) return hipErrorInvalidValue;
    if (own_sort) return rsort_u32_pairs(temp, temp_bytes, keys_in, keys_out, vals_in, vals_out, n, begin_bit, s);
    if (n < (1ull << 22)) begin_bit = 0;
    if (sort_u32_three_wide_passes(begin_bit))
        return rocprim::radix_sort_pairs<Sort10>(temp, temp_bytes, keys_in, keys_out, vals_in, vals_out, (size_t) n, (unsigned) begin_bit, 32u, s);
    return rocprim::radix_sort_pairs(temp, temp_bytes, keys_in, keys_out, vals_in, vals_out, (size_t) n, (unsigned) begin_bit, 32u, s);
}

size_t sort_desc_temp_bytes(uint64_t n) { return std::max(sort_records_temp_bytes(n, 32), rsort_u64_pairs_temp_bytes(n)); }
hipError_t sort_desc(void *temp, size_t temp_bytes, const uint32_t *keys_in, uint32_t *keys_out, const unsigned long long *vals_in, unsigned long long *vals_out, uint64_t n,
                     int begin_bit, int end_bit, hipStream_t s, bool own_sort) {
    if (n == 0) return hipSuccess;
    if (begin_bit < 0 || end_bit > 32 || end_bit <= begin_bit) { begin_bit = 0; end_bit = 32; }
    if (own_sort) return rsort_u32_u64(temp, temp_bytes, keys_in, keys_out, vals_in, vals_out, n, begin_bit, end_bit, s);
    if (n < (1ull << 22)) { begin_bit = 0; end_bit = 32; }
    return rocprim::radix_sort_pairs(temp, temp_bytes, keys_in, keys_out, vals_in, vals_out, (size_t) n, (unsigned) begin_bit, (unsigned) end_bit, s);
}

size_t sort_u64_keys_temp_bytes(uint64_t n) {
    size_t bytes = 0;
    (void) rocprim::radix_sort_keys(nullptr, bytes, (const unsigned long long *) nullptr, (unsigned long long *) nullptr, (size_t) n, 0u, 64u,
                                    (hipStream_t) 0);
    return bytes;
}

hipError_t sort_u64_keys(void *temp, size_t temp_bytes, const unsigned long long *keys_in, unsigned long long *keys_out, uint64_t n, hipStream_t s) {
    if (n == 0) return hipSuccess;
    return rocprim::radix_sort_keys(temp, temp_bytes, keys_in, keys_out, (size_t) n, 0u, 64u, s);
}

hipError_t sort_u32_pairs_bits(void *temp, size_t temp_bytes, const uint32_t *keys_in, uint32_t *keys_out, const uint32_t *vals_in, uint32_t *vals_out,
                               uint64_t n, int bits, hipStream_t s) {
    if (n == 0) return hipSuccess;
    return rocprim::radix_sort_pairs(temp, temp_bytes, keys_in, keys_out, vals_in, vals_out, (size_t) n, 0u, (unsigned) bits, s);
}

hipError_t sort_u64_keys_bits(void *temp, size_t temp_bytes, const unsigned long long *keys_in, unsigned long long *keys_out, uint64_t n, int bits,
                              hipStream_t s) {
    if (n == 0) return hipSuccess;
    return rocprim::radix_sort_keys(temp, temp_bytes, keys_in, keys_out, (size_t) n, 0u, (unsigned) bits, s);
}

struct EdgePairEq { __device__ bool operator()(unsigned long long a, unsigned long long b) const { return (a >> 9) == (b >> 9); } };

size_t merge_u64_temp_bytes(uint64_t na, uint64_t nb) {
    size_t bytes = 0;
    (void) rocprim::merge(nullptr, bytes, (const unsigned long long *) nullptr, (const unsigned long long *) nullptr, (unsigned long long *) nullptr,
                          (size_t) na, (size_t) nb, rocprim::less<unsigned long long>(), (hipStream_t) 0);
    return bytes;
}

hipError_t merge_u64(void *temp, size_t temp_bytes, const unsigned long long *a, uint64_t na, const unsigned long long *b, uint64_t nb,
                     unsigned long long *out, hipStream_t s) {
    if (na + nb == 0) return hipSuccess;
    return rocprim::merge(temp, temp_bytes, a, b, out, (size_t) na, (size_t) nb, rocprim::less<unsigned long long>(), s);
}

size_t unique_edge_keys_temp_bytes(uint64_t n) {
    size_t bytes = 0;
    (void) rocprim::unique(nullptr, bytes, (const unsigned long long *) nullptr, (unsigned long long *) nullptr, (unsigned long long *) nullptr, (size_t) n,
                           EdgePairEq(), (hipStream_t) 0);
    return bytes;
}

hipError_t unique_edge_keys(void *temp, size_t temp_bytes, const unsigned long long *in, unsigned long long *out, unsigned long long *d_count, uint64_t n,
                            hipStream_t s) {
    return rocprim::unique(temp, temp_bytes, in, out, d_count, (size_t) n, EdgePairEq(), s);
}

size_t sort_u64_u32_temp_bytes(uint64_t n) { return sort_edges_temp_bytes(n); }
hipError_t sort_u64_u32(void *temp, size_t temp_bytes, const unsigned long long *keys_in, unsigned long long *keys_out, const uint32_t *vals_in,
                        uint32_t *vals_out, uint64_t n, int bits, hipStream_t s) {
    if (n == 0) return hipSuccess;
    return rocprim::radix_sort_pairs(temp, temp_bytes, keys_in, keys_out, vals_in, vals_out, (size_t) n, 0u, (unsigned) bits, s);
}

}
```

Measured before the change: 5.594 billion edges/s.

## Fuse first radix-sort pass histogram into cluster key generation kernel

After: 5.509 billion edges/s. 0.985x the previous value.

```diff
diff --git a/alga_amd/csrc/engine.hip b/alga_amd/csrc/engine.hip
--- a/alga_amd/csrc/engine.hip
+++ b/alga_amd/csrc/engine.hip
@@ -175,14 +175,19 @@
             keys_only = pile && e->pile_keys_only;
         } else {
             int32_t run_begin = 0, run_end = nd.n;
+            bool first_counts_ready = false;
+            uint32_t *key_meta = pp.uniform_len > 0 ? nullptr : (uint32_t *) e->cl_meta.p;
             if (pp.keys_shared == 1) {
                 if (e->keyed_n != nd.n || e->keyed_words != (const void *) nd.words || src_begin < e->keyed_begin || src_end > e->keyed_end)
                     return alga_fail(e, ALGA_ERR_INVALID_ARGUMENT, "keys_shared: alga_prefsuf_keys_device has not been called on this node set for a range that covers the sources");
                 run_begin = e->keyed_begin; run_end = e->keyed_end;
             } else {
                 keys_only = pile && e->opt_pile_runs != 0 && !e->expect_pairwise && !e->opt_pile_check;
-                launch_cluster_keys(nd, cfg, cc, 0, nd.n, (uint32_t *) e->cl_keys[0].p, need_vals ? (uint32_t *) e->cl_vals[0].p : nullptr, (uint32_t *) e->cl_meta.p, e->cl_runs.p,
-                                    (uint8_t *) e->cl_nruns.p, s, !keys_only);
+                RsFirstPass fp;
+                const bool count_here = e->opt_keys_hist != 0 && e->opt_own_sort != 0 && !e->opt_test_unsorted_index &&
+                                        rsort_u32_first_pass(e->sort_temp.p, cluster_sort_temp_bytes((uint64_t) nd.n), (uint64_t) nd.n, cluster_sort_begin_bit(cc), &fp);
+                first_counts_ready = launch_cluster_keys(nd, cfg, cc, 0, nd.n, (uint32_t *) e->cl_keys[0].p, need_vals ? (uint32_t *) e->cl_vals[0].p : nullptr, key_meta, e->cl_runs.p,
+                                                         (uint8_t *) e->cl_nruns.p, s, !keys_only, nullptr, count_here ? &fp : nullptr);
                 if ((rc = alga_check_launch(e, "k_node_runs"))) return rc;
             }
             HIP_TRY(e, hipEventRecord(e->ev[EV_KEYS], s));
@@ -190,7 +195,7 @@
             e->store_n = -1;
             HIP_TRY(e, launch_cluster_sort(nd, cc, (uint32_t *) e->cl_keys[0].p, (uint32_t *) e->cl_vals[0].p, (uint32_t *) e->cl_keys[1].p,
                                            (uint32_t *) e->cl_vals[1].p, e->sort_temp.p, cluster_sort_temp_bytes((uint64_t) nd.n), pp.keys_shared == 1 || !need_vals,
-                                           e->ev[EV_SORT], e->opt_test_unsorted_index != 0, s, e->opt_own_sort != 0));
+                                           e->ev[EV_SORT], e->opt_test_unsorted_index != 0, s, e->opt_own_sort != 0, first_counts_ready));
             const bool dir_late = pile && e->opt_pile_dir >= 1;
             e->dir_late = dir_late;
             if (!dir_late) {
@@ -209,7 +214,7 @@
                     pile = false;
                     rc = ALGA_OK;
                     if (keys_only) {
-                        launch_cluster_keys(nd, cfg, cc, 0, nd.n, (uint32_t *) e->cl_keys[0].p, (uint32_t *) e->cl_vals[0].p, (uint32_t *) e->cl_meta.p, e->cl_runs.p,
+                        launch_cluster_keys(nd, cfg, cc, 0, nd.n, (uint32_t *) e->cl_keys[0].p, (uint32_t *) e->cl_vals[0].p, key_meta, e->cl_runs.p,
                                             (uint8_t *) e->cl_nruns.p, s, true);
                         if ((rc = alga_check_launch(e, "k_node_runs"))) return rc;
                         keys_only = false;
@@ -248,7 +253,7 @@
                                         (unsigned long long *) e->cl_pile_cnt.p, s);
                     launch_cluster_runs_list(nd, cfg, cc, (const int32_t *) e->cl_defer.p, (const unsigned long long *) e->cl_pile_cnt.p + 3, (uint32_t) nd.n, (uint32_t) e->n_cu * 16u,
                                              e->cl_runs.p, (uint8_t *) e->cl_nruns.p, s);
-                    launch_cluster_keys(nd, cfg, cc, 0, nd.n, (uint32_t *) e->cl_keys[0].p, (uint32_t *) e->cl_vals[0].p, (uint32_t *) e->cl_meta.p, e->cl_runs.p,
+                    launch_cluster_keys(nd, cfg, cc, 0, nd.n, (uint32_t *) e->cl_keys[0].p, (uint32_t *) e->cl_vals[0].p, key_meta, e->cl_runs.p,
                                         (uint8_t *) e->cl_nruns.p, s, true, (const unsigned long long *) e->cl_pile_cnt.p);
                     if ((rc = alga_check_launch(e, "k_node_runs (own lists)"))) return rc;
                 }
@@ -685,6 +690,8 @@
         e->opt_pile_range = value != 0;
     } else if (!strcmp(name, "pkb_legacy")) {
         e->opt_pkb_legacy = (int) value;
+    } else if (!strcmp(name, "keys_hist")) {
+        e->opt_keys_hist = value != 0;
     } else if (!strcmp(name, "own_sort")) {
         e->opt_own_sort = value != 0;
     } else if (!strcmp(name, "test_presort_oom")) {
diff --git a/alga_amd/csrc/engine_internal.h b/alga_amd/csrc/engine_internal.h
--- a/alga_amd/csrc/engine_internal.h
+++ b/alga_amd/csrc/engine_internal.h
@@ -66,6 +66,7 @@
     int    opt_pile_probe_lean = 1;
     int    opt_pile_probe_tail = 1;
     int    opt_pile_runs_ahead = 0;
+    int    opt_keys_hist = 1;
     bool   pile_deg_pending = false;
     int    opt_pile_check = 0;
     bool   expect_pairwise = false;
diff --git a/alga_amd/csrc/prefsuf_cluster.hip b/alga_amd/csrc/prefsuf_cluster.hip
--- a/alga_amd/csrc/prefsuf_cluster.hip
+++ b/alga_amd/csrc/prefsuf_cluster.hip
@@ -8,21 +8,31 @@
 namespace alga {
 
 
-template <int TKW, bool WIDE, bool RUNS>
+template <int TKW, bool WIDE, bool RUNS, bool TILED = false>
 __global__ void __launch_bounds__(TK_ROWS) k_node_runs(NodesDev nd, PrefSufCfg cfg, ClusterCfg cc, int node_begin, int node_end,
                                                         uint32_t *__restrict__ keys, uint32_t *__restrict__ vals, uint32_t *__restrict__ meta,
                                                         uint2 *__restrict__ runs, uint8_t *__restrict__ nruns, const int32_t *__restrict__ id_list, const unsigned long long *__restrict__ id_count,
-                                                        const unsigned long long *__restrict__ only_if_declined ) {
-    if (only_if_declined && !pile_cnt_declines(only_if_declined)) return;
+                                                        const unsigned long long *__restrict__ only_if_declined ,
+                                                        KeyTileCounts tc ) {
+    if (!TILED && only_if_declined && !pile_cnt_declines(only_if_declined)) return;
+    if (TILED) { node_begin = 0; node_end = nd.n; nd.from = nullptr; nd.to = nullptr; vals = nullptr; meta = nullptr; }
+    __shared__ uint32_t tcnt[TILED ? KT_MAX_DIGITS / 2 : 1];
+    constexpr bool tiled = TILED;
     __shared__ uint32_t s[TK_ROWS][TKW];
     __shared__ uint32_t stk[RUNS ? 2 * (NR_STACK + 1) : 1][TK_ROWS];
     __shared__ uint16_t rbuf[RUNS ? CL_RMAX + 1 : 1][TK_ROWS];
+    if (TILED) id_list = nullptr;
     const int list_n = id_list ? (int) min((unsigned long long) (node_end - node_begin), *id_count) : 0;
-    __shared__ int sid[TK_ROWS];
-    for (int blk = (int) blockIdx.x; id_list ? blk * TK_ROWS < list_n : node_begin + blk * TK_ROWS < node_end; blk += (int) gridDim.x) {
+    __shared__ int sid[TILED ? 1 : TK_ROWS];
+    const int n_chunks = (int) (((int64_t) (id_list ? list_n : node_end - node_begin) + TK_ROWS - 1) / TK_ROWS);
+    constexpr int cpt = TILED ? KT_TILE / TK_ROWS : 1;
+    const int blk0 = (int) blockIdx.x * cpt;
+    int in_tile = 0;
+    if (tiled) for (int d = (int) threadIdx.x; d < KT_MAX_DIGITS / 2; d += TK_ROWS) tcnt[d] = 0u;
+    for (int blk = blk0; blk < n_chunks; blk += tiled ? 1 : (int) gridDim.x) {
     const int base = node_begin + blk * TK_ROWS;
     const int nrows = id_list ? min(TK_ROWS, list_n - blk * TK_ROWS) : min(TK_ROWS, node_end - base);
-    if (blk != (int) blockIdx.x) __syncthreads();
+    if (blk != blk0) __syncthreads();
     if (id_list) {
         if ((int) threadIdx.x < nrows) sid[threadIdx.x] = min(max(id_list[blk * TK_ROWS + (int) threadIdx.x], 0), nd.n - 1);
         __syncthreads();
@@ -105,7 +115,21 @@
         key = tgt_sort_key(cluster_key(h, fs), pmin & 255u, fs);
         m = (pmin & 255u) | ((uint32_t) len << 8) | (is_src ? CL_META_FROM : 0u);
     }
-    if (in) { keys[i] = key; if (vals) vals[i] = (uint32_t) i; meta[i] = m; }
+    if (in) { keys[i] = key; if (vals) vals[i] = (uint32_t) i; if (meta) meta[i] = m; }
+    if (tiled) {
+        if (in) { const uint32_t d = (key >> tc.shift) & ((1u << tc.nbits) - 1u); atomicAdd(&tcnt[d >> 1], 1u << ((d & 1u) << 4)); }
+        if (++in_tile == cpt || blk + 1 >= n_chunks) {
+            __syncthreads();
+            const size_t row0 = (size_t) (blk / cpt) << tc.nbits;
+#pragma unroll 1
+            for (int d = (int) threadIdx.x; d < (1 << tc.nbits); d += TK_ROWS) tc.counts[row0 + d] = (tcnt[d >> 1] >> ((d & 1) << 4)) & 0xFFFFu;
+            __syncthreads();
+#pragma unroll 1
+            for (int d = (int) threadIdx.x; d < KT_MAX_DIGITS / 2; d += TK_ROWS) tcnt[d] = 0u;
+            in_tile = 0;
+            blk += ((int) gridDim.x - 1) * cpt;
+        }
+    }
     }
 }
 
@@ -1057,20 +1081,30 @@
 }
 
 size_t cluster_sort_temp_bytes(uint64_t n) { return sort_u32_pairs_temp_bytes(n); }
-
-void launch_cluster_keys(const NodesDev &nd, const PrefSufCfg &cfg, const ClusterCfg &cc, int32_t node_begin, int32_t node_end, uint32_t *keys, uint32_t *vals,
-                         uint32_t *meta, void *runs, uint8_t *nruns, hipStream_t s, bool with_runs, const unsigned long long *only_if_declined) {
-    if (node_end <= node_begin) return;
+int cluster_sort_begin_bit(const ClusterCfg &cc) { return cc.idx_shift - 3; }
+
+bool launch_cluster_keys(const NodesDev &nd, const PrefSufCfg &cfg, const ClusterCfg &cc, int32_t node_begin, int32_t node_end, uint32_t *keys, uint32_t *vals,
+                         uint32_t *meta, void *runs, uint8_t *nruns, hipStream_t s, bool with_runs, const unsigned long long *only_if_declined, const RsFirstPass *first_pass) {
+    if (node_end <= node_begin) return false;
     const uint64_t m = (uint64_t) (node_end - node_begin);
     const unsigned long long *gate = only_if_declined;
-    const dim3 grid((unsigned) (gate ? std::min<uint64_t>((m + TK_ROWS - 1) / TK_ROWS, 8192) : (m + TK_ROWS - 1) / TK_ROWS)), block(TK_ROWS);
+    KeyTileCounts tc{nullptr, 0, 0, 0};
+    if (first_pass && first_pass->counts && !gate && node_begin == 0 && node_end == nd.n && first_pass->tile == KT_TILE && first_pass->nbits >= 1 && (1 << first_pass->nbits) <= KT_MAX_DIGITS &&
+        !with_runs && !vals && !meta && !nd.from && !nd.to && blocks_of(cfg.Lcap - 1) <= 9 && (cfg.Lcap - 1) - cfg.Lmin + 1 <= 64 &&
+        (uint64_t) first_pass->n_tiles == (m + (uint64_t) first_pass->tile - 1) / (uint64_t) first_pass->tile)
+        tc = KeyTileCounts{first_pass->counts, first_pass->shift, first_pass->nbits, first_pass->tile};
+    const dim3 grid((unsigned) (tc.counts ? first_pass->n_tiles : (gate ? std::min<uint64_t>((m + TK_ROWS - 1) / TK_ROWS, 8192) : (m + TK_ROWS - 1) / TK_ROWS))), block(TK_ROWS);
     const int32_t *nol = nullptr; const unsigned long long *noc = nullptr;
-#define NR_LAUNCH(TKW, WIDE) do { if (with_runs) hipLaunchKernelGGL((k_node_runs<TKW, WIDE, true>), grid, block, 0, s, nd, cfg, cc, (int) node_begin, (int) node_end, keys, vals, meta, (uint2 *) runs, nruns, nol, noc, gate); \
-                                  else hipLaunchKernelGGL((k_node_runs<TKW, WIDE, false>), grid, block, 0, s, nd, cfg, cc, (int) node_begin, (int) node_end, keys, vals, meta, (uint2 *) runs, nruns, nol, noc, gate); } while (0)
+#define NR_LAUNCH_(TKW, WIDE, R, T) hipLaunchKernelGGL((k_node_runs<TKW, WIDE, R, T>), grid, block, 0, s, nd, cfg, cc, (int) node_begin, (int) node_end, keys, vals, meta, (uint2 *) runs, nruns, nol, noc, gate, tc)
+#define NR_LAUNCH(TKW, WIDE) do { if (with_runs) NR_LAUNCH_(TKW, WIDE, true, false); else NR_LAUNCH_(TKW, WIDE, false, false); } while (0)
+    if (tc.counts) NR_LAUNCH_(11, false, false, true);
+    else
     if (blocks_of(cfg.Lcap - 1) > 13 || (cfg.Lcap - 1) - cfg.Lmin + 1 > 64) NR_LAUNCH(21, true);
     else if (blocks_of(cfg.Lcap - 1) <= 9) NR_LAUNCH(11, false);
     else NR_LAUNCH(17, false);
 #undef NR_LAUNCH
+#undef NR_LAUNCH_
+    return tc.counts != nullptr;
 }
 
 void launch_cluster_runs_list(const NodesDev &nd, const PrefSufCfg &cfg, const ClusterCfg &cc, const int32_t *ids, const unsigned long long *count, uint32_t cap, uint32_t grid_blocks,
@@ -1078,7 +1112,7 @@
     if (cap == 0 || nd.n <= 0) return;
     const dim3 grid(std::max<uint32_t>(1u, std::min<uint32_t>(grid_blocks, (cap + TK_ROWS - 1) / TK_ROWS))), block(TK_ROWS);
     uint32_t *nok = nullptr;
-#define NR_LAUNCH(TKW, WIDE) hipLaunchKernelGGL((k_node_runs<TKW, WIDE, true>), grid, block, 0, s, nd, cfg, cc, 0, (int) cap, nok, nok, nok, (uint2 *) runs, nruns, ids, count, (const unsigned long long *) nullptr)
+#define NR_LAUNCH(TKW, WIDE) hipLaunchKernelGGL((k_node_runs<TKW, WIDE, true>), grid, block, 0, s, nd, cfg, cc, 0, (int) cap, nok, nok, nok, (uint2 *) runs, nruns, ids, count, (const unsigned long long *) nullptr, KeyTileCounts{nullptr, 0, 0, 0})
     if (blocks_of(cfg.Lcap - 1) > 13 || (cfg.Lcap - 1) - cfg.Lmin + 1 > 64) NR_LAUNCH(21, true);
     else if (blocks_of(cfg.Lcap - 1) <= 9) NR_LAUNCH(11, false);
     else NR_LAUNCH(17, false);
@@ -1097,7 +1131,7 @@
 }
 
 hipError_t launch_cluster_sort(const NodesDev &nd, const ClusterCfg &cc, uint32_t *keys, uint32_t *vals, uint32_t *keys2, uint32_t *vals2, void *sort_temp, size_t sort_temp_bytes,
-                               bool fill_vals, hipEvent_t ev_sorted, bool test_skip_sort, hipStream_t s, bool own_sort) {
+                               bool fill_vals, hipEvent_t ev_sorted, bool test_skip_sort, hipStream_t s, bool own_sort, bool first_counts_ready) {
     if (nd.n <= 0) return hipSuccess;
     const uint64_t n = (uint64_t) nd.n;
     if (fill_vals && (!own_sort || test_skip_sort)) hipLaunchKernelGGL(k_iota, dim3((unsigned) std::min<uint64_t>((n + 255) / 256, 8192)), dim3(256), 0, s, vals, (uint32_t) n);
@@ -1105,7 +1139,7 @@
     if (test_skip_sort) {
         err = hipMemcpyAsync(keys2, keys, n * sizeof(uint32_t), hipMemcpyDeviceToDevice, s);
         if (err == hipSuccess) err = hipMemcpyAsync(vals2, vals, n * sizeof(uint32_t), hipMemcpyDeviceToDevice, s);
-    } else err = sort_u32_pairs(sort_temp, sort_temp_bytes, keys, keys2, own_sort ? (const uint32_t *) nullptr : vals, vals2, n, cc.idx_shift - 3, s, own_sort);
+    } else err = sort_u32_pairs(sort_temp, sort_temp_bytes, keys, keys2, own_sort ? (const uint32_t *) nullptr : vals, vals2, n, cluster_sort_begin_bit(cc), s, own_sort, first_counts_ready);
     if (err != hipSuccess) return err;
     if (ev_sorted) (void) hipEventRecord(ev_sorted, s);
     return hipSuccess;
diff --git a/alga_amd/csrc/prefsuf_cluster_device.h b/alga_amd/csrc/prefsuf_cluster_device.h
--- a/alga_amd/csrc/prefsuf_cluster_device.h
+++ b/alga_amd/csrc/prefsuf_cluster_device.h
@@ -96,6 +96,8 @@
 }
 
 constexpr int TK_ROWS = 128;
+constexpr int KT_TILE = 8192;
+constexpr int KT_MAX_DIGITS = 1024;
 constexpr int NR_STACK = 8;
 
 template <bool WIDE, int RCAP = CL_RMAX, int RS = 1, int RW = 0>
diff --git a/alga_amd/csrc/prefsuf_kernels.h b/alga_amd/csrc/prefsuf_kernels.h
--- a/alga_amd/csrc/prefsuf_kernels.h
+++ b/alga_amd/csrc/prefsuf_kernels.h
@@ -36,9 +36,13 @@
 
 bool       cluster_plan(const PrefSufCfg &cfg, int max_len, uint64_t live, int bucket_log2_bias, ClusterCfg *c, int *eq);
 size_t     cluster_sort_temp_bytes(uint64_t n);
-void       launch_cluster_keys(const NodesDev &nd, const PrefSufCfg &cfg, const ClusterCfg &cc, int32_t node_begin, int32_t node_end, uint32_t *keys,
+struct RsFirstPass;
+struct KeyTileCounts { uint32_t *counts; int shift, nbits, tile; };
+bool       launch_cluster_keys(const NodesDev &nd, const PrefSufCfg &cfg, const ClusterCfg &cc, int32_t node_begin, int32_t node_end, uint32_t *keys,
                                uint32_t *vals, uint32_t *meta, void *runs, uint8_t *nruns, hipStream_t s, bool with_runs = true ,
-                               const unsigned long long *only_if_declined = nullptr );
+                               const unsigned long long *only_if_declined = nullptr ,
+                               const RsFirstPass *first_pass = nullptr);
+int        cluster_sort_begin_bit(const ClusterCfg &cc);
 void       launch_cluster_runs_list(const NodesDev &nd, const PrefSufCfg &cfg, const ClusterCfg &cc, const int32_t *ids, const unsigned long long *count, uint32_t cap,
                                     uint32_t grid_blocks, void *runs, uint8_t *nruns, hipStream_t s);
 hipError_t launch_cluster_store(const NodesDev &nd, const ClusterCfg &cc, uint32_t *keys, uint32_t *vals, uint32_t *keys2 , uint32_t *vals2, void *sort_temp,
@@ -46,7 +50,8 @@
                                 unsigned long long *bad_flag ,
                                 bool test_skip_sort , hipStream_t s, bool own_sort = true);
 hipError_t launch_cluster_sort(const NodesDev &nd, const ClusterCfg &cc, uint32_t *keys, uint32_t *vals, uint32_t *keys2, uint32_t *vals2, void *sort_temp, size_t sort_temp_bytes,
-                               bool fill_vals, hipEvent_t ev_sorted, bool test_skip_sort, hipStream_t s, bool own_sort = true);
+                               bool fill_vals, hipEvent_t ev_sorted, bool test_skip_sort, hipStream_t s, bool own_sort = true,
+                               bool first_counts_ready = false );
 hipError_t launch_cluster_dir(const NodesDev &nd, const ClusterCfg &cc, const uint32_t *keys2, void *dir, unsigned long long *bad_flag, const unsigned long long *only_if_no_pure_piles,
                               hipStream_t s);
 hipError_t launch_cluster_gather(const NodesDev &nd, const ClusterCfg &cc, int eq, const uint32_t *keys2, const uint32_t *vals2, const uint32_t *meta,
@@ -101,10 +106,13 @@
 size_t     rsort_u32_pairs_temp_bytes(uint64_t n);
 void       rsort_set_variant(int v);
 hipError_t rsort_u32_pairs(void *temp, size_t temp_bytes, const uint32_t *keys_in, uint32_t *keys_out, const uint32_t *vals_in, uint32_t *vals_out, uint64_t n,
-                           int begin_bit, hipStream_t s);
+                           int begin_bit, hipStream_t s, bool first_counts_ready = false );
+struct RsFirstPass { int shift = 0, nbits = 0, tile = 0; uint32_t n_tiles = 0; uint32_t *counts = nullptr; };
+bool       rsort_u32_first_pass(void *temp, size_t temp_bytes, uint64_t n, int begin_bit, RsFirstPass *fp);
 size_t     sort_u32_pairs_temp_bytes(uint64_t n);
 hipError_t sort_u32_pairs(void *temp, size_t temp_bytes, const uint32_t *keys_in, uint32_t *keys_out, const uint32_t *vals_in, uint32_t *vals_out,
-                          uint64_t n, int begin_bit , hipStream_t s, bool own_sort = true );
+                          uint64_t n, int begin_bit , hipStream_t s, bool own_sort = true ,
+                          bool first_counts_ready = false );
 size_t     rsort_u64_pairs_temp_bytes(uint64_t n);
 hipError_t rsort_u64_pairs(void *temp, size_t temp_bytes, const unsigned long long *keys_in, unsigned long long *keys_out, const unsigned long long *vals_in,
                            unsigned long long *vals_out, uint64_t n, int bits, hipStream_t s);
diff --git a/alga_amd/csrc/radix_sort.hip b/alga_amd/csrc/radix_sort.hip
--- a/alga_amd/csrc/radix_sort.hip
+++ b/alga_amd/csrc/radix_sort.hip
@@ -93,6 +93,27 @@
         for (int j = 0; j < Q; j++) k[j] = kn[j];
     }
     for (uint32_t d = threadIdx.x; d < D; d += RS_THREADS) chunk_tot[(size_t) c * D + d] = run[d];
+}
+
+constexpr int RS_TC_AHEAD = 8;
+__global__ void __launch_bounds__(RS_THREADS) k_rs_tile_counts(int nbits, uint32_t n_tiles, uint32_t tiles_per_chunk, uint32_t *__restrict__ tile_pref,
+                                                               uint32_t *__restrict__ chunk_tot) {
+    const uint32_t D = 1u << nbits;
+    const uint32_t c = blockIdx.x, t0 = c * tiles_per_chunk, t1 = min(t0 + tiles_per_chunk, n_tiles);
+    for (uint32_t d = threadIdx.x; d < D; d += RS_THREADS) {
+        uint32_t run = 0;
+        for (uint32_t t = t0; t < t1; t += RS_TC_AHEAD) {
+            uint32_t x[RS_TC_AHEAD];
+#pragma unroll
+            for (int j = 0; j < RS_TC_AHEAD; j++) x[j] = t + j < t1 ? tile_pref[(size_t) (t + j) * D + d] : 0u;
+#pragma unroll
+            for (int j = 0; j < RS_TC_AHEAD; j++) {
+                if (t + j < t1) tile_pref[(size_t) (t + j) * D + d] = run;
+                run += x[j];
+            }
+        }
+        chunk_tot[(size_t) c * D + d] = run;
+    }
 }
 
 constexpr int RS_SC_DIGITS = 16, RS_SC_GROUPS = RS_THREADS / RS_SC_DIGITS;
@@ -404,27 +425,47 @@
 
 void rsort_set_variant(int v) { if (v == 0 || v == 1) g_rs_variant = v; }
 
+struct RsTemp32 { uint32_t *tk, *tv, *tile_pref, *chunk_tot, *digit_tot, *digit_base; };
+static RsTemp32 rs_temp32(void *temp, uint64_t n) {
+    RsTemp32 r;
+    char *at = (char *) temp;
+    r.tk = (uint32_t *) at; at += rs_align((size_t) (n + 4) * 4);
+    r.tv = (uint32_t *) at; at += rs_align((size_t) (n + 4) * 4);
+    r.tile_pref = (uint32_t *) at; at += rs_align((size_t) rs_plan(n, 0, 32, 0).n_tiles * RS_MAX_DIGITS * 4);
+    r.chunk_tot = (uint32_t *) at; at += rs_align((size_t) RS_CHUNKS * RS_MAX_DIGITS * 4);
+    r.digit_tot = (uint32_t *) at; at += rs_align(RS_MAX_DIGITS * 4);
+    r.digit_base = (uint32_t *) at;
+    return r;
+}
+
+bool rsort_u32_first_pass(void *temp, size_t temp_bytes, uint64_t n, int begin_bit, RsFirstPass *fp) {
+    if (n == 0 || begin_bit < 0 || begin_bit > 31 || n >= (1ull << 32) - RS_TILE_MAX || !temp || temp_bytes < rsort_u32_pairs_temp_bytes(n)) return false;
+    const RsPlan p = rs_plan(n, begin_bit, 32, g_rs_variant);
+    if (p.tile != 8192 || p.passes < 1) return false;
+    fp->shift = p.shift[0]; fp->nbits = p.bits[0]; fp->tile = p.tile; fp->n_tiles = p.n_tiles;
+    fp->counts = rs_temp32(temp, n).tile_pref;
+    return true;
+}
+
 hipError_t rsort_u32_pairs(void *temp, size_t temp_bytes, const uint32_t *keys_in, uint32_t *keys_out, const uint32_t *vals_in, uint32_t *vals_out, uint64_t n,
-                           int begin_bit, hipStream_t s) {
+                           int begin_bit, hipStream_t s, bool first_counts_ready) {
     if (n == 0) return hipSuccess;
     if (begin_bit < 0 || begin_bit > 31 || n >= (1ull << 32) - RS_TILE_MAX) return hipErrorInvalidValue;
     if (temp_bytes < rsort_u32_pairs_temp_bytes(n)) return hipErrorInvalidValue;
     const int variant = g_rs_variant;
     const RsPlan p = rs_plan(n, begin_bit, 32, variant);
-    char *at = (char *) temp;
-    uint32_t *tk = (uint32_t *) at; at += rs_align((size_t) (n + 4) * 4);
-    uint32_t *tv = (uint32_t *) at; at += rs_align((size_t) (n + 4) * 4);
-    uint32_t *tile_pref = (uint32_t *) at; at += rs_align((size_t) rs_plan(n, 0, 32, 0).n_tiles * RS_MAX_DIGITS * 4);
-    uint32_t *chunk_tot = (uint32_t *) at; at += rs_align((size_t) RS_CHUNKS * RS_MAX_DIGITS * 4);
-    uint32_t *digit_tot = (uint32_t *) at; at += rs_align(RS_MAX_DIGITS * 4);
-    uint32_t *digit_base = (uint32_t *) at;
+    if (first_counts_ready && p.tile != 8192) return hipErrorInvalidValue;
+    const RsTemp32 tm = rs_temp32(temp, n);
+    uint32_t *tk = tm.tk, *tv = tm.tv, *tile_pref = tm.tile_pref, *chunk_tot = tm.chunk_tot, *digit_tot = tm.digit_tot, *digit_base = tm.digit_base;
     const uint32_t *ki = keys_in, *vi = vals_in;
     for (int i = 0; i < p.passes; i++) {
         const bool to_out = ((p.passes - 1 - i) & 1) == 0;
         uint32_t *ko = to_out ? keys_out : tk, *vo = to_out ? vals_out : tv;
         const int nb = p.bits[i], sh = p.shift[i];
         const int aligned = (int) ((((uintptr_t) ki) & 15u) == 0);
-        if (p.tile == 8192)
+        if (i == 0 && first_counts_ready)
+            hipLaunchKernelGGL(k_rs_tile_counts, dim3(p.chunks), dim3(RS_THREADS), 0, s, nb, p.n_tiles, p.tiles_per_chunk, tile_pref, chunk_tot);
+        else if (p.tile == 8192)
             hipLaunchKernelGGL((k_rs_hist<8192>), dim3(p.chunks), dim3(RS_THREADS), 0, s, ki, n, sh, nb, p.n_tiles, p.tiles_per_chunk, tile_pref, chunk_tot, aligned);
         else
             hipLaunchKernelGGL((k_rs_hist<16384>), dim3(p.chunks), dim3(RS_THREADS), 0, s, ki, n, sh, nb, p.n_tiles, p.tiles_per_chunk, tile_pref, chunk_tot, aligned);
diff --git a/alga_amd/csrc/sort_records.hip b/alga_amd/csrc/sort_records.hip
--- a/alga_amd/csrc/sort_records.hip
+++ b/alga_amd/csrc/sort_records.hip
@@ -67,10 +67,11 @@
 }
 
 hipError_t sort_u32_pairs(void *temp, size_t temp_bytes, const uint32_t *keys_in, uint32_t *keys_out, const uint32_t *vals_in, uint32_t *vals_out,
-                          uint64_t n, int begin_bit, hipStream_t s, bool own_sort) {
+                          uint64_t n, int begin_bit, hipStream_t s, bool own_sort, bool first_counts_ready) {
     if (n == 0) return hipSuccess;
     if (begin_bit < 0 || begin_bit > 31) return hipErrorInvalidValue;
-    if (own_sort) return rsort_u32_pairs(temp, temp_bytes, keys_in, keys_out, vals_in, vals_out, n, begin_bit, s);
+    if (first_counts_ready && !own_sort) return hipErrorInvalidValue;
+    if (own_sort) return rsort_u32_pairs(temp, temp_bytes, keys_in, keys_out, vals_in, vals_out, n, begin_bit, s, first_counts_ready);
     if (n < (1ull << 22)) begin_bit = 0;
     if (sort_u32_three_wide_passes(begin_bit))
         return rocprim::radix_sort_pairs<Sort10>(temp, temp_bytes, keys_in, keys_out, vals_in, vals_out, (size_t) n, (unsigned) begin_bit, 32u, s);
```
